# robj0nes/VectorizedMultiAgentSimulator

Hardware: AMD Instinct MI355X
Metric: env-steps/sec (num_envs x steps / wall-s), 'balance' @32k envs, 1->8 GPU (higher is better)
Workload: dtype f32; 1 GPU; balance 32768 envs/GPU, n_agents=4, substeps=10, broadphase=batch; scenario=balance, num_envs_per_gpu=32768, global_envs=32768, n_agents=4, substeps=10, parallelism=replicas x1 (one process per GPU, no collective in the step), math=relaxed

## Files before the change

### include/vmas_mi355x.h

```cpp
#ifndef VMAS_MI355X_H
#define VMAS_MI355X_H

#ifndef __HIPCC_RTC__
#include <stdint.h>
#endif

#ifdef __cplusplus
extern "C" {
#endif

#define VMAS_ABI_VERSION 14

#define VMAS_OK 0
#define VMAS_E_INVALID (-1)
#define VMAS_E_HIP (-2)
#define VMAS_E_NOMEM (-3)
#define VMAS_E_NOCONVERGE (-4)
#define VMAS_E_UNSUPPORTED (-5)

#define VMAS_SPHERE 0
#define VMAS_BOX 1
#define VMAS_LINE 2

#define VMAS_PAIR_JOINT 0
// ... 376 lines not shown
    float* obs[VMAS_SCN_MAX_AGENTS];
    uint8_t* done;
    float* pos_rew_prev;
    const int64_t* out_delta;
} VmasBalanceIO;
int32_t vmas_balance_outputs(int32_t device, const VmasBalanceIO* io, void* stream);
int32_t vmas_test_exact_math(int32_t device, const float* a, const float* b, float* out, int64_t n, void* stream);
int32_t vmas_test_fast_trig(int32_t device, const float* x, float* out, int64_t n, void* stream);

#define VMAS_SCN_MAX_RAY_TARGETS 16
#define VMAS_FLOCK_MAX_AGENTS 16
typedef struct VmasFlockingIO {
    int32_t batch, n_all, n_policy, what;
    int32_t target, n_rays, n_ray_targets, sum_mode;
    float min_collision_distance, collision_reward, desired_distance, dist_shaping_factor;
    float max_range, pad0;
    int32_t collide_reward_on;
    int32_t fast_lidar;
    VmasShapeRef agents[VMAS_FLOCK_MAX_AGENTS];
    int32_t scripted[VMAS_FLOCK_MAX_AGENTS];
    int32_t policy[VMAS_FLOCK_MAX_AGENTS];
    VmasVec vel[VMAS_FLOCK_MAX_AGENTS];
    VmasVec rot[VMAS_FLOCK_MAX_AGENTS];
    const float* angles[VMAS_FLOCK_MAX_AGENTS];
    int32_t ang_s0[VMAS_FLOCK_MAX_AGENTS], ang_s1[VMAS_FLOCK_MAX_AGENTS];
    VmasRayTarget ray_targets[VMAS_SCN_MAX_RAY_TARGETS];
    float* t;
    const float* shaping_in[VMAS_FLOCK_MAX_AGENTS];
    float* shaping_out[VMAS_FLOCK_MAX_AGENTS];
    float* dist_rew[VMAS_FLOCK_MAX_AGENTS];
    float* collision_rew[VMAS_FLOCK_MAX_AGENTS];
    float* rewards[VMAS_FLOCK_MAX_AGENTS];
    float* obs[VMAS_FLOCK_MAX_AGENTS];
    float* lidar[VMAS_FLOCK_MAX_AGENTS];
    const int64_t* out_delta;
} VmasFlockingIO;
int32_t vmas_flocking_outputs(int32_t device, const VmasFlockingIO* io, void* stream);
int32_t vmas_flocking_target_action(int32_t device, const float* t, int32_t batch, float period, float* u,
                                    void* stream);

#define VMAS_NAV_MAX_AGENTS 16
#define VMAS_NAV_WS_WORDS 32
typedef struct VmasNavigationIO {
    int32_t batch, n_agents, what, n_rays;
    int32_t shared_rew, observe_all_goals;
    int32_t lidar_on;
    int32_t fast_lidar;
    float pos_shaping_factor, final_reward, agent_collision_penalty, min_collision_distance;
    float max_range, pad0;
    VmasShapeRef agents[VMAS_NAV_MAX_AGENTS];
    VmasVec goal_pos[VMAS_NAV_MAX_AGENTS];
    float goal_radius[VMAS_NAV_MAX_AGENTS];
    double circ[VMAS_NAV_MAX_AGENTS];
    uint32_t pair_static[VMAS_NAV_MAX_AGENTS];
    VmasVec vel[VMAS_NAV_MAX_AGENTS];
    VmasVec rot[VMAS_NAV_MAX_AGENTS];
    const float* angles[VMAS_NAV_MAX_AGENTS];
    int32_t ang_s0[VMAS_NAV_MAX_AGENTS], ang_s1[VMAS_NAV_MAX_AGENTS];
    const float* shaping_in[VMAS_NAV_MAX_AGENTS];
    float* shaping_out[VMAS_NAV_MAX_AGENTS];
    float* dist_to_goal[VMAS_NAV_MAX_AGENTS];
    uint8_t* on_goal[VMAS_NAV_MAX_AGENTS];
    float* agent_pos_rew[VMAS_NAV_MAX_AGENTS];
    float* collision_rew[VMAS_NAV_MAX_AGENTS];
    float* rewards[VMAS_NAV_MAX_AGENTS];
    float* obs[VMAS_NAV_MAX_AGENTS];
    float* lidar[VMAS_NAV_MAX_AGENTS];
    float* pos_rew;
    float* final_rew;
    uint8_t* all_goal_reached;
    uint8_t* done;
    uint32_t* ws;
    const int64_t* out_delta;
} VmasNavigationIO;
int32_t vmas_navigation_outputs(int32_t device, const VmasNavigationIO* io, void* stream);

#define VMAS_TRANSPORT_MAX_PACKAGES 8
#define VMAS_TRANSPORT_MAX_AGENTS 16
typedef struct VmasTransportIO {
    int32_t batch, n_agents, n_packages, what;
    float shaping_factor, red[3], green[3], pad0;
    VmasShapeRef package[VMAS_TRANSPORT_MAX_PACKAGES], goal[VMAS_TRANSPORT_MAX_PACKAGES];
    VmasVec package_vel[VMAS_TRANSPORT_MAX_PACKAGES];
    VmasVec agent_pos[VMAS_TRANSPORT_MAX_AGENTS], agent_vel[VMAS_TRANSPORT_MAX_AGENTS];
    const float* global_shaping[VMAS_TRANSPORT_MAX_PACKAGES];
    int32_t gs_s0[VMAS_TRANSPORT_MAX_PACKAGES];
    float* global_shaping_out[VMAS_TRANSPORT_MAX_PACKAGES];
    float* dist_to_goal[VMAS_TRANSPORT_MAX_PACKAGES];
    uint8_t* on_goal[VMAS_TRANSPORT_MAX_PACKAGES];
    float* color[VMAS_TRANSPORT_MAX_PACKAGES];
    const uint8_t* on_goal_in[VMAS_TRANSPORT_MAX_PACKAGES];
    float* rew;
    float* obs[VMAS_TRANSPORT_MAX_AGENTS];
    uint8_t* done;
    const int64_t* out_delta;
    float* rew_attr;
} VmasTransportIO;
int32_t vmas_transport_outputs(int32_t device, const VmasTransportIO* io, void* stream);

#define VMAS_DISC_MAX_AGENTS 16
#define VMAS_DISC_MAX_TARGETS 16
#define VMAS_DISC_MAX_ENTITIES 32
#define VMAS_DISC_MAX_LIDARS 2
typedef struct VmasDiscoveryIO {
    int32_t batch, n_agents, n_targets, what;
    float covering_range, covering_rew_coeff, time_penalty;
    int32_t agents_per_target, shared_reward, n_entities, n_lidars;
    int32_t time_int;
    int32_t fast_lidar;
    int64_t time_penalty_i;
    int32_t agent_entity[VMAS_DISC_MAX_AGENTS];
    int32_t target_entity[VMAS_DISC_MAX_TARGETS];
    VmasVec pos[VMAS_DISC_MAX_ENTITIES];
    float radius[VMAS_DISC_MAX_ENTITIES];
    VmasVec vel[VMAS_DISC_MAX_AGENTS], rot[VMAS_DISC_MAX_AGENTS];
    int32_t n_rays[VMAS_DISC_MAX_LIDARS];
    float max_range[VMAS_DISC_MAX_LIDARS];
    uint32_t mask[VMAS_DISC_MAX_LIDARS];
    const float* angles[VMAS_DISC_MAX_LIDARS][VMAS_DISC_MAX_AGENTS];
    int32_t ang_s0[VMAS_DISC_MAX_LIDARS][VMAS_DISC_MAX_AGENTS], ang_s1[VMAS_DISC_MAX_LIDARS][VMAS_DISC_MAX_AGENTS];
    float* lidar[VMAS_DISC_MAX_LIDARS][VMAS_DISC_MAX_AGENTS];
    float* obs[VMAS_DISC_MAX_AGENTS];
    float* agents_pos;
    float* targets_pos;
    float* dists;
    int64_t* per_target;
    uint8_t* covered;
    void* time_rew;
    float* shared;
    float* covering[VMAS_DISC_MAX_AGENTS];
    float* collision[VMAS_DISC_MAX_AGENTS];
    float* rewards[VMAS_DISC_MAX_AGENTS];
    int64_t* covered_count;
    const uint8_t* all_time;
    uint8_t* done;
    const int64_t* out_delta;
    const uint64_t* stage_in;
    uint64_t* stage_out;
} VmasDiscoveryIO;
int32_t vmas_discovery_outputs(int32_t device, const VmasDiscoveryIO* io, void* stream);

#define VMAS_COPY_STORE64 (-8)
#define VMAS_COPY_MAX_SPANS 160
typedef struct VmasCopySpan {
    const void* src;
    void* dst;
    int64_t nbytes;
} VmasCopySpan;
int32_t vmas_copy_spans(int32_t device, const VmasCopySpan* spans, int32_t n, void* stream);
int32_t vmas_copy_spans_draw(int32_t device, const VmasCopySpan* spans, int32_t n_spans, int64_t numel,
                             const VmasUniformColumn* cols, int32_t n_cols, uint64_t seed, uint64_t offset,
                             const uint64_t* offset_dev, int32_t mode, int64_t u_snap_delta, uint64_t* increment,
                             void* stream);
int32_t vmas_graph_chain_launch_tail(const VmasKernelChain* chain, int32_t wb, const VmasCopySpan* spans,
                                     int32_t n_spans, int64_t numel, const VmasUniformColumn* cols, int32_t n_cols,
                                     uint64_t seed, uint64_t offset, const uint64_t* offset_dev, int32_t mode,
                                     int64_t u_snap_delta, uint64_t* increment, void* stream);
int32_t vmas_test_tail_draw(int32_t device, const VmasUniformColumn* cols, int32_t n_cols, int64_t numel, uint64_t seed,
                            uint64_t offset, int32_t mode, uint64_t* increment, void* stream);

const char* vmas_aux_last_error(void);

typedef struct VmasGradIO {
    float* const* pos;
    float* const* vel;
    float* const* rot;
    float* const* ang_vel;
    float* const* force;
    float* const* torque;
} VmasGradIO;
int32_t vmas_world_step_vjp(const VmasWorldConfig* cfg, const VmasEntityDesc* entities,
                            const VmasPairDesc* pairs, const VmasJointDesc* joints,
                            const VmasStepIO* io, const VmasStepIO* grad_out,
                            const VmasGradIO* grad_in, void* stream);
int32_t vmas_distance_vjp(int32_t device, int32_t batch, int32_t kind, const VmasShapeRef* a,
                          const VmasShapeRef* b, const float* test_point, int32_t tp_s0, int32_t tp_s1,
                          const float* grad_out, float* grad_a_pos, float* grad_a_rot, float* grad_b_pos,
                          float* grad_b_rot, float* grad_point, void* stream);
int32_t vmas_cast_rays_vjp(int32_t device, int32_t batch, int32_t n_rays, const float* origin,
                           int32_t o_s0, int32_t o_s1, const float* angles, int32_t a_s0,
                           int32_t a_s1, const float* rot, int32_t r_s0,
                           const VmasRayTarget* targets, int32_t n_targets, float max_range,
                           const float* grad_out, float* grad_origin, float* grad_rot,
                           float* grad_angles, float* const* grad_target_pos,
                           float* const* grad_target_rot, void* stream);

typedef struct VmasJitWorld VmasJitWorld;
int32_t vmas_jit_world_create(const VmasWorldConfig* cfg, const VmasEntityDesc* entities,
                              const VmasPairDesc* pairs, const VmasJointDesc* joints,
                              VmasJitWorld** out_world);
int32_t vmas_jit_world_destroy(VmasJitWorld* world);
int32_t vmas_jit_world_step(VmasJitWorld* world, const VmasStepIO* io, void* stream,
                            int32_t* iterations);
int32_t vmas_jit_world_set_params(VmasJitWorld* world, const VmasWorldConfig* cfg,
                                  const VmasEntityDesc* entities, const VmasPairDesc* pairs,
                                  const VmasJointDesc* joints);
int32_t vmas_jit_world_check(VmasJitWorld* world);
int32_t vmas_jit_world_passes(VmasJitWorld* world, int32_t* passes);
int32_t vmas_jit_world_grid(const VmasJitWorld* world);
int32_t vmas_jit_world_set_timing(VmasJitWorld* world, int32_t enable);
int32_t vmas_jit_world_get_timing(VmasJitWorld* world, int32_t reset, double* total_ms,
                                  int64_t* launches);
int32_t vmas_jit_world_device_timing(VmasJitWorld* world, int32_t reset, double* total_ms,
                                     int64_t* launches, double* clock_ghz);
int32_t vmas_jit_world_source(const VmasJitWorld* world, char* buf, int64_t cap);
int32_t vmas_jit_world_epilogue(const VmasJitWorld* world);
int32_t vmas_jit_program_outputs(VmasJitWorld* world, int32_t kind, const void* io, void* stream);
int32_t vmas_jit_compile_check(const VmasWorldConfig* cfg, const VmasEntityDesc* entities,
                               const VmasPairDesc* pairs, const VmasJointDesc* joints, char* buf,
                               int64_t cap);
int32_t vmas_jit_world_profile(VmasJitWorld* world, uint64_t* out, int64_t cap);
const char* vmas_jit_last_error(void);
int32_t vmas_jit_stats(int64_t* compiles, int64_t* cached);

#define VMAS_PRIM_NONE 0
#define VMAS_PRIM_DISC 1
#define VMAS_PRIM_POLY 2
#define VMAS_PRIM_SEG 3
#define VMAS_PRIM_RING 4
#define VMAS_PRIM_GRID 5
#define VMAS_PRIM_BORDER 1

typedef struct VmasRenderPrim {
    int32_t kind;
    int32_t flags;
    float rgba[4];
    float p[6];
    int32_t v0, nv;
    float bbox[4];
} VmasRenderPrim;

int32_t vmas_render_frames(int32_t device, int32_t n_frames, int32_t height, int32_t width,
                           const VmasRenderPrim* prims, int32_t n_prims, const float* verts,
                           int32_t n_verts, uint8_t* out, void* stream);

#define VMAS_RENDER_AGENT 1
#define VMAS_RENDER_ACTION 2
#define VMAS_RENDER_MAX_AGENTS 32

typedef struct VmasRenderEntity {
    const float* pos;
    const float* rot;
    const float* color;
    const uint8_t* mask;
    const float* force;
    int32_t pos_s0, rot_s0, color_s0, force_s0;
    int32_t shape;
    int32_t flags;
    float radius, length, width;
    float alpha;
    float action_scale;
    int32_t slot;
    int32_t action_slot;
    int32_t vert_slot;
} VmasRenderEntity;

typedef struct VmasRenderLidar {
    const float* pos;
    const float* rot;
    const float* angles;
    const float* dist;
    const uint8_t* mask;
    int32_t pos_s0, rot_s0, angles_s0, dist_s0;
    int32_t n_rays;
    int32_t slot;
    float alpha;
    float rgb[3];
} VmasRenderLidar;

typedef struct VmasRenderScene {
    int32_t width, height;
    int32_t focus;
    int32_t n_boundary;
    float boundary[4][4];
    int32_t plot_grid;
    float grid_spacing;
    float origin[2];
    float zoom;
    float max_agent_radius;
    int32_t n_boxes;
    int32_t n_prims;
    int32_t batch;
} VmasRenderScene;

int32_t vmas_render_scene(int32_t device, int32_t n_frames, const int64_t* env_index,
                          const VmasRenderEntity* entities, int32_t n_entities,
                          const VmasRenderLidar* lidars, int32_t n_lidars,
                          const VmasRenderScene* scene, VmasRenderPrim* prims, float* verts,
                          float* bounds, void* stream);

#define VMAS_MASKED_MAX_SPANS 96
typedef struct VmasMaskedSpan {
    void* dst;
    const void* src;
    int64_t row_bytes;
    int64_t dst_stride, src_stride;
} VmasMaskedSpan;
int32_t vmas_masked_rows(int32_t device, const VmasMaskedSpan* spans, int32_t n, const uint8_t* mask, int64_t batch,
                         int32_t copy_if_set, void* stream);

typedef struct VmasMutVec {
    float* p;
    int32_t s0, s1;
} VmasMutVec;
typedef struct VmasResetEntity {
    VmasMutVec pos, vel, rot, ang_vel;
// ... 119 lines not shown
```

### vectorizedmultiagentsimulator_amd/_native.py

```python
from __future__ import annotations

import ctypes
import os
from pathlib import Path

import numpy as np

LIB_NAME = "libvmas_mi355x.so"
LIB_PATH = Path(os.environ.get("VMAS_LIB_PATH") or Path(__file__).resolve().parent / LIB_NAME)

VMAS_ABI_VERSION = 14
VMAS_SPHERE, VMAS_BOX, VMAS_LINE = 0, 1, 2
(
    VMAS_PAIR_JOINT,
    VMAS_PAIR_SS,
    VMAS_PAIR_LS,
    VMAS_PAIR_LL,
    VMAS_PAIR_BS,
    VMAS_PAIR_BL,
    VMAS_PAIR_BB,
) = range(7)
F_MOVABLE = 1 << 0
F_ROTATABLE = 1 << 1
F_HOLLOW = 1 << 2
F_AGENT = 1 << 3
F_MAX_F = 1 << 4
F_F_RANGE = 1 << 5
F_MAX_T = 1 << 6
F_T_RANGE = 1 << 7
F_MAX_SPEED = 1 << 8
F_V_RANGE = 1 << 9
F_LIN_FRIC = 1 << 10
F_ANG_FRIC = 1 << 11
F_GRAVITY = 1 << 12
BROADPHASE_BATCH = 0
BROADPHASE_ENV = 1
DIST_POINT, DIST_PAIR, OVERLAP_PAIR = 0, 1, 2
EPILOGUE_NONE, EPILOGUE_BALANCE, EPILOGUE_TRANSPORT = 0, 1, 2

EXPORTED_SYMBOLS = (
    "vmas_abi_version",
    "vmas_device_count",
    "vmas_last_error",
    "vmas_stream_abort_capture",
    "vmas_graph_launch",
    "vmas_graph_chain_build",
    "vmas_graph_chain_launch",
    "vmas_graph_chain_free",
    "vmas_graph_chain_nodes",
    "vmas_graph_chain_fused",
    "vmas_graph_chain_set_writeback",
    "vmas_graph_chain_launch_wb",
    "vmas_jit_world_epilogue",
    "vmas_jit_program_outputs",
    "vmas_host_waits",
    "vmas_test_hold",
    "vmas_balance_outputs",
    "vmas_test_exact_math",
    "vmas_test_fast_trig",
    "vmas_copy_spans",
    "vmas_spawn_targets",
    "vmas_spawn_scratch_words",
    "vmas_spawn_channel_create",
    "vmas_spawn_channel_destroy",
    "vmas_spawn_channel_arm",
    "vmas_spawn_channel_in",
    "vmas_spawn_channel_wait",
    "vmas_spawn_profile",
    "vmas_world_step_vjp",
    "vmas_distance_vjp",
    "vmas_cast_rays_vjp",
    "vmas_flocking_outputs",
    "vmas_flocking_target_action",
    "vmas_navigation_outputs",
    "vmas_sampling_outputs",
    "vmas_sampling_max_pdf",
    "vmas_assert_publish_range",
    "vmas_transport_outputs",
    "vmas_discovery_outputs",
    "vmas_world_create",
    "vmas_world_destroy",
    "vmas_world_step",
    "vmas_world_set_timing",
    "vmas_world_get_timing",
    "vmas_cast_rays",
    "vmas_distance",
    "vmas_check_actions",
    "vmas_apply_actions",
    "vmas_apply_actions_launch",
    "vmas_apply_actions_flags",
    "vmas_apply_discrete_actions",
    "vmas_apply_discrete_actions_launch",
    "vmas_uniform_columns",
    "vmas_uniform_columns_snap",
    "vmas_copy_spans_draw",
    "vmas_graph_chain_launch_tail",
    "vmas_test_tail_draw",
    "vmas_assert_create",
    "vmas_assert_destroy",
    "vmas_assert_publish",
    "vmas_assert_wait",
    "vmas_spawn_resolve",
    "vmas_aux_last_error",
    "vmas_jit_world_create",
    "vmas_jit_world_destroy",
    "vmas_jit_world_step",
    "vmas_jit_world_set_timing",
    "vmas_jit_world_get_timing",
    "vmas_jit_world_device_timing",
    "vmas_jit_world_source",
    "vmas_jit_compile_check",
    "vmas_jit_world_profile",
    "vmas_jit_world_passes",
    "vmas_jit_world_check",
    "vmas_jit_world_grid",
    "vmas_jit_world_set_params",
    "vmas_jit_stats",
    "vmas_jit_last_error",
    "vmas_render_frames",
    "vmas_render_scene",
    "vmas_masked_rows",
    "vmas_balance_reset",
    "vmas_spawn_reset",
    "vmas_action_programs",
    "vmas_velocity_pid",
)

_i32 = ctypes.c_int32
_u32 = ctypes.c_uint32
_f32 = ctypes.c_float
_vp = ctypes.c_void_p


class VmasEntityDesc(ctypes.Structure):
    _fields_ = [
        ("shape", _i32),
        ("flags", _u32),
        ("agent_index", _i32),
        ("out_lin", _i32),
        ("out_rot", _i32),
        ("out_force", _i32),
        ("out_torque", _i32),
        ("radius", _f32),
        ("half_length", _f32),
        ("half_width", _f32),
        ("mass", _f32),
        ("inertia", _f32),
        ("one_minus_drag", _f32),
        ("lin_fric", _f32),
        ("ang_fric", _f32),
        ("max_speed", _f32),
        ("v_range", _f32),
        ("max_f", _f32),
        ("f_range", _f32),
        ("max_t", _f32),
        ("t_range", _f32),
    ]


class VmasPairDesc(ctypes.Structure):
    _fields_ = [
        ("cls", _i32),
        ("ea", _i32),
        ("eb", _i32),
        ("joint", _i32),
        ("bp_radius", _f32),
        ("dmin", _f32),
    ]


class VmasJointDesc(ctypes.Structure):
    _fields_ = [
        ("delta_a_x", _f32),
        ("delta_a_y", _f32),
        ("delta_b_x", _f32),
        ("delta_b_y", _f32),
        ("dist", _f32),
        ("rotate", _i32),
        ("fixed_rotation", _f32),
        ("pad", _i32),
    ]


class VmasWorldConfig(ctypes.Structure):
    _fields_ = [
        ("n_entities", _i32),
        ("n_agents", _i32),
        ("n_pairs", _i32),
        ("n_joints", _i32),
        ("batch", _i32),
        ("device", _i32),
        ("n_out_lin", _i32),
        ("n_out_rot", _i32),
        ("n_out_force", _i32),
        ("n_out_torque", _i32),
        ("contact_margin", _f32),
        ("collision_force", _f32),
        ("joint_force", _f32),
        ("torque_constraint_force", _f32),
        ("gravity_x", _f32),
        ("gravity_y", _f32),
        ("has_world_gravity", _i32),
        ("x_semidim", _f32),
        ("y_semidim", _f32),
        ("has_x_semidim", _i32),
        ("has_y_semidim", _i32),
        ("max_substeps", _i32),
        ("export_forces", _i32),
        ("epilogue", _i32),
        ("pad_cfg", _i32),
    ]


class VmasStepIO(ctypes.Structure):
    _fields_ = [
        ("entities", _vp),
        ("agents", _vp),
        ("joints", _vp),
        ("out_pos", _vp),
        ("out_vel", _vp),
        ("out_rot", _vp),
        ("out_ang_vel", _vp),
        ("out_force", _vp),
        ("out_torque", _vp),
        ("substeps", _i32),
        ("sub_dt", _f32),
        ("broadphase", _i32),
        ("pad", _i32),
        ("out_fdict", _vp),
        ("out_tdict", _vp),
    ]


class VmasShapeRef(ctypes.Structure):
    _fields_ = [
        ("shape", _i32),
        ("pad0", _i32),
        ("radius", _f32),
        ("length", _f32),
        ("width", _f32),
        ("radius_lmd", _f32),
        ("pos", _vp),
        ("rot", _vp),
        ("pos_s0", _i32),
        ("pos_s1", _i32),
        ("rot_s0", _i32),
        ("pad", _i32),
    ]


VMAS_COPY_MAX_SPANS = 160


class VmasCopySpan(ctypes.Structure):
    _fields_ = [("src", _vp), ("dst", _vp), ("nbytes", ctypes.c_int64)]


def copy_raw(device_index: int, spans, stream) -> None:
    n = len(spans)
    if not n:
        return
    arr = (VmasCopySpan * n)()
    for i, (src, dst, nb) in enumerate(spans):
        arr[i].src, arr[i].dst, arr[i].nbytes = src, dst, nb
    check_aux(load_library().vmas_copy_spans(device_index, arr, n, stream), "vmas_copy_spans")


VMAS_SPAWN_MAX_TARGETS = 16
VMAS_SPAWN_MAX_TRIES = 65536


VMAS_SPAWN_ERR_WORD = 64
VMAS_SPAWN_OFF_END_WORD = 36
VMAS_SPAWN_RNG_WORD = 40


def spawn_words(n_targets: int) -> int:
    return 96 + 32 * n_targets + 32 * 32


class VmasSpawnTargetsIO(ctypes.Structure):
    _fields_ = [
        ("batch", _i32), ("n_agents", _i32), ("n_targets", _i32), ("mode", _i32),
        ("agents", _vp), ("ag_s0", _i32), ("ag_s1", _i32), ("ag_s2", _i32), ("max_tries", _i32),
        ("pos", _vp * VMAS_SPAWN_MAX_TARGETS), ("pos_s0", _i32 * VMAS_SPAWN_MAX_TARGETS),
        ("pos_s1", _i32 * VMAS_SPAWN_MAX_TARGETS),
        ("covered", _vp), ("cov_s0", _i32), ("cov_s1", _i32),
        ("min_dist", _f32), ("x_lo", _f32), ("x_hi", _f32), ("y_lo", _f32), ("y_hi", _f32), ("pad1", _f32),
        ("seed", ctypes.c_uint64), ("offset", ctypes.c_uint64), ("max_accepted", _vp), ("channel", _vp),
        ("backup", _vp), ("scratch", _vp), ("scratch_words", ctypes.c_int64), ("prestaged", _i32), ("pad2", _i32),
    ]


COPY_SPAN_DTYPE = np.dtype([("src", np.uint64), ("dst", np.uint64), ("nbytes", np.int64)])
VMAS_COPY_STORE64 = -8


def stream_ptr(index: int) -> int:
    return _raw_stream(index)


def _raw_stream(index):
    import torch

    return torch._C._cuda_getCurrentRawStream(index)


def launch_args(device):
    if device.type != "cuda":
        return -1, None
    import torch

    idx = device.index if device.index is not None else torch.cuda.current_device()
    return idx, stream_ptr(idx)


def copy_table(device_index: int, table: np.ndarray, lo: int, hi: int, stream) -> None:
    copy_table_at(device_index, table.ctypes.data, lo, hi, stream)


def copy_table_at(device_index: int, table_addr: int, lo: int, hi: int, stream) -> None:
    if hi > lo:
        rc = (_copy_fn or _bind_copy())(device_index, table_addr + lo * COPY_SPAN_DTYPE.itemsize, hi - lo, stream)
        if rc:
            check_aux(rc, "vmas_copy_spans")


_copy_fn = None


def _bind_copy():
    global _copy_fn
    _copy_fn = load_library().vmas_copy_spans
    return _copy_fn


def copy_spans(device_index: int, pairs, stream) -> None:
    copy_raw(device_index, [(s.data_ptr(), d.data_ptr(), d.numel() * d.element_size()) for d, s in pairs], stream)


VMAS_PRIM_NONE, VMAS_PRIM_DISC, VMAS_PRIM_POLY, VMAS_PRIM_SEG, VMAS_PRIM_RING, VMAS_PRIM_GRID = range(6)
VMAS_PRIM_BORDER = 1
VMAS_RENDER_AGENT, VMAS_RENDER_ACTION = 1, 2
VMAS_RENDER_MAX_AGENTS = 32
RENDER_PRIM_DTYPE = np.dtype([("kind", np.int32), ("flags", np.int32), ("rgba", np.float32, 4), ("p", np.float32, 6),
                              ("v0", np.int32), ("nv", np.int32), ("bbox", np.float32, 4)])
assert RENDER_PRIM_DTYPE.itemsize == 72


class VmasRenderEntity(ctypes.Structure):
    _fields_ = [("pos", _vp), ("rot", _vp), ("color", _vp), ("mask", _vp), ("force", _vp),
                ("pos_s0", _i32), ("rot_s0", _i32), ("color_s0", _i32), ("force_s0", _i32),
                ("shape", _i32), ("flags", _i32), ("radius", _f32), ("length", _f32), ("width", _f32),
                ("alpha", _f32), ("action_scale", _f32), ("slot", _i32), ("action_slot", _i32), ("vert_slot", _i32)]


class VmasRenderLidar(ctypes.Structure):
    _fields_ = [("pos", _vp), ("rot", _vp), ("angles", _vp), ("dist", _vp), ("mask", _vp),
                ("pos_s0", _i32), ("rot_s0", _i32), ("angles_s0", _i32), ("dist_s0", _i32),
                ("n_rays", _i32), ("slot", _i32), ("alpha", _f32), ("rgb", _f32 * 3)]


class VmasRenderScene(ctypes.Structure):
    _fields_ = [("width", _i32), ("height", _i32), ("focus", _i32), ("n_boundary", _i32),
                ("boundary", (_f32 * 4) * 4), ("plot_grid", _i32), ("grid_spacing", _f32), ("origin", _f32 * 2),
                ("zoom", _f32), ("max_agent_radius", _f32), ("n_boxes", _i32), ("n_prims", _i32), ("batch", _i32)]


assert ctypes.sizeof(VmasRenderEntity) == 96 and ctypes.sizeof(VmasRenderLidar) == 80


class VmasGradIO(ctypes.Structure):
    _fields_ = [("pos", _vp), ("vel", _vp), ("rot", _vp), ("ang_vel", _vp), ("force", _vp), ("torque", _vp)]


class VmasVec(ctypes.Structure):
    _fields_ = [("p", _vp), ("s0", _i32), ("s1", _i32)]


VMAS_SCN_MAX_AGENTS = 32
VMAS_SCN_REWARD, VMAS_SCN_OBS, VMAS_SCN_DONE = 1, 2, 4


class VmasBalanceIO(ctypes.Structure):
    _fields_ = [
        ("batch", _i32), ("n_agents", _i32), ("what", _i32), ("pad0", _i32),
        ("shaping_factor", _f32), ("fall_reward", _f32), ("pi", _f32), ("pad1", _f32),
        ("package", VmasShapeRef), ("goal", VmasShapeRef), ("line", VmasShapeRef), ("floor", VmasShapeRef),
        ("package_vel", VmasVec), ("line_vel", VmasVec), ("line_ang_vel", VmasVec),
        ("agent_pos", VmasVec * VMAS_SCN_MAX_AGENTS), ("agent_vel", VmasVec * VMAS_SCN_MAX_AGENTS),
        ("global_shaping", _vp), ("gs_s0", _i32), ("pad2", _i32),
        ("global_shaping_out", _vp), ("package_dist", _vp), ("pos_rew", _vp), ("ground_rew", _vp),
        ("on_the_ground", _vp),
        ("rewards", _vp * VMAS_SCN_MAX_AGENTS), ("obs", _vp * VMAS_SCN_MAX_AGENTS),
        ("done", _vp), ("pos_rew_prev", _vp),
        ("out_delta", _vp),
    ]


VMAS_MASKED_MAX_SPANS = 96
MASKED_SPAN_DTYPE = np.dtype([("dst", np.uint64), ("src", np.uint64), ("row_bytes", np.int64),
                              ("dst_stride", np.int64), ("src_stride", np.int64)])


class VmasMaskedSpan(ctypes.Structure):
    _fields_ = [("dst", _vp), ("src", _vp), ("row_bytes", ctypes.c_int64), ("dst_stride", ctypes.c_int64),
                ("src_stride", ctypes.c_int64)]


def masked_rows(device_index: int, spans, mask_ptr: int, batch: int, copy_if_set: bool, stream) -> None:
    n = len(spans)
    if not n:
        return
    tbl = np.array(spans, dtype=np.uint64)
    assert tbl.shape == (n, 5)
    check_aux(load_library().vmas_masked_rows(device_index, tbl.ctypes.data, n, mask_ptr, batch, int(bool(copy_if_set)),
                                              stream), "vmas_masked_rows")


class VmasMutVec(ctypes.Structure):
    _fields_ = [("p", _vp), ("s0", _i32), ("s1", _i32)]


class VmasResetEntity(ctypes.Structure):
    _fields_ = [("pos", VmasMutVec), ("vel", VmasMutVec), ("rot", VmasMutVec), ("ang_vel", VmasMutVec)]


class VmasBalanceResetIO(ctypes.Structure):
    _fields_ = [
        ("batch", _i32), ("n_agents", _i32), ("mode", _i32), ("pad0", _i32),
        ("seed", ctypes.c_uint64), ("offset", ctypes.c_uint64), ("mask", _vp),
        ("lo", _f32 * 4), ("hi", _f32 * 4),
        ("line_y", _f32), ("package_rel_y", _f32), ("floor_x", _f32), ("floor_y", _f32), ("agent_dy", _f32),
        ("shaping_factor", _f32),
        ("floor_length", _f32), ("floor_width", _f32), ("line_length", _f32), ("package_radius_lmd", _f32),
        ("agent_dx", _f32 * VMAS_SCN_MAX_AGENTS),
        ("goal", VmasResetEntity), ("package", VmasResetEntity), ("line", VmasResetEntity), ("floor", VmasResetEntity),
        ("agents", VmasResetEntity * VMAS_SCN_MAX_AGENTS),
        ("force", VmasMutVec * VMAS_SCN_MAX_AGENTS), ("torque", VmasMutVec * VMAS_SCN_MAX_AGENTS),
        ("on_the_ground", _vp), ("global_shaping", VmasMutVec), ("steps", _vp),
    ]


VMAS_RESET_MAX_PLACE = 16
VMAS_RESET_MAX_WRITE = 24
VMAS_RESET_MAX_AGENTS = 16
VMAS_RESET_MAX_FIXED = 8
# ... 242 lines not shown
        ("flat", "<i4"),
        ("n_comp", "<i4"),
        ("n_phys", "<i4"),
        ("nvec", "<i4", (DISCRETE_MAX_COMPONENTS,)),
    ]
)
UNIFORM_COLUMN_DTYPE = np.dtype([("out", "<u8"), ("stride", "<i8"), ("from_", "<f4"), ("to", "<f4"), ("offset", "<u8"),
                                 ("u_out", "<u8"), ("u_stride", "<i8"), ("u_range", "<f4"), ("u_mult", "<f4"),
                                 ("u_clamp", "<i4"), ("pad", "<i4")])
DYNAMICS_DIFF_DRIVE, DYNAMICS_BICYCLE, DYNAMICS_DRONE = range(3)
INTEGRATION_EULER, INTEGRATION_RK4 = 0, 1
ACTION_PROGRAM_MAX_REFS = 8
ACTION_PROGRAM_REF_DTYPE = np.dtype(
    [(k, "<u8") for k in ("u", "pos", "vel", "rot", "ang_vel", "force", "torque", "drone_in", "drone_out")]
    + [(k, "<i8") for k in ("u_s0", "u_s1", "pos_s0", "pos_s1", "vel_s0", "vel_s1", "rot_s0", "ang_s0", "force_s0",
                            "force_s1")]
    + [(k, "<i4") for k in ("kind", "integration", "div_mode", "pad")]
    + [(k, "<f4") for k in ("mass", "moment_of_inertia", "dt", "dt2", "inv_dt2", "dt_6", "l_r", "wheelbase",
                            "inv_wheelbase", "max_steering_angle", "inv_mass", "g", "mass_g", "i_yz", "i_zx", "i_xy",
                            "i_xx", "i_yy", "i_zz", "inv_i_xx", "inv_i_yy", "inv_i_zz")]
)
VELOCITY_PID_REF_DTYPE = np.dtype(
    [(k, "<u8") for k in ("u", "vel", "u_out", "err_out", "prev_err", "accum", "accum_clamped")]
    + [(k, "<i8") for k in ("u_s0", "u_s1", "vel_s0", "vel_s1")]
    + [(k, "<i4") for k in ("dim", "use_integrator", "div_mode", "pad")]
    + [(k, "<f4") for k in ("gain", "inv_ti", "t_d", "dt", "inv_dt", "cutoff", "mass", "pad2")]
)
assert ACTION_PROGRAM_REF_DTYPE.itemsize == 256
assert VELOCITY_PID_REF_DTYPE.itemsize == 136
ACTION_PROGRAM_CALLS = {"vmas_action_programs": 0, "vmas_velocity_pid": 0}


def action_programs(device_index: int, batch: int, refs: np.ndarray, stream) -> int:
    ACTION_PROGRAM_CALLS["vmas_action_programs"] += 1
    return load_library().vmas_action_programs(device_index, batch, refs.ctypes.data, len(refs), stream)


def velocity_pid(device_index: int, batch: int, ref: np.ndarray, stream) -> int:
    ACTION_PROGRAM_CALLS["vmas_velocity_pid"] += 1
    return load_library().vmas_velocity_pid(device_index, batch, ref.ctypes.data, stream)


assert UNIFORM_COLUMN_DTYPE.itemsize == 64
assert ACTION_REF_DTYPE.itemsize == 40
assert ACTION_APPLY_REF_DTYPE.itemsize == 56
assert DISCRETE_ACTION_REF_DTYPE.itemsize == 96
assert ENTITY_IO_DTYPE.itemsize == 72
assert AGENT_IO_DTYPE.itemsize == 32
assert JOINT_IO_DTYPE.itemsize == 16
assert RAY_TARGET_DTYPE.itemsize == 48 and ctypes.sizeof(VmasRayTarget) == 48
assert ctypes.sizeof(VmasEntityDesc) == 84
assert ctypes.sizeof(VmasShapeRef) == 56


class NativeLibraryError(RuntimeError):
    pass


_lib = None


def load_library(path: os.PathLike | str | None = None) -> ctypes.CDLL:
    global _lib
    if _lib is not None and path is None:
        return _lib
    p = Path(path) if path is not None else LIB_PATH
    if not p.exists():
        raise NativeLibraryError(
            f"{p} not found: build it with `python -c 'import __graft_entry__ as g; g.build()'` "
            "(the MI355X engine has no Python fallback)"
        )
    lib = ctypes.CDLL(str(p))
    lib.vmas_abi_version.restype = _i32
    lib.vmas_device_count.restype = _i32
    lib.vmas_last_error.restype = ctypes.c_char_p
    lib.vmas_host_waits.restype = _i32
    lib.vmas_host_waits.argtypes = []
    lib.vmas_test_hold.restype = _i32
    lib.vmas_test_hold.argtypes = [_i32, _i32, ctypes.c_int64, _vp]
    lib.vmas_balance_outputs.restype = _i32
    lib.vmas_balance_outputs.argtypes = [_i32, _vp, _vp]
    lib.vmas_test_exact_math.restype = _i32
    lib.vmas_test_exact_math.argtypes = [_i32, _vp, _vp, _vp, ctypes.c_int64, _vp]
    lib.vmas_test_fast_trig.restype = _i32
    lib.vmas_test_fast_trig.argtypes = [_i32, _vp, _vp, ctypes.c_int64, _vp]
    lib.vmas_discovery_outputs.restype = _i32
    lib.vmas_discovery_outputs.argtypes = [_i32, _vp, _vp]
    lib.vmas_transport_outputs.restype = _i32
    lib.vmas_transport_outputs.argtypes = [_i32, _vp, _vp]
    lib.vmas_flocking_outputs.restype = _i32
    lib.vmas_flocking_outputs.argtypes = [_i32, _vp, _vp]
    lib.vmas_navigation_outputs.restype = _i32
    lib.vmas_navigation_outputs.argtypes = [_i32, _vp, _vp]
    lib.vmas_sampling_outputs.restype = _i32
    lib.vmas_sampling_outputs.argtypes = [_i32, _vp, _vp]
    lib.vmas_sampling_max_pdf.restype = _i32
    lib.vmas_sampling_max_pdf.argtypes = [_i32, _vp, _vp]
    lib.vmas_distance_vjp.restype = _i32
    lib.vmas_distance_vjp.argtypes = [_i32, _i32, _i32, _vp, _vp, _vp, _i32, _i32, _vp, _vp, _vp, _vp, _vp, _vp, _vp]
    lib.vmas_cast_rays_vjp.restype = _i32
    lib.vmas_cast_rays_vjp.argtypes = [_i32, _i32, _i32, _vp, _i32, _i32, _vp, _i32, _i32, _vp, _i32, _vp, _i32,
                                       ctypes.c_float, _vp, _vp, _vp, _vp, _vp, _vp, _vp]
    lib.vmas_world_step_vjp.restype = _i32
    lib.vmas_world_step_vjp.argtypes = [_vp, _vp, _vp, _vp, _vp, _vp, _vp, _vp]
    lib.vmas_spawn_targets.restype = _i32
    lib.vmas_spawn_targets.argtypes = [_i32, _vp, ctypes.POINTER(ctypes.c_uint64), _vp]
    lib.vmas_spawn_scratch_words.restype = ctypes.c_int64
    lib.vmas_spawn_scratch_words.argtypes = [_i32, _i32]
    lib.vmas_spawn_channel_create.restype = _i32
    lib.vmas_spawn_channel_create.argtypes = [_i32, ctypes.POINTER(_vp)]
    lib.vmas_spawn_channel_destroy.restype = _i32
    lib.vmas_spawn_channel_destroy.argtypes = [_vp]
    lib.vmas_spawn_channel_in.restype = _i32
    lib.vmas_spawn_channel_in.argtypes = [_vp, ctypes.POINTER(_vp)]
    lib.vmas_spawn_channel_arm.restype = _i32
    lib.vmas_spawn_channel_arm.argtypes = [_vp, ctypes.c_uint64, ctypes.c_uint64, ctypes.c_uint32]
    lib.vmas_spawn_channel_wait.restype = _i32
    lib.vmas_spawn_channel_wait.argtypes = [_vp, ctypes.c_uint32, ctypes.POINTER(_i32), _i32, _vp]
    lib.vmas_spawn_profile.restype = _i32
    lib.vmas_spawn_profile.argtypes = [_vp, ctypes.c_int64]
    lib.vmas_copy_spans.restype = _i32
    lib.vmas_copy_spans.argtypes = [_i32, _vp, _i32, _vp]
    lib.vmas_copy_spans_draw.restype = _i32
    lib.vmas_copy_spans_draw.argtypes = [_i32, _vp, _i32, ctypes.c_int64, _vp, _i32, ctypes.c_uint64, ctypes.c_uint64,
                                         _vp, _i32, ctypes.c_int64, ctypes.POINTER(ctypes.c_uint64), _vp]
    lib.vmas_masked_rows.restype = _i32
    lib.vmas_masked_rows.argtypes = [_i32, _vp, _i32, _vp, ctypes.c_int64, _i32, _vp]
    lib.vmas_balance_reset.restype = _i32
    lib.vmas_balance_reset.argtypes = [_i32, _vp, ctypes.POINTER(ctypes.c_uint64), _vp]
    lib.vmas_spawn_reset.restype = _i32
    lib.vmas_spawn_reset.argtypes = [_i32, _vp, ctypes.POINTER(ctypes.c_uint64), ctypes.POINTER(_i32), _vp]
    lib.vmas_stream_abort_capture.restype = _i32
    lib.vmas_stream_abort_capture.argtypes = [_vp]
    lib.vmas_graph_launch.restype = _i32
    lib.vmas_graph_launch.argtypes = [_vp, _vp]
    lib.vmas_graph_chain_build.restype = _i32
    lib.vmas_graph_chain_build.argtypes = [_vp, _i32, ctypes.POINTER(_vp)]
    lib.vmas_graph_chain_launch.restype = _i32
    lib.vmas_graph_chain_launch.argtypes = [_vp, _vp]
    lib.vmas_graph_chain_free.restype = _i32
    lib.vmas_graph_chain_nodes.restype = _i32
    lib.vmas_graph_chain_nodes.argtypes = [_vp]
    lib.vmas_graph_chain_fused.restype = _i32
    lib.vmas_graph_chain_fused.argtypes = [_vp]
    lib.vmas_graph_chain_set_writeback.restype = _i32
    lib.vmas_graph_chain_set_writeback.argtypes = [_vp, ctypes.c_int64]
    lib.vmas_graph_chain_launch_wb.restype = _i32
    lib.vmas_graph_chain_launch_wb.argtypes = [_vp, _vp]
    lib.vmas_test_tail_draw.restype = _i32
    lib.vmas_test_tail_draw.argtypes = [_i32, _vp, _i32, ctypes.c_int64, ctypes.c_uint64, ctypes.c_uint64, _i32, _vp, _vp]
    lib.vmas_graph_chain_launch_tail.restype = _i32
    lib.vmas_graph_chain_launch_tail.argtypes = [_vp, _i32, _vp, _i32, ctypes.c_int64, _vp, _i32, ctypes.c_uint64,
                                                 ctypes.c_uint64, _vp, _i32, ctypes.c_int64, _vp, _vp]
    lib.vmas_graph_chain_free.argtypes = [_vp]
    lib.vmas_world_create.restype = _i32
    lib.vmas_world_create.argtypes = [_vp, _vp, _vp, _vp, ctypes.POINTER(_vp)]
    lib.vmas_world_destroy.restype = _i32
    lib.vmas_world_destroy.argtypes = [_vp]
    lib.vmas_world_step.restype = _i32
    lib.vmas_world_step.argtypes = [_vp, _vp, _vp, _vp]
    lib.vmas_world_set_timing.restype = _i32
    lib.vmas_world_set_timing.argtypes = [_vp, _i32]
    lib.vmas_world_get_timing.restype = _i32
    lib.vmas_world_get_timing.argtypes = [_vp, _i32, ctypes.POINTER(ctypes.c_double), ctypes.POINTER(ctypes.c_int64)]
    lib.vmas_cast_rays.restype = _i32
    lib.vmas_cast_rays.argtypes = [
        _i32, _i32, _i32, _vp, _i32, _i32, _vp, _i32, _i32, _vp, _i32, _vp, _i32, _f32, _vp, _vp,
    ]
    lib.vmas_check_actions.restype = _i32
    lib.vmas_check_actions.argtypes = [_i32, _i32, _vp, _i32, _vp, _vp]
    lib.vmas_apply_actions.restype = _i32
    lib.vmas_apply_actions.argtypes = [_i32, _i32, _vp, _i32, _vp, _vp, _vp]
    lib.vmas_apply_actions_launch.restype = _i32
    lib.vmas_apply_actions_launch.argtypes = [_i32, _i32, _vp, _i32, _vp, ctypes.POINTER(ctypes.c_uint32), _vp]
    lib.vmas_apply_actions_flags.restype = _i32
    lib.vmas_apply_actions_flags.argtypes = [_i32, ctypes.c_uint32, _i32, _vp, _vp]
    lib.vmas_apply_discrete_actions.restype = _i32
    lib.vmas_apply_discrete_actions.argtypes = [_i32, _i32, _vp, _i32, _vp, _i32, _vp, _vp]
    lib.vmas_apply_discrete_actions_launch.restype = _i32
    lib.vmas_apply_discrete_actions_launch.argtypes = [_i32, _i32, _vp, _i32, _vp, _i32, ctypes.POINTER(ctypes.c_uint32), _vp]
    lib.vmas_uniform_columns.restype = _i32
    lib.vmas_uniform_columns.argtypes = [_i32, ctypes.c_int64, _vp, _i32, ctypes.c_uint64, ctypes.c_uint64, _i32,
                                         ctypes.POINTER(ctypes.c_uint64), _vp]
    lib.vmas_uniform_columns_snap.restype = _i32
    lib.vmas_uniform_columns_snap.argtypes = [_i32, ctypes.c_int64, _vp, _i32, ctypes.c_uint64, ctypes.c_uint64, _i32,
                                              ctypes.c_int64, ctypes.POINTER(ctypes.c_uint64), _vp]
    lib.vmas_assert_create.restype = _i32
    lib.vmas_assert_create.argtypes = [_i32, _i32, ctypes.POINTER(_vp)]
    lib.vmas_assert_destroy.restype = _i32
    lib.vmas_assert_destroy.argtypes = [_vp]
    lib.vmas_assert_publish.restype = _i32
    lib.vmas_assert_publish.argtypes = [_vp, _i32, _vp, ctypes.c_int64, _vp]
    lib.vmas_assert_wait.restype = _i32
    lib.vmas_assert_wait.argtypes = [_vp, _i32, ctypes.c_uint32, ctypes.POINTER(_i32), _vp]
    lib.vmas_assert_publish_range.restype = _i32
    lib.vmas_assert_publish_range.argtypes = [_vp, _i32, _vp, ctypes.c_int64, ctypes.c_int64, _i32, _i32, _vp, _vp, _vp]
    lib.vmas_flocking_target_action.restype = _i32
    lib.vmas_flocking_target_action.argtypes = [_i32, _vp, _i32, _f32, _vp, _vp]
    lib.vmas_distance.restype = _i32
    lib.vmas_distance.argtypes = [_i32, _i32, _i32, _vp, _vp, _vp, _i32, _i32, _vp, _vp]
    lib.vmas_spawn_resolve.restype = _i32
    lib.vmas_spawn_resolve.argtypes = [
        _i32, _i32, _vp, _i32, _i32, _i32, _i32, _vp, _i32, _i32, _f32, _vp, _vp,
        ctypes.POINTER(_i32), ctypes.POINTER(_i32), _vp,
    ]
    lib.vmas_aux_last_error.restype = ctypes.c_char_p
    lib.vmas_render_frames.restype = _i32
    lib.vmas_render_frames.argtypes = [_i32, _i32, _i32, _i32, _vp, _i32, _vp, _i32, _vp, _vp]
    lib.vmas_render_scene.restype = _i32
    lib.vmas_render_scene.argtypes = [_i32, _i32, _vp, _vp, _i32, _vp, _i32, _vp, _vp, _vp, _vp, _vp]
    lib.vmas_jit_world_create.restype = _i32
    lib.vmas_jit_world_create.argtypes = [_vp, _vp, _vp, _vp, ctypes.POINTER(_vp)]
    lib.vmas_jit_world_destroy.restype = _i32
    lib.vmas_jit_world_destroy.argtypes = [_vp]
    lib.vmas_jit_world_step.restype = _i32
    lib.vmas_jit_world_step.argtypes = [_vp, _vp, _vp, _vp]
    lib.vmas_jit_world_set_timing.restype = _i32
    lib.vmas_jit_world_set_timing.argtypes = [_vp, _i32]
    lib.vmas_jit_world_get_timing.restype = _i32
    lib.vmas_jit_world_get_timing.argtypes = [_vp, _i32, ctypes.POINTER(ctypes.c_double),
                                              ctypes.POINTER(ctypes.c_int64)]
    lib.vmas_jit_world_source.restype = _i32
    lib.vmas_jit_world_source.argtypes = [_vp, _vp, ctypes.c_int64]
    lib.vmas_jit_compile_check.restype = _i32
    lib.vmas_jit_compile_check.argtypes = [_vp, _vp, _vp, _vp, _vp, ctypes.c_int64]
    lib.vmas_jit_world_profile.restype = _i32
    lib.vmas_jit_world_profile.argtypes = [_vp, _vp, ctypes.c_int64]
    lib.vmas_jit_world_passes.restype = _i32
    lib.vmas_jit_world_passes.argtypes = [_vp, ctypes.POINTER(_i32)]
    lib.vmas_jit_world_device_timing.restype = _i32
    lib.vmas_jit_world_device_timing.argtypes = [_vp, _i32, ctypes.POINTER(ctypes.c_double),
                                                 ctypes.POINTER(ctypes.c_int64), ctypes.POINTER(ctypes.c_double)]
    lib.vmas_jit_world_check.restype = _i32
    lib.vmas_jit_world_check.argtypes = [_vp]
    lib.vmas_jit_world_grid.restype = _i32
    lib.vmas_jit_world_grid.argtypes = [_vp]
    lib.vmas_jit_world_set_params.restype = _i32
    lib.vmas_jit_world_set_params.argtypes = [_vp, _vp, _vp, _vp, _vp]
    lib.vmas_jit_stats.restype = _i32
    lib.vmas_jit_stats.argtypes = [ctypes.POINTER(ctypes.c_int64), ctypes.POINTER(ctypes.c_int64)]
    lib.vmas_jit_last_error.restype = ctypes.c_char_p
    lib.vmas_jit_world_epilogue.restype = _i32
    lib.vmas_jit_world_epilogue.argtypes = [_vp]
    lib.vmas_jit_program_outputs.restype = _i32
    lib.vmas_jit_program_outputs.argtypes = [_vp, _i32, _vp, _vp]
    lib.vmas_action_programs.restype = _i32
    lib.vmas_action_programs.argtypes = [_i32, _i32, _vp, _i32, _vp]
    lib.vmas_velocity_pid.restype = _i32
    lib.vmas_velocity_pid.argtypes = [_i32, _i32, _vp, _vp]
    ver = lib.vmas_abi_version()
    if ver != VMAS_ABI_VERSION:
        raise NativeLibraryError(f"ABI version mismatch: library {ver}, python {VMAS_ABI_VERSION}")
    if path is None:
        _lib = lib
    return lib


def check(rc: int, what: str) -> None:
    if rc != 0:
        msg = load_library().vmas_last_error().decode(errors="replace")
        raise NativeLibraryError(f"{what} failed ({rc}): {msg}")


def check_jit(rc: int, what: str) -> None:
    if rc < 0:
        msg = load_library().vmas_jit_last_error().decode(errors="replace")
        raise NativeLibraryError(f"{what} failed ({rc}): {msg}")


def check_aux(rc: int, what: str) -> None:
    if rc != 0:
        msg = load_library().vmas_aux_last_error().decode(errors="replace")
        raise NativeLibraryError(f"{what} failed ({rc}): {msg}")


def jit_stats():
    c, n = ctypes.c_int64(0), ctypes.c_int64(0)
    load_library().vmas_jit_stats(ctypes.byref(c), ctypes.byref(n))
    return c.value, n.value


HOST_EXT_PATH = Path(__file__).resolve().parent / "_vmas_host.so"
_host = None


def load_host():
    global _host
    if _host is not None:
        return _host
    if not HOST_EXT_PATH.exists():
        raise NativeLibraryError(
            f"{HOST_EXT_PATH} not found: build it with `python -c 'import __graft_entry__ as g; g.build()'`")
    import importlib.util

    load_library()
    spec = importlib.util.spec_from_file_location("_vmas_host", HOST_EXT_PATH)
    mod = importlib.util.module_from_spec(spec)
    spec.loader.exec_module(mod)
    if mod.ABI_VERSION != VMAS_ABI_VERSION:
        raise NativeLibraryError(f"_vmas_host ABI {mod.ABI_VERSION} != library ABI {VMAS_ABI_VERSION}")
    _host = mod
    return mod


_fn_addrs = {}

# ... 7 lines not shown
```

### vectorizedmultiagentsimulator_amd/csrc/vmas_jit.hip

```cpp
#include <hip/hip_runtime.h>
#include <hip/hiprtc.h>
#include <hip/hip_ext.h>
#include <dlfcn.h>

#include "vmas_aux.hpp"
#include "vmas_jit_ops.hpp"
#include "vmas_jit_registry.hpp"

#include <algorithm>
#include <cstdarg>
#include <cstdio>
#include <cstdlib>
#include <cmath>
#include <cstring>
#include <memory>
#include <mutex>
#include <string>
#include <unordered_map>
#include <unordered_set>
#include <utility>
#include <vector>

#include "vmas_mi355x.h"

namespace {

thread_local std::string g_jit_err;

int32_t jfail(int32_t code, const char* fmt, ...) {
    char buf[1024];
    va_list ap;
    va_start(ap, fmt);
    vsnprintf(buf, sizeof buf, fmt, ap);
    va_end(ap);
    g_jit_err = buf;
    return code;
}

#define JHIP(x)                                                                                 \
    do {                                                                                        \
        hipError_t e_ = (x);                                                                    \
        if (e_ != hipSuccess) {                                                                 \
            (void)hipGetLastError();                                                            \
            return jfail(VMAS_E_HIP, "%s: %s", #x, hipGetErrorString(e_));                      \
        }                                                                                       \
    } while (0)

std::string fl(float v) {
    if (v != v) return "__builtin_nanf(\"\")";
    if (v == __builtin_huge_valf()) return "__builtin_huge_valf()";
    if (v == -__builtin_huge_valf()) return "(-__builtin_huge_valf())";
    char b[64];
    snprintf(b, sizeof b, "%af", (double)v);
    return b;
}
std::string it(long v) { return std::to_string(v); }
std::string bl(bool v) { return v ? "true" : "false"; }

constexpr const char* kRelaxedTag = "// vmas-math: relaxed";
constexpr const char* kFlagsTag = "// vmas-cflags:";

std::string codegen_flags(bool relaxed) {
    std::string f = " -fno-slp-vectorize";
    if (relaxed) f += " -fapprox-func -fno-hip-fp32-correctly-rounded-divide-sqrt";
    if (const char* x = getenv("VMAS_JIT_CFLAGS")) f += std::string(" ") + x;
    return f;
}


float sq_limit(float r) {
    if (!(r >= 0.f)) return -1.f;
    if (r == __builtin_huge_valf()) return __builtin_huge_valf();
    float x = r * r;
    while (x > 0.f && std::sqrt(x) > r) x = std::nextafter(x, 0.f);
    while (std::sqrt(std::nextafter(x, __builtin_huge_valf())) <= r) x = std::nextafter(x, __builtin_huge_valf());
    return x;
}

constexpr int kNW = 8;
constexpr int kMaxNW = 16;
constexpr int kProfBlocks = 4096;
constexpr int kProfRec = 24;
constexpr int kMaxArgBytes = 3584;
static_assert(sizeof(VmasBalanceIO) % 8 == 0 && sizeof(VmasTransportIO) % 8 == 0,
              "a scenario program's argument block is copied into LDS in 8-byte words");
constexpr int kEpiQRows = 28;
constexpr int kLdsTwoPerCu = 64 * 1024;
constexpr int kLdsOnePerCu = 150 * 1024;

enum Src { S_POS, S_VEL, S_ROT, S_ANG, S_GRAV, S_FORCE, S_TORQUE, S_JFIX };
enum Prm { kPrmMass, kPrmInertia, kPrmDrag, kPrmLinFric, kPrmAngFric, kPrmMaxSpeed, kPrmVRange, kPrmMaxF, kPrmFRange,
           kPrmMaxT, kPrmTRange };
inline float prm_value(const VmasEntityDesc& d, int k) {
    switch (k) {
        case kPrmMass: return d.mass;
        case kPrmInertia: return d.inertia;
        case kPrmDrag: return d.one_minus_drag;
        case kPrmLinFric: return d.lin_fric;
        case kPrmAngFric: return d.ang_fric;
        case kPrmMaxSpeed: return d.max_speed;
        case kPrmVRange: return d.v_range;
        case kPrmMaxF: return d.max_f;
        case kPrmFRange: return d.f_range;
        case kPrmMaxT: return d.max_t;
        default: return d.t_range;
    }
}
inline float prm_world_value(const VmasWorldConfig& c, int k) {
    return k == 0 ? c.gravity_x : k == 1 ? c.gravity_y : k == 2 ? c.x_semidim : c.y_semidim;
}

struct Item {
    int pair, side, torque;
};
constexpr int kWhole = -1, kFinish = -2;
struct Task {
    int pair, part;
    float cost;
};

struct Gen {
    const VmasWorldConfig& cfg;
    const std::vector<VmasEntityDesc>& ed;
    const std::vector<VmasPairDesc>& pd;
    const std::vector<VmasJointDesc>& jd;
    int E, P, A, J, W, nfl;
    bool split_boxes = true;
    bool side_prune = true;
    bool splits(int cls) const {
        return split_boxes && (cls == VMAS_PAIR_BB || (cls == VMAS_PAIR_BL && !side_prune));
    }
    long lds_budget = kLdsTwoPerCu;
    bool global_rows = false;
    int nw = kNW;
    int prof_block = -1;
    bool relaxed = false;
    std::vector<char> dyn, in_pair, need_trig, need_rot, split;
    std::vector<int> owner;
    std::vector<std::vector<int>> wave_ents, wave_static;
    std::vector<std::vector<Task>> wave_tasks;
    std::vector<std::vector<Item>> items;
    std::vector<int> split_idx;
    int n_split = 0;
    std::vector<int> r_p, r_rot, r_trig, r_res;
    int n_rows = 0;
    std::vector<std::pair<int, int>> ptr_src, str_src;
    std::vector<int> ptr_of[8], str_of[8][2];
    std::string src;

    Gen(const VmasWorldConfig& c, const std::vector<VmasEntityDesc>& e, const std::vector<VmasPairDesc>& p,
        const std::vector<VmasJointDesc>& j)
        : cfg(c), ed(e), pd(p), jd(j) {
        E = c.n_entities;
        P = c.n_pairs;
        A = c.n_agents;
        J = c.n_joints;
        W = std::max(1, (P + 31) / 32);
        nfl = 2 * c.max_substeps * W;
    }

    static int parts(int cls) { return cls == VMAS_PAIR_BL ? 4 : 8; }

    int ptr(Src s, int idx) {
        int& slot = ptr_of[s][idx];
        if (slot < 0) {
            slot = (int)ptr_src.size();
            ptr_src.push_back({s, idx});
        }
        return slot;
    }
    int str(Src s, int k, int idx) {
        int& slot = str_of[s][k][idx];
        if (slot < 0) {
            slot = (int)str_src.size();
            str_src.push_back({s * 4 + k, idx});
        }
        return slot;
    }
    int rows(int n) {
        const int r = n_rows;
        n_rows += n;
        return r;
    }

    bool plan(std::string* why) {
        dyn.assign(E, 0);
        in_pair.assign(E, 0);
        need_trig.assign(E, 0);
        need_rot.assign(E, 0);
        split.assign(P, 0);
        split_idx.assign(P, -1);
        for (int e = 0; e < E; ++e) dyn[e] = (ed[e].flags & (VMAS_F_MOVABLE | VMAS_F_ROTATABLE)) != 0;
        for (const auto& q : pd) {
            in_pair[q.ea] = in_pair[q.eb] = 1;
            if (q.cls == VMAS_PAIR_JOINT) need_trig[q.ea] = need_trig[q.eb] = need_rot[q.ea] = need_rot[q.eb] = 1;
        }
        for (int e = 0; e < E; ++e) {
            if (in_pair[e] && ed[e].shape != VMAS_SPHERE) need_trig[e] = 1;
            if (need_trig[e]) need_rot[e] = 1;
        }
        for (int p = 0; p < P; ++p) {
            split[p] = splits(pd[p].cls);
            if (split[p]) split_idx[p] = n_split++;
        }
        items.assign(E, {});
        for (int p = 0; p < P; ++p) {
            for (int side = 0; side < 2; ++side) {
                const int e = side ? pd[p].eb : pd[p].ea;
                if (!dyn[e]) continue;
                int tq = 1;
                if (pd[p].cls == VMAS_PAIR_SS) tq = 0;
                if ((pd[p].cls == VMAS_PAIR_LS || pd[p].cls == VMAS_PAIR_BS) && side == 1) tq = 0;
                items[e].push_back({p, side, tq});
            }
        }
        const float kCost[7] = {1.5f, 0.5f, 2.0f, 1.8f, 2.2f, 7.4f, 30.f};
        const float finish_cost = 3.0f;
        const float bl_part_cost = 1.8f, bb_part_cost = 3.8f;
        std::vector<Task> all;
        for (int p = 0; p < P; ++p) {
            if (split[p]) {
                for (int k = 0; k < parts(pd[p].cls); ++k)
                    all.push_back({p, k, pd[p].cls == VMAS_PAIR_BL ? bl_part_cost : bb_part_cost});
                all.push_back({p, kFinish, finish_cost});
            } else {
                all.push_back({p, kWhole, kCost[pd[p].cls]});
            }
        }
        std::stable_sort(all.begin(), all.end(), [](const Task& a, const Task& b) { return a.cost > b.cost; });
        wave_tasks.assign(nw, {});
        std::vector<float> load(nw, 0.f);
        auto place = [&](const Task& t) {
            const int w = (int)(std::min_element(load.begin(), load.end()) - load.begin());
            wave_tasks[w].push_back(t);
            load[w] += t.cost;
        };
        for (const Task& t : all) place(t);
        for (auto& v : wave_tasks)
            std::stable_sort(v.begin(), v.end(), [](const Task& a, const Task& b) {
                const int ra = a.part >= 0 ? 0 : a.part == kFinish ? 2 : 1;
                const int rb = b.part >= 0 ? 0 : b.part == kFinish ? 2 : 1;
                return ra != rb ? ra < rb : a.pair < b.pair;
            });
        owner.assign(E, -1);
        wave_ents.assign(nw, {});
        wave_static.assign(nw, {});
        {
            std::vector<int> order;
            for (int e = 0; e < E; ++e)
                if (dyn[e]) order.push_back(e);
            std::stable_sort(order.begin(), order.end(), [&](int a, int b) { return items[a].size() > items[b].size(); });
            std::vector<float> eload(nw, 0.f);
            for (int e : order) {
                const int w = (int)(std::min_element(eload.begin(), eload.end()) - eload.begin());
                owner[e] = w;
                wave_ents[w].push_back(e);
                eload[w] += 4.f + items[e].size();
            }
            int rr = 0;
            for (int e = 0; e < E; ++e)
                if (!dyn[e] && in_pair[e]) {
                    owner[e] = rr % nw;
                    wave_static[rr % nw].push_back(e);
                    ++rr;
                }
        }
        r_p.assign(E, -1);
        r_rot.assign(E, -1);
        r_trig.assign(E, -1);
        r_res.assign(P, -1);
        for (int e = 0; e < E; ++e) {
            if (!in_pair[e]) continue;
            r_p[e] = rows(2);
            if (need_rot[e]) r_rot[e] = rows(1);
            if (need_trig[e]) r_trig[e] = rows(4);
        }
        for (int p = 0; p < P; ++p) r_res[p] = rows(split[p] ? 4 * parts(pd[p].cls) + 8 : res_rows(p));
        const long red = (!global_rows && (long)std::max(n_rows, 1) * 64 >= nfl + 2) ? 0 : nfl + 2;
        const long lds = (global_rows ? 0L : (long)n_rows * 256) + (long)nfl * 4 + 4 * (n_split + 1) +
                         4L * (nfl / 2) + 4 * red + (has_epi() && !epi_q_in_rows() ? (long)kEpiQRows * 256 : 0L) +
                         (has_epi() ? (long)(cfg.epilogue == VMAS_EPILOGUE_BALANCE ? sizeof(VmasBalanceIO)
                                                                                   : sizeof(VmasTransportIO)) : 0L);
        if (lds > lds_budget) {
            *why = "LDS budget exceeded (" + it(lds) + " B)";
            return false;
        }
        for (auto& v : ptr_of) v.assign(std::max(E, std::max(A, J)) + 1, -1);
        for (auto& a : str_of)
            for (auto& v : a) v.assign(std::max(E, std::max(A, J)) + 1, -1);
        for (int e = 0; e < E; ++e) {
            if (!(dyn[e] || in_pair[e])) continue;
            ptr(S_POS, e), str(S_POS, 0, e), str(S_POS, 1, e);
            if (need_rot[e] || dyn[e]) ptr(S_ROT, e), str(S_ROT, 0, e);
            if (dyn[e]) {
                ptr(S_VEL, e), str(S_VEL, 0, e), str(S_VEL, 1, e);
                ptr(S_ANG, e), str(S_ANG, 0, e);
                if (ed[e].flags & VMAS_F_GRAVITY) ptr(S_GRAV, e), str(S_GRAV, 0, e), str(S_GRAV, 1, e);
                if (ed[e].agent_index >= 0) {
                    const int a = ed[e].agent_index;
                    ptr(S_FORCE, a), str(S_FORCE, 0, a), str(S_FORCE, 1, a);
                    ptr(S_TORQUE, a), str(S_TORQUE, 0, a);
                }
            }
        }
        for (int p = 0; p < P; ++p)
            if (pd[p].cls == VMAS_PAIR_JOINT) ptr(S_JFIX, pd[p].joint), str(S_JFIX, 0, pd[p].joint);
        if (str_src.size() % 2) str_src.push_back({-1, 0});
        plan_params();
        {
            const char* tl = getenv("VMAS_JIT_TAIL");
            tail = has_epi() && !(tl && tl[0] == '0');
            if (tail && arg_bytes() > kMaxArgBytes) tail = false;
            tail_stage = tail && lds + (long)sizeof(VmasTail) <= lds_budget;
        }
        if (arg_bytes() > kMaxArgBytes) {
            *why = "kernel argument block too large (" + it(arg_bytes()) + " B)";
            return false;
        }
        return true;
    }

    size_t n_out() const { return cfg.export_forces ? 8 : 6; }

    bool has_epi() const { return cfg.epilogue == VMAS_EPILOGUE_BALANCE || cfg.epilogue == VMAS_EPILOGUE_TRANSPORT; }
    const char* epi_type() const { return cfg.epilogue == VMAS_EPILOGUE_BALANCE ? "VmasBalanceIO" : "VmasTransportIO"; }
    std::string epi_call(const std::string& io, const std::string& g, const std::string& wave, const std::string& lane,
                         const std::string& q) const {
        if (cfg.epilogue == VMAS_EPILOGUE_BALANCE)
            return "balance_group(" + io + ", " + g + ", " + wave + ", " + it(nw) + ", " + lane + ", " + q + ")";
        return "transport_group(" + io + ", " + g + ", " + wave + ", " + it(nw) + ", " + lane + ")";
    }
    bool epi_q_in_rows() const { return !global_rows && n_rows >= kEpiQRows; }
    size_t epi_offset() const { return 8 * (std::max<size_t>(ptr_src.size(), 1) + n_out() + 7 + (global_rows ? 1 : 0)); }
    size_t wbd_offset() const { return epi_offset() + (has_epi() ? 8 : 0); }

    size_t tail_offset() const {
        const size_t n = 8 * (std::max<size_t>(ptr_src.size(), 1) + n_out() + 7 + (global_rows ? 1 : 0) + (has_epi() ? 1 : 0) + 1) +
                         4 * (std::max<size_t>(str_src.size(), 2) + 4) +
                         4 * std::max<size_t>(prm_src.size(), 1);
        return (n + 7) & ~(size_t)7;
    }
    size_t arg_bytes() const {
        return tail_offset() + (tail ? sizeof(VmasTail) : 0);
    }

    static std::string row(int r, int k = 0) { return "L[" + it((long)(r + k) * 64) + " + lane]"; }
    bool mine(int e, int w) const { return dyn[e] && owner[e] == w; }
    std::vector<char> pre_pos, pre_trig, pre_rot;
    std::string pos(int e, int w) const {
        if (mine(e, w)) return "p" + it(e);
        if (!pre_pos.empty() && pre_pos[e]) return "q" + it(e);
        return "mk(" + row(r_p[e]) + ", " + row(r_p[e], 1) + ")";
    }
    std::string rot(int e, int w) const {
        if (mine(e, w)) return "r" + it(e);
        if (!pre_rot.empty() && pre_rot[e]) return "o" + it(e);
        return row(r_rot[e]);
    }
    std::string trig(int e, int w) const {
        if (mine(e, w)) return "t" + it(e);
        if (!pre_trig.empty() && pre_trig[e]) return "u" + it(e);
        return "Trig{" + row(r_trig[e]) + ", " + row(r_trig[e], 1) + ", " + row(r_trig[e], 2) + ", " +
               row(r_trig[e], 3) + "}";
    }
    void task_reads(int w, std::vector<char>& rp, std::vector<char>& rt, std::vector<char>& rr) const {
        rp.assign(E, 0);
        rt.assign(E, 0);
        rr.assign(E, 0);
        for (const Task& k : wave_tasks[w]) {
            if (k.part == kFinish) continue;
            const VmasPairDesc& q = pd[k.pair];
            for (int side = 0; side < 2; ++side) {
                const int e = side ? q.eb : q.ea;
                if (mine(e, w)) continue;
                rp[e] = 1;
                const bool t = q.cls == VMAS_PAIR_LL || q.cls == VMAS_PAIR_BL || q.cls == VMAS_PAIR_BB ||
                               q.cls == VMAS_PAIR_JOINT ||
                               (side == 0 && (q.cls == VMAS_PAIR_LS || q.cls == VMAS_PAIR_BS));
                if (t && r_trig[e] >= 0) rt[e] = 1;
                if (q.cls == VMAS_PAIR_JOINT && r_rot[e] >= 0) rr[e] = 1;
            }
        }
    }
    std::string preload(int e, bool p, bool t, bool r) const {
        std::string o;
        if (p) o += "        const V2 q" + it(e) + " = mk(" + row(r_p[e]) + ", " + row(r_p[e], 1) + ");\n";
        if (t)
            o += "        const Trig u" + it(e) + " = Trig{" + row(r_trig[e]) + ", " + row(r_trig[e], 1) + ", " +
                 row(r_trig[e], 2) + ", " + row(r_trig[e], 3) + "};\n";
        if (r) o += "        const float o" + it(e) + " = " + row(r_rot[e]) + ";\n";
        return o;
    }
    std::string P_(Src s, int i) const { return "a.ptr[" + it(ptr_of[s][i]) + "]"; }
    std::string S_(Src s, int k, int i) const { return "a.str[" + it(str_of[s][k][i]) + "]"; }
    std::string ld2(Src s, int i, bool rb = false) const {
        return "ld2(" + (rb ? "rbp(" + P_(s, i) + ", rbd)" : P_(s, i)) + ", " + S_(s, 0, i) + ", " + S_(s, 1, i) + ", bb)";
    }
    std::string ld1(Src s, int i, bool rb = false) const {
        return (rb ? "rbp(" + P_(s, i) + ", rbd)" : P_(s, i)) + "[(long)bb * " + S_(s, 0, i) + "]";
    }
    std::string mbit(int p) const { return "(m" + it(p >> 5) + " & " + it(1u << (p & 31)) + "u)"; }
    int res(int p) const { return split[p] ? r_res[p] + 4 * parts(pd[p].cls) + 4 : r_res[p]; }

    std::string stamp(int w, const std::string& slot) const {
        if (prof_block < 0) return "";
        return "if ((b >> 6) == " + it(prof_block) + " && lane == 0) a.prof[(" + slot + ") * " + it(kMaxNW) + " + " +
               it(w) + "] = __builtin_amdgcn_s_memtime();\n";
    }

    std::string block_stamp(int k, const std::string& v) const {
        if (prof_block < 0) return "";
        return "    if (threadIdx.x == 0 && blockIdx.x < " + it(kProfBlocks) + ") a.prof[" +
               it((long)(cfg.max_substeps * 4 + 2) * kMaxNW) + " + blockIdx.x * " + it(kProfRec) + " + " + it(k) +
               "] = " + v + ";\n";
    }

    std::string desc(int e) const {
        const VmasEntityDesc& d = ed[e];
        std::string o = "{" + it(d.shape) + ", " + it(d.flags) + "u, " + it(d.agent_index) + ", " + it(d.out_lin) + ", " +
                        it(d.out_rot) + ", " + it(d.out_force) + ", " + it(d.out_torque) + ", " + fl(d.radius) + ", " +
                        fl(d.half_length) + ", " + fl(d.half_width);
        for (int k = 0; k <= kPrmTRange; ++k) o += ", 0.f";
        return o + "}";
    }
    static std::vector<int> value_fields(const VmasEntityDesc& d) {
        std::vector<int> f;
        const bool mov = d.flags & VMAS_F_MOVABLE, rotb = d.flags & VMAS_F_ROTATABLE;
        if (mov || (d.flags & VMAS_F_LIN_FRIC)) f.push_back(kPrmMass);
        if (rotb || (d.flags & VMAS_F_ANG_FRIC)) f.push_back(kPrmInertia);
        if (mov || rotb) f.push_back(kPrmDrag);
        if (d.flags & VMAS_F_LIN_FRIC) f.push_back(kPrmLinFric);
        if (d.flags & VMAS_F_ANG_FRIC) f.push_back(kPrmAngFric);
        if (d.flags & VMAS_F_MAX_SPEED) f.push_back(kPrmMaxSpeed);
        if (d.flags & VMAS_F_V_RANGE) f.push_back(kPrmVRange);
        if (d.flags & VMAS_F_MAX_F) f.push_back(kPrmMaxF);
// ... 220 lines not shown
                if (rotf)
                    bk_code += "        bk1(" + P_(S_ROT, e) + ", " + S_(S_ROT, 0, e) + ", bb, a.wbd, r" + s + ");\n        bk1(" +
                               P_(S_ANG, e) + ", " + S_(S_ANG, 0, e) + ", bb, a.wbd, w" + s + ");\n";
            }
            if (d.agent_index >= 0)
                o += "    V2 af" + s + " = " + ld2(S_FORCE, d.agent_index) + "; float at" + s + " = " +
                     ld1(S_TORQUE, d.agent_index) + ";\n";
            else
                o += "    V2 af" + s + " = mk(0.f, 0.f); float at" + s + " = 0.f;\n";
            if (d.flags & VMAS_F_GRAVITY) o += "    const V2 eg" + s + " = " + ld2(S_GRAV, e) + ";\n";
            else o += "    const V2 eg" + s + " = mk(0.f, 0.f);\n";
            if (need_trig[e])
                o += "    Trig t" + s + " = make_trig_for(r" + s + ", " + bl(d.shape == VMAS_BOX) + ");\n";
            publish(o, e, "    ", true, true);
            if (cfg.export_forces) o += "    float lfx" + s + " = 0.f, lfy" + s + " = 0.f, ltq" + s + " = 0.f;\n";
            o += runtime_desc(e, "    ");
        }
        const std::string pro = it((long)cfg.max_substeps * 4);
        if (w == 0) o += "    if (spec && threadIdx.x == 0) QL[65] = spec_ok ? 1u : 0u;\n";
        o += "    " + stamp(w, pro);
        o += "    __syncthreads();\n";
        o += "    const bool own = !spec || QL[65] != 0u;  // (a lost speculative claim: compute, store nothing)\n";
        if (!bk_code.empty()) o += "    if (bk && valid && own) {\n" + bk_code + "    }\n";
        o += "    " + stamp(w, pro + " + 1");
        std::vector<char> rp, rt, rr;
        task_reads(w, rp, rt, rr);
        for (int e = 0; e < E; ++e)
            if (!dyn[e] && (rp[e] || rt[e] || rr[e])) o += preload(e, rp[e], rt[e], rr[e]).substr(4);
        o += "    for (int s = 0; s < a.S; ++s) {\n";
        o += "        if (4 * s < a.S) __builtin_amdgcn_s_setprio(3); else if (2 * s < a.S) __builtin_amdgcn_s_setprio(2);"
             " else if (4 * s < 3 * a.S) __builtin_amdgcn_s_setprio(1); else __builtin_amdgcn_s_setprio(0);\n";
        std::vector<char> word(W, 0);
        for (const Task& t : wave_tasks[w]) word[t.pair >> 5] = 1;
        for (int e : wave_ents[w])
            for (const Item& x : items[e]) word[x.pair >> 5] = 1;
        for (int k = 0; k < W; ++k)
            if (word[k]) o += "        const uint32_t m" + it(k) + " = MSK[s * " + it(W) + " + " + it(k) + "];\n";
        std::vector<char> fword(W, 0);
        for (const Task& t : wave_tasks[w]) fword[t.pair >> 5] = 1;
        for (int k = 0; k < W; ++k)
            if (fword[k]) o += "        uint32_t fr" + it(k) + " = 0u, fz" + it(k) + " = 0u;\n";
        for (int e = 0; e < E; ++e)
            if (dyn[e] && (rp[e] || rt[e] || rr[e])) o += preload(e, rp[e], rt[e], rr[e]);
        pre_pos = rp;
        pre_trig = rt;
        pre_rot = rr;
        for (const Task& t : wave_tasks[w]) task_code(o, t, w);
        pre_pos.clear();
        pre_trig.clear();
        pre_rot.clear();
        o += flag_flush(fword);
        o += "        " + stamp(w, "s * 4");
        o += "        __syncthreads();\n";
        o += "        " + stamp(w, "s * 4 + 1");
        if (w == 0 && n_split)
            o += "        for (int i = lane; i < " + it(n_split) + "; i += 64) DONE[i] = 0u;\n";
        for (int e : wave_ents[w]) {
            const VmasEntityDesc& d = ed[e];
            const std::string s = it(e);
            const bool mov = d.flags & VMAS_F_MOVABLE, rotb = d.flags & VMAS_F_ROTATABLE;
            o += "        {  // entity " + s + "\n";
            o += "            float fx, fy, tq;\n";
            o += "            pre_forces(D" + s + ", " + bl(d.agent_index >= 0) + ", af" + s + ", at" + s + ", v" + s +
                 ", w" + s + ", eg" + s + ", " + bl(d.flags & VMAS_F_GRAVITY) + ", GX, GY, HAS_G, a.sdt, fx, fy, tq);\n";
            int k = 0;
            for (const Item& x : items[e]) {
                const int r = res(x.pair);
                const std::string c = "c" + it(k++);
                if (mov) o += "            const float " + c + "x = " + row(r) + ", " + c + "y = " + row(r, 1) + ";\n";
                if (rotb && x.torque) o += "            const float " + c + "t = " + row(r, x.side ? 3 : 2) + ";\n";
            }
            k = 0;
            for (const Item& x : items[e]) {
                const std::string c = "c" + it(k++), m = mbit(x.pair);
                if (mov) {
                    const std::string sx = x.side ? "-" + c + "x" : c + "x", sy = x.side ? "-" + c + "y" : c + "y";
                    o += "            fx = " + m + " ? fx + " + sx + " : fx; fy = " + m + " ? fy + " + sy + " : fy;\n";
                }
                if (rotb && x.torque) o += "            tq = " + m + " ? tq + " + c + "t : tq;\n";
            }
            if (cfg.export_forces) o += "            lfx" + s + " = fx; lfy" + s + " = fy; ltq" + s + " = tq;\n";
            o += "            integrate(D" + s + ", s, a.sdt, fx, fy, tq, HAS_XS, XS, HAS_YS, YS, p" + s + ", v" + s +
                 ", r" + s + ", w" + s + ");\n";
            if (need_trig[e] && rotb)
                o += "            t" + s + " = make_trig_for(r" + s + ", " + bl(d.shape == VMAS_BOX) + ");\n";
            publish(o, e, "            ", mov, rotb);
            o += "        }\n";
        }
        o += "        " + stamp(w, "s * 4 + 2");
        o += "        __syncthreads();\n";
        o += "        " + stamp(w, "s * 4 + 3");
        o += "    }\n";
        if (!wave_ents[w].empty()) {
            o += "    if (valid && own) {\n";
            for (int e : wave_ents[w]) {
                const VmasEntityDesc& d = ed[e];
                const std::string s = it(e);
                if (d.out_lin >= 0)
                    o += "        st_out2(a.out[0], (size_t)" + it(d.out_lin) + " * a.B + b, p" + s + ");\n        st_out2(a.out[1], (size_t)" +
                         it(d.out_lin) + " * a.B + b, v" + s + ");\n";
                if (d.out_rot >= 0)
                    o += "        st_out1(a.out[2], (size_t)" + it(d.out_rot) + " * a.B + b, r" + s + ");\n        st_out1(a.out[3], (size_t)" +
                         it(d.out_rot) + " * a.B + b, w" + s + ");\n";
                if (d.agent_index >= 0) {
                    if (d.out_force >= 0)
                        o += "        st_out2(a.out[4], (size_t)" + it(d.out_force) + " * a.B + b, af" + s + ");\n";
                    if (d.out_torque >= 0)
                        o += "        st_out1(a.out[5], (size_t)" + it(d.out_torque) + " * a.B + b, at" + s + ");\n";
                }
                if (cfg.export_forces)
                    o += "        st_out2(a.out[6], (size_t)" + s + " * a.B + b, mk(lfx" + s + ", lfy" + s +
                         "));\n        st_out1(a.out[7], (size_t)" + s + " * a.B + b, ltq" + s + ");\n";
                if (d.out_lin >= 0 || d.out_rot >= 0) {
                    o += "        if (wbk) {\n";
                    if (d.out_lin >= 0)
                        o += "            wb2(" + P_(S_POS, e) + ", " + S_(S_POS, 0, e) + ", " + S_(S_POS, 1, e) + ", b, p" + s +
                             ");\n            wb2(" + P_(S_VEL, e) + ", " + S_(S_VEL, 0, e) + ", " + S_(S_VEL, 1, e) + ", b, v" +
                             s + ");\n";
                    if (d.out_rot >= 0)
                        o += "            wb1(" + P_(S_ROT, e) + ", " + S_(S_ROT, 0, e) + ", b, r" + s + ");\n            wb1(" +
                             P_(S_ANG, e) + ", " + S_(S_ANG, 0, e) + ", b, w" + s + ");\n";
                    o += "        }\n";
                }
            }
            o += "    }\n";
        }
        o += "    return own;\n}\n\n";
    }

    std::string wb_helpers() const {
        return "__device__ __forceinline__ const float* rbp(const float* p, long long d) {\n"
               "    return reinterpret_cast<const float*>(reinterpret_cast<const char*>(p) + d);\n}\n"
               "__device__ __forceinline__ void bk1(const float* p, int s0, int b, long long d, float v) {\n"
               "    st_out1(const_cast<float*>(rbp(p, d)), (size_t)((long)b * s0), v);\n}\n"
               "__device__ __forceinline__ void bk2(const float* p, int s0, int s1, int b, long long d, V2 v) {\n"
               "    float* q = const_cast<float*>(rbp(p, d));\n"
               "    st_out1(q, (size_t)((long)b * s0), v.x);\n    st_out1(q, (size_t)((long)b * s0 + s1), v.y);\n}\n"
               "__device__ __forceinline__ void wb1(const float* p, int s0, int b, float v) {\n"
               "    const_cast<float*>(p)[(long)b * s0] = v;\n}\n"
               "__device__ __forceinline__ void wb2(const float* p, int s0, int s1, int b, V2 v) {\n"
               "    float* q = const_cast<float*>(p);\n    q[(long)b * s0] = v.x;\n    q[(long)b * s0 + s1] = v.y;\n}\n\n";
    }

    bool tail = false;
    bool tail_stage = false;
    std::string epi_text() const {
        if (!has_epi()) return "";
        return "        if (a.epi) {\n"
               "            __syncthreads();\n"
               "            " + epi_call("*PROG_IOP", "g", "wave", "lane", epi_q_in_rows() ? "L" : "EQ") + ";\n"
               "            __syncthreads();\n"
               "        }\n";
    }
    std::string loop_text() const {
        return "    bool spec = persistent && spec_first, spec_ok = true, own = true;\n"
               "    if (spec && threadIdx.x == 0) spec_ok = grid_claim(claim, (int)blockIdx.x, (CURP)->base);\n"
               "    for (;;) {\n"
               "        const int g = spec ? (int)blockIdx.x : grid_next(persistent, a.ctl, claim, a.mask, MSK, nwords, ngrp, CURP, QL);\n"
               "        if (g < 0) break;\n" + block_stamp(4, "__builtin_amdgcn_s_memrealtime()") +
               "        if (persistent) {\n"
               "            for (int i = threadIdx.x; i < nfl; i += blockDim.x) FL[i] = 0u;\n"
               "            __syncthreads();\n"
               "        }\n"
               "        {\n"
               "            const int b = g * 64 + lane;\n"
               "            const bool valid = b < a.B;\n"
               "            const int bb = valid ? b : (a.B - 1);\n"
               "            // the state write-back (Args.wbd, wb_text): this pass's inputs, its backup\n"
               "            const bool wbx = persistent && a.wbd != 0;\n"
               "            const long long rbd = (wbx && (CURP)->pass > 0) ? a.wbd : 0ll;\n"
               "            const bool bk = wbx && (CURP)->pass == 0;\n"
               "            own = run<WAVE>(a, L, FL, DONE, MSK, lane, b, bb, valid, rbd, bk, wbx, spec, spec_ok, QL);\n"
               "        }\n"
               "        spec = false;\n"
               "        if (!own) continue;\n" + epi_text() +
               "        if (persistent && grid_finish(g, FL, nfl, a.blk, a.mask, MSK, a.ctl, a.err, a.herr, nwords, ngrp, CURP,\n"
               "                                      a.max_pass, RED, &QL[65], a.tm, t0s.rt, t0s.sc))\n"
               "            poison_outputs(a);\n" + block_stamp(5, "__builtin_amdgcn_s_memrealtime()") +
               "    }\n";
    }

    void generate() {
        std::string& o = src;
        o += "// generated by vmas_jit.hip for one world\n";
        if (relaxed) o += std::string(kRelaxedTag) + "\n#define VMAS_PHYS_RELAXED 1\n";
        o += std::string(kFlagsTag) + codegen_flags(relaxed) + "\n";
        if (prof_block >= 0) o += "#define VMAS_JIT_PROFILE_SLOTS 1\n";
        if (const char* mp = getenv("VMAS_JIT_TEST_PASSES"))
            o += "#define VMAS_GRID_MIN_PASSES " + it(std::max(1, atoi(mp))) + "\n";
        o += "#include \"vmas_jit_ops.hpp\"\n";
        if (has_epi()) o += "#include \"vmas_programs.hpp\"\n";
        o += "using namespace vmas;\n\n";
        o += "struct Args {\n    const float* ptr[" + it(std::max<size_t>(ptr_src.size(), 1)) +
             "];\n    float* out[" + it(n_out()) + "];\n    uint32_t* mask;\n    uint32_t* blk;\n    unsigned long long* prof;\n"
             "    uint32_t* ctl;\n    uint32_t* err;\n    uint32_t* herr;\n    unsigned long long* tm;\n" +
             std::string(global_rows ? "    float* rows;\n" : "") +
             std::string(has_epi() ? std::string("    const ") + epi_type() + "* epi;\n" : std::string()) +
             "    long long wbd;\n" +
             "    int str[" + it(std::max<size_t>(str_src.size(), 2)) + "];\n    int B, S;\n    float sdt;\n    int max_pass;\n"
             "    float prm[" + it(std::max<size_t>(prm_src.size(), 1)) + "];\n" +
             std::string(tail ? "    VmasTail tail;\n" : "") + "};\n"
             "static_assert(sizeof(Args) == " + it((long)arg_bytes()) + ", \"argument block layout\");\n\n";
        o += "__device__ __forceinline__ V2 ld2(const float* p, int s0, int s1, int b) {\n"
             "    return mk(p[(long)b * s0], p[(long)b * s0 + s1]);\n}\n\n";
        o += wb_helpers();
        o += "constexpr WorldK WK{" + fl(cfg.contact_margin) + ", " + fl(cfg.collision_force) + ", " +
             fl(cfg.joint_force) + ", " + fl(cfg.torque_constraint_force) + "};\n";
        o += "__shared__ float PRM[" + it(std::max<size_t>(prm_src.size(), 1)) + "];\n";
        o += "constexpr float GX = " + fl(cfg.gravity_x) + ", GY = " + fl(cfg.gravity_y) + ";\n";
        o += "constexpr float XS = " + fl(cfg.x_semidim) + ", YS = " + fl(cfg.y_semidim) + ";\n";
        o += "constexpr bool HAS_G = " + bl(cfg.has_world_gravity) + ";\n";
        o += "constexpr bool HAS_XS = " + bl(cfg.has_x_semidim) + ", HAS_YS = " + bl(cfg.has_y_semidim) + ";\n";
        for (int e = 0; e < E; ++e)
            if (dyn[e]) o += "constexpr VmasEntityDesc D" + it(e) + "c" + desc(e) + ";\n";
        o += "\ntemplate <int WAVE>\n__device__ __forceinline__ bool run(const Args& a, float* L, uint32_t* FL, "
             "uint32_t* DONE, const uint32_t* MSK, int lane, int b, int bb, bool valid, long long rbd, bool bk, bool wbk, "
             "bool spec, bool spec_ok, uint32_t* QL);\n\n";
        for (int w = 0; w < nw; ++w) wave_body(o, w);
        const int waves_per_eu = (lds_budget <= kLdsTwoPerCu ? 2 : 1) * nw / 4;
        {
            const int n_lin = cfg.n_out_lin, n_rot = cfg.n_out_rot, n_f = cfg.n_out_force, n_t = cfg.n_out_torque;
            const int per_env[6] = {2 * n_lin, 2 * n_lin, n_rot, n_rot, 2 * n_f, n_t};
            o += "__device__ __forceinline__ void poison_outputs(const Args& a) {\n"
                 "    const float nan = __builtin_nanf(\"\");\n";
            for (int k = 0; k < 6; ++k)
                if (per_env[k] > 0)
                    o += "    for (size_t i = threadIdx.x; i < (size_t)" + it(per_env[k]) +
                         " * a.B; i += blockDim.x) a.out[" + it(k) + "][i] = nan;\n";
            o += "}\n\n";
        }
        o += "template <int WAVE>\n__device__ __forceinline__ void group_loop(const Args& a, float* L, uint32_t* FL, uint32_t* DONE, "
             "uint32_t* MSK, uint32_t* QL, uint32_t* RED, float* EQ, GridCursor* CURP, uint32_t* claim, TimerStart t0s, "
             "bool persistent, bool spec_first, int nfl, int nwords, int ngrp, int lane, int wave" +
             std::string(has_epi() ? std::string(", const ") + epi_type() + "* PROG_IOP" : std::string()) + ") {\n    (void)EQ;\n";
        o += loop_text();
        o += "}\n\n";
        o += "__device__ __forceinline__ void world_body(const Args& a) {\n";
        if (global_rows)
            o += "    float* L = a.rows + (size_t)blockIdx.x * " + it((long)std::max(n_rows, 1) * 64) + ";\n";
        else
            o += "    __shared__ __attribute__((aligned(16))) float L[" + it(std::max(n_rows, 1) * 64) + "];\n";
        o += "    __shared__ uint32_t FL[" + it(nfl) + "];\n";
        if (has_epi() && !epi_q_in_rows()) o += "    __shared__ float EQ[" + it((long)kEpiQRows * 64) + "];\n";
        if (has_epi()) o += std::string("    __shared__ __attribute__((aligned(16))) ") + epi_type() + " PROG_IO;\n";
        o += "    __shared__ uint32_t DONE[" + it(std::max(n_split, 1)) + "];\n";
        if (tail_stage)
            o += "    __shared__ __attribute__((aligned(16))) VmasTail TL;\n";
        const int red_words = nfl + 2;
        o += "    __shared__ uint32_t MSK[" + it(std::max(nfl / 2, 1)) + "];\n";
        o += "    __shared__ uint32_t QL[66];\n";
        if (!global_rows && (long)std::max(n_rows, 1) * 64 >= red_words)
            o += "    uint32_t* RED = reinterpret_cast<uint32_t*>(L);\n";
        else
            o += "    __shared__ uint32_t RED[" + it(red_words) + "];\n";
        o += "    const int lane = threadIdx.x & 63, wave = threadIdx.x >> 6;\n";
        o += "    const int nfl = 2 * a.S * " + it(W) + ", nwords = a.S * " + it(W) + ", ngrp = (a.B + 63) >> 6;\n"
             "    for (int i = threadIdx.x; i < " + it(n_split) + "; i += blockDim.x) DONE[i] = 0u;\n";
        o += "    const bool persistent = a.ctl != nullptr;\n"
             "    uint32_t* claim = a.mask + " + it(vmas::grid_claim_offset((long)cfg.max_substeps * W)) + ";\n"
             "    const TimerStart t0s = device_timer_start(persistent ? a.tm : nullptr, true);\n"
             "    __shared__ GridCursor CUR;\n"
             "    const bool spec_first = persistent && (int)blockIdx.x < ngrp;  // (the speculative first group: loop_text)\n"
             "    if (threadIdx.x == 0)\n"
             "        CUR = GridCursor{0, (int)blockIdx.x + (spec_first ? (int)gridDim.x : 0), 0, 0, 0, persistent ? ld64(&a.ctl[kGridEpoch]) : 0ull, 0};\n"
             "    for (int i = threadIdx.x; i < nfl; i += blockDim.x) FL[i] = 0u;\n"
             "    for (int i = threadIdx.x; i < nwords; i += blockDim.x) MSK[i] = ~ld_agent(&a.mask[i]);\n" +
             std::string(has_epi() ?
                 "    if (a.epi)\n"
                 "        for (int i = threadIdx.x; i < (int)(sizeof(PROG_IO) / 8); i += blockDim.x)\n"
                 "            reinterpret_cast<unsigned long long*>(&PROG_IO)[i] = reinterpret_cast<const unsigned long long*>(a.epi)[i];\n"
                 : "") +
             std::string(tail_stage ?
                 "    if (persistent && a.tail.n_items > 0) {\n"
                 "        const unsigned long long* ka = reinterpret_cast<const unsigned long long*>(\n"
                 "            (const char*)__builtin_amdgcn_kernarg_segment_ptr() + " + it((long)tail_offset()) + ");\n"
                 "        for (int i = threadIdx.x; i < (int)(sizeof(VmasTail) / 8); i += blockDim.x)\n"
                 "            reinterpret_cast<unsigned long long*>(&TL)[i] = ka[i];\n"
                 "    }\n"
                 : "") +
             prm_copy() +
             "    __syncthreads();\n" +
             block_stamp(0, "__builtin_amdgcn_s_memrealtime()") + block_stamp(1, "__builtin_amdgcn_s_getreg(63492)") +
             block_stamp(2, "__builtin_amdgcn_s_getreg(30740)") +
             (prof_block >= 0 ? "    if (lane == 0 && blockIdx.x < " + it(kProfBlocks) + ") a.prof[" +
                                    it((long)(cfg.max_substeps * 4 + 2) * kMaxNW) + " + blockIdx.x * " + it(kProfRec) +
                                    " + 8 + wave] = __builtin_amdgcn_s_getreg(63492);\n"
                              : "") +
             (prof_block >= 0 ? "    if (threadIdx.x == 0) vmas_prof_blk = a.prof + " + it((long)(cfg.max_substeps * 4 + 2) * kMaxNW) + ";\n" : "") +
             "";
        std::string sw = "    switch (wave) {\n";
        for (int w = 0; w < nw; ++w)
            sw += "        case " + it(w) + ": group_loop<" + it(w) + ">(a, L, FL, DONE, MSK, QL, RED, " +
                  std::string(has_epi() && !epi_q_in_rows() ? "EQ" : "nullptr") +
                  ", &CUR, claim, t0s, persistent, spec_first, nfl, nwords, ngrp, lane, wave" +
                  std::string(has_epi() ? ", &PROG_IO" : "") + "); break;\n";
        o += sw + "        default: break;\n    }\n";
        o += block_stamp(3, "__builtin_amdgcn_s_memrealtime()") +
             std::string(tail ? "    // the replay's post-replay work (vmas_tail.hpp): every group's final pass is decided\n"
                                "    if (persistent && a.tail.n_items > 0) " +
                                    std::string(tail_stage ? "vmas_tail::run(TL)" : "vmas_tail::run(a.tail)") + ";\n" : "") +
             "    if (!persistent) {\n"
             "        if (!a.blk) return;\n"
             "        __syncthreads();\n"
             "        for (int i = threadIdx.x; i < nfl; i += blockDim.x) st_agent(&a.blk[(size_t)blockIdx.x * nfl + i], FL[i]);\n"
             "        return;\n"
             "    }\n"
             "}\n\n";
        const std::string bounds = "__launch_bounds__(" + it(nw * 64) + ", " + it(waves_per_eu) + ")";
        o += "extern \"C\" __global__ void " + bounds + " k_world(Args a) {\n    world_body(a);\n}\n";
        if (has_epi())
            o += "\nextern \"C\" __global__ void __launch_bounds__(" + it(nw * 64) + ") k_program_jit(" + epi_type() + " io_arg) {\n"
                 "    VMAS_PROGRAM_ARGS(" + epi_type() + ", io_arg);\n"
                 "    __shared__ float Q[" + it((long)kEpiQRows * 64) + "];\n"
                 "    " + epi_call("io", "blockIdx.x", "(int)(threadIdx.x >> 6)", "(int)(threadIdx.x & 63)", "Q") + ";\n}\n";
    }
};

std::unique_ptr<Gen> make_plan(const VmasWorldConfig& cfg, const std::vector<VmasEntityDesc>& ed,
                               const std::vector<VmasPairDesc>& pd, const std::vector<VmasJointDesc>& jd,
                               std::string* why, int force_nw = 0) {
    const char* sp = getenv("VMAS_JIT_SPLIT");
    const bool allow_split = !(sp && sp[0] == '0');
    const char* spr = getenv("VMAS_JIT_SIDE_PRUNE");
    const bool side_prune = !(spr && spr[0] == '0');
    const struct {
        bool split;
        long budget;
        bool global_rows;
    } tries[] = {{true, kLdsTwoPerCu, false}, {false, kLdsTwoPerCu, false}, {false, kLdsOnePerCu, false},
                 {false, kLdsOnePerCu, true}};
    for (const auto& t : tries) {
        if (t.split && !allow_split) continue;
        std::unique_ptr<Gen> g(new Gen(cfg, ed, pd, jd));
        if ((size_t)cfg.max_substeps * g->W > 1024) {
            *why = "too many substeps x pairs";
            return nullptr;
        }
        g->split_boxes = t.split;
        g->side_prune = side_prune;
        g->lds_budget = t.budget;
        g->global_rows = t.global_rows;
        int n_tasks = 0;
        for (const auto& q : pd)
            n_tasks += g->splits(q.cls) ? Gen::parts(q.cls) + 1 : 1;
        g->nw = n_tasks >= 32 ? 16 : kNW;
        if (const char* nws = getenv("VMAS_JIT_WAVES")) g->nw = atoi(nws) == 16 ? 16 : kNW;
        if (force_nw) g->nw = force_nw;
        why->clear();
        if (g->plan(why)) return g;
    }
    return nullptr;
}

__global__ void __launch_bounds__(1024) k_jit_flags_reduce(const uint32_t* blk, int nblk, int S, int W,
                                                           uint32_t* mask, uint32_t* viol_out) {
    __shared__ uint32_t R[1024], Z[1024];
    __shared__ uint32_t viol;
    const int nwords = S * W;
    for (int w = threadIdx.x; w < nwords; w += blockDim.x) {
        R[w] = 0u;
        Z[w] = 0u;
    }
    if (threadIdx.x == 0) viol = 0u;
    __syncthreads();
    const int groups = max(1, (int)blockDim.x / nwords);
    if ((int)threadIdx.x < groups * nwords) {
        const int w = threadIdx.x % nwords, g0 = threadIdx.x / nwords;
        uint32_t r = 0u, z = 0u;
        for (int i = g0; i < nblk; i += groups) {
            r |= blk[(size_t)i * 2 * nwords + w];
            z |= blk[(size_t)i * 2 * nwords + nwords + w];
        }
        if (r) atomicOr(&R[w], r);
        if (z) atomicOr(&Z[w], z);
    }
    __syncthreads();
    for (int w = threadIdx.x; w < nwords; w += blockDim.x) {
        const uint32_t m = ~mask[w];
        if ((m & ~R[w] & Z[w]) | (~m & R[w])) atomicOr(&viol, 1u);
    }
    __syncthreads();
    if (viol)
        for (int w = threadIdx.x; w < nwords; w += blockDim.x) mask[w] = ~R[w];
    if (threadIdx.x == 0) *viol_out = viol;
}

bool relaxed_math(const VmasWorldConfig& cfg) {
    const char* m = getenv("VMAS_JIT_MATH");
    return !(m && std::string(m) == "exact") && cfg.n_joints == 0;
}

std::mutex g_cache_mu;
std::unordered_map<std::string, std::pair<std::vector<char>, uint64_t>> g_code_cache;
uint64_t g_cache_tick = 0;
constexpr size_t kCodeCacheMax = 32;
size_t code_cache_max() {
    const char* c = getenv("VMAS_JIT_CACHE");
    return c ? (size_t)std::max(1, atoi(c)) : kCodeCacheMax;
}

std::string module_dir() {
    Dl_info info{};
    if (dladdr((const void*)&jfail, &info) && info.dli_fname) {
        std::string p = info.dli_fname;
        const size_t k = p.rfind('/');
        return k == std::string::npos ? std::string(".") : p.substr(0, k);
    }
    return ".";
}

int64_t g_jit_compiles = 0;

int32_t compile(const std::string& src, std::vector<char>* code) {
    {
        std::lock_guard<std::mutex> lk(g_cache_mu);
        auto f = g_code_cache.find(src);
        if (f != g_code_cache.end()) {
            *code = f->second.first;
            f->second.second = ++g_cache_tick;
            return VMAS_OK;
        }
    }
    const std::string dir = module_dir();
    const std::string inc1 = "-I" + dir + "/csrc", inc2 = "-I" + dir + "/../include";
    std::vector<const char*> opts = {"--offload-arch=gfx950", "-O3", "-std=c++17", "-ffp-contract=off", "-fno-fast-math",
                                     inc1.c_str(), inc2.c_str()};
    std::vector<std::string> extra;
    const size_t at = src.find(kFlagsTag);
    if (at != std::string::npos) {
        const size_t b = at + strlen(kFlagsTag), e = src.find('\n', b);
        const std::string line = src.substr(b, e == std::string::npos ? std::string::npos : e - b);
        std::string t;
        for (char c : line + " ") {
            if (c == ' ') {
                if (!t.empty()) extra.push_back(t);
                t.clear();
            } else {
                t += c;
            }
        }
    }
    for (const std::string& x : extra) opts.push_back(x.c_str());
    hiprtcProgram prog;
    if (hiprtcCreateProgram(&prog, src.c_str(), "vmas_world.hip", 0, nullptr, nullptr) != HIPRTC_SUCCESS)
        return jfail(VMAS_E_HIP, "hiprtcCreateProgram failed");
    const hiprtcResult rc = hiprtcCompileProgram(prog, (int)opts.size(), opts.data());
    if (rc != HIPRTC_SUCCESS) {
        size_t n = 0;
        hiprtcGetProgramLogSize(prog, &n);
        std::string log(n + 1, '\0');
        hiprtcGetProgramLog(prog, &log[0]);
        hiprtcDestroyProgram(&prog);
        return jfail(VMAS_E_HIP, "hipRTC compile failed: %.900s", log.c_str());
    }
    size_t n = 0;
    hiprtcGetCodeSize(prog, &n);
    code->resize(n);
    hiprtcGetCode(prog, code->data());
    hiprtcDestroyProgram(&prog);
    std::lock_guard<std::mutex> lk(g_cache_mu);
    ++g_jit_compiles;
    while (!g_code_cache.empty() && g_code_cache.size() >= code_cache_max()) {
        auto lru = g_code_cache.begin();
        for (auto it2 = g_code_cache.begin(); it2 != g_code_cache.end(); ++it2)
            if (it2->second.second < lru->second.second) lru = it2;
        g_code_cache.erase(lru);
    }
    g_code_cache[src] = {*code, ++g_cache_tick};
    return VMAS_OK;
}

}

namespace vmas {
namespace {
std::mutex g_fn_mu;
std::unordered_map<const void*, JitFnInfo> g_live_fns;
}
void fn_register(hipFunction_t f, const JitFnInfo& info) {
    std::lock_guard<std::mutex> lk(g_fn_mu);
    g_live_fns[(const void*)f] = info;
}
void fn_unregister(hipFunction_t f) {
    if (!f) return;
    std::lock_guard<std::mutex> lk(g_fn_mu);
    g_live_fns.erase((const void*)f);
}
bool jit_fn_info(const void* f, JitFnInfo* out) {
    std::lock_guard<std::mutex> lk(g_fn_mu);
    auto it = g_live_fns.find(f);
    if (it == g_live_fns.end()) return false;
    if (out) *out = it->second;
    return true;
}
}

struct VmasJitWorld {
    VmasWorldConfig cfg{};
    std::vector<VmasEntityDesc> ed;
    std::vector<VmasPairDesc> pd;
    std::vector<VmasJointDesc> jd;
    std::string src;
    std::vector<std::pair<int, int>> ptr_src, str_src, prm_src;
    size_t arg_bytes = 0;
    int W = 1, nblk = 0, nw = kNW;
    hipModule_t mod = nullptr;
    hipFunction_t fn = nullptr;
    hipFunction_t fn_prog = nullptr;
    size_t epi_offset = 0;
    uint32_t *d_mask = nullptr, *d_blk = nullptr, *d_viol = nullptr, *h_viol = nullptr;
    uint32_t *d_ctl = nullptr, *d_err = nullptr, *h_err = nullptr, *dh_err = nullptr;
    int grid = 0;
    int max_passes = 0;
    hipStream_t last_stream = nullptr;
    int last_passes = 0;
    bool last_persistent = false;
    unsigned long long* d_prof = nullptr;
    size_t n_prof = 0;
    bool timing = false;
    std::vector<std::pair<hipEvent_t, hipEvent_t>> ev_pending, ev_free;
    double timed_ms = 0.0;
    long timed_launches = 0;
    unsigned long long* d_tm = nullptr;
    int wall_khz = 0;
    bool global_rows = false;
    float* d_rows = nullptr;
};

extern "C" {

const char* vmas_jit_last_error(void) { return g_jit_err.c_str(); }

int32_t vmas_jit_stats(int64_t* compiles, int64_t* cached) {
    std::lock_guard<std::mutex> lk(g_cache_mu);
    if (compiles) *compiles = g_jit_compiles;
    if (cached) *cached = (int64_t)g_code_cache.size();
    return VMAS_OK;
}

int32_t vmas_jit_world_destroy(VmasJitWorld* W) {
    if (!W) return VMAS_OK;
    if (W->cfg.device >= 0) {
        (void)hipSetDevice(W->cfg.device);
        vmas::chain_free_drain();
        vmas::fn_unregister(W->fn);
        vmas::fn_unregister(W->fn_prog);
        if (W->mod) (void)hipModuleUnload(W->mod);
        if (W->d_mask) (void)hipFree(W->d_mask);
        if (W->d_blk) (void)hipFree(W->d_blk);
        if (W->d_viol) (void)hipFree(W->d_viol);
        if (W->h_viol) (void)hipHostFree(W->h_viol);
        if (W->d_prof) (void)hipFree(W->d_prof);
        if (W->d_rows) (void)hipFree(W->d_rows);
        if (W->d_ctl) (void)hipFree(W->d_ctl);
        if (W->d_err) (void)hipFree(W->d_err);
        if (W->h_err) (void)hipHostFree(W->h_err);
        for (auto& ev : W->ev_pending) { (void)hipEventDestroy(ev.first); (void)hipEventDestroy(ev.second); }
        for (auto& ev : W->ev_free) { (void)hipEventDestroy(ev.first); (void)hipEventDestroy(ev.second); }
        if (W->d_tm) (void)hipFree(W->d_tm);
    }
    delete W;
    return VMAS_OK;
}

int32_t vmas_jit_world_create(const VmasWorldConfig* cfg, const VmasEntityDesc* entities, const VmasPairDesc* pairs,
                              const VmasJointDesc* joints, VmasJitWorld** out_world) {
    if (!cfg || !out_world) return jfail(VMAS_E_INVALID, "null argument");
    if (cfg->device < 0) return jfail(VMAS_E_INVALID, "the specialised step is a GPU path (device >= 0)");
    if (cfg->batch <= 0 || cfg->n_entities <= 0 || cfg->n_pairs < 0 || cfg->max_substeps <= 0)
        return jfail(VMAS_E_INVALID, "bad world config");
    auto* W = new VmasJitWorld();
    W->cfg = *cfg;
    W->ed.assign(entities, entities + cfg->n_entities);
    W->pd.assign(pairs, pairs + cfg->n_pairs);
    if (cfg->n_joints) W->jd.assign(joints, joints + cfg->n_joints);
    for (const auto& q : W->pd)
        if (q.ea < 0 || q.ea >= cfg->n_entities || q.eb < 0 || q.eb >= cfg->n_entities || q.cls < 0 || q.cls > 6 ||
            (q.cls == VMAS_PAIR_JOINT && (q.joint < 0 || q.joint >= cfg->n_joints))) {
            delete W;
            return jfail(VMAS_E_INVALID, "bad pair table");
        }
    auto cleanup = [&](int32_t rc) {
        vmas_jit_world_destroy(W);
        return rc;
    };
    JHIP(hipSetDevice(cfg->device));
    std::string why;
    std::unique_ptr<Gen> gp;
    for (int force_nw : {0, kNW}) {
        gp = make_plan(W->cfg, W->ed, W->pd, W->jd, &why, force_nw);
        if (!gp) {
            delete W;
            return jfail(VMAS_E_INVALID, "world not specialised: %s", why.c_str());
        }
        Gen& g = *gp;
        if (const char* pb = getenv("VMAS_JIT_PROFILE")) g.prof_block = std::max(0, atoi(pb));
        g.relaxed = relaxed_math(W->cfg);
        g.generate();
        std::vector<char> code;
        if (int32_t rc = compile(g.src, &code)) return cleanup(rc);
        if (W->mod) {
            W->fn = nullptr;
            (void)hipModuleUnload(W->mod);
            W->mod = nullptr;
        }
        if (hipModuleLoadData(&W->mod, code.data()) != hipSuccess)
            return cleanup(jfail(VMAS_E_HIP, "hipModuleLoadData"));
        if (hipModuleGetFunction(&W->fn, W->mod, "k_world") != hipSuccess)
            return cleanup(jfail(VMAS_E_HIP, "hipModuleGetFunction"));
        int scratch = 0;
        (void)hipFuncGetAttribute(&scratch, HIP_FUNC_ATTRIBUTE_LOCAL_SIZE_BYTES, W->fn);
        if (scratch == 0 || g.nw == kNW) break;
    }
    Gen& g = *gp;
    W->src = g.src;
    W->ptr_src = g.ptr_src;
    W->str_src = g.str_src;
    W->prm_src = g.prm_src;
    W->arg_bytes = g.arg_bytes();
    W->W = g.W;
    W->nw = g.nw;
    W->nblk = (cfg->batch + 63) / 64;
    if (g.has_epi()) {
        if (hipModuleGetFunction(&W->fn_prog, W->mod, "k_program_jit") != hipSuccess)
            return cleanup(jfail(VMAS_E_HIP, "hipModuleGetFunction(k_program_jit)"));
        W->epi_offset = g.epi_offset();
    }
    {
        vmas::JitFnInfo info{};
        info.kind = vmas::kJitFnWorld;
        info.world = W;
        info.world_fn = W->fn;
        info.arg_bytes = W->arg_bytes;
        info.epi_offset = W->fn_prog ? (long)W->epi_offset : -1L;
        info.wbd_offset = (long)g.wbd_offset();
        info.tail_offset = g.tail ? (long)g.tail_offset() : -1L;
        info.batch = cfg->batch;
        info.epilogue = g.has_epi() ? cfg->epilogue : VMAS_EPILOGUE_NONE;
        info.io_bytes = cfg->epilogue == VMAS_EPILOGUE_BALANCE ? sizeof(VmasBalanceIO)
                        : cfg->epilogue == VMAS_EPILOGUE_TRANSPORT ? sizeof(VmasTransportIO) : 0;
        vmas::fn_register(W->fn, info);
        if (W->fn_prog) {
            info.kind = vmas::kJitFnProgram;
            vmas::fn_register(W->fn_prog, info);
        }
    }
    const size_t nwords = (size_t)cfg->max_substeps * W->W;
    if (hipMalloc((void**)&W->d_mask, nwords * 4) != hipSuccess ||
        hipMalloc((void**)&W->d_blk, (size_t)W->nblk * 2 * nwords * 4) != hipSuccess ||
        hipMalloc((void**)&W->d_viol, 4) != hipSuccess ||
        hipHostMalloc((void**)&W->h_viol, 4, hipHostMallocDefault) != hipSuccess)
        return cleanup(jfail(VMAS_E_NOMEM, "hipMalloc broadphase scratch"));
    const size_t ctl_words = vmas::kGridCtlWords + (size_t)vmas::grid_claim_offset((long)nwords) +
                             (size_t)W->nblk * vmas::kClaimStride;
    if (hipMalloc((void**)&W->d_ctl, ctl_words * 4) != hipSuccess || hipMalloc((void**)&W->d_err, 4) != hipSuccess ||
        hipHostMalloc((void**)&W->h_err, 4, hipHostMallocMapped | hipHostMallocCoherent) != hipSuccess ||
        hipHostGetDevicePointer((void**)&W->dh_err, W->h_err, 0) != hipSuccess ||
        hipMemset(W->d_err, 0, 4) != hipSuccess ||
        hipMemset(W->d_ctl, 0, ctl_words * 4) != hipSuccess)
        return cleanup(jfail(VMAS_E_NOMEM, "hipMalloc fixed-point control words"));
    *W->h_err = 0u;
    if (hipMalloc((void**)&W->d_tm, 8 * 8) != hipSuccess || hipMemset(W->d_tm, 0, 8 * 8) != hipSuccess ||
        hipDeviceGetAttribute(&W->wall_khz, hipDeviceAttributeWallClockRate, cfg->device) != hipSuccess ||
        W->wall_khz <= 0)
        return cleanup(jfail(VMAS_E_HIP, "device timer (hipMalloc / wall clock rate)"));
    {
        const char* gm = getenv("VMAS_JIT_GRID");
        const std::string mode = gm ? gm : "persistent";
        int per_cu = 0, cus = 0;
        if (mode != "host" &&
            hipModuleOccupancyMaxActiveBlocksPerMultiprocessor(&per_cu, W->fn, W->nw * 64, 0) == hipSuccess &&
            hipDeviceGetAttribute(&cus, hipDeviceAttributeMultiprocessorCount, cfg->device) == hipSuccess &&
            per_cu > 0 && cus > 0) {
            W->grid = std::min(W->nblk, per_cu * cus);
            if (const char* cap = getenv("VMAS_JIT_GRID_CAP")) W->grid = std::max(1, std::min(W->grid, atoi(cap)));
            if (const char* r = getenv("VMAS_JIT_MAX_PASSES")) W->max_passes = std::max(1, atoi(r));
        }
    }
    W->global_rows = g.global_rows;
    if (g.global_rows) {
        const size_t slab = (size_t)std::max(W->nblk, W->grid) * (size_t)std::max(g.n_rows, 1) * 64 * 4;
        if (hipMalloc((void**)&W->d_rows, slab) != hipSuccess) return cleanup(jfail(VMAS_E_NOMEM, "hipMalloc row slabs"));
    }
    if (g.prof_block >= 0) {
        W->n_prof = ((size_t)cfg->max_substeps * 4 + 2) * kMaxNW + (size_t)kProfBlocks * kProfRec;
        if (hipMalloc((void**)&W->d_prof, W->n_prof * 8) != hipSuccess ||
            hipMemset(W->d_prof, 0, W->n_prof * 8) != hipSuccess)
            return cleanup(jfail(VMAS_E_NOMEM, "hipMalloc profile buffer"));
    }
    *out_world = W;
    return VMAS_OK;
}

int32_t vmas_jit_world_profile(VmasJitWorld* W, uint64_t* out, int64_t cap) {
    if (!W) return jfail(VMAS_E_INVALID, "null world");
    if (!W->d_prof) return 0;
    JHIP(hipSetDevice(W->cfg.device));
    JHIP(hipDeviceSynchronize());
    const size_t n = std::min<size_t>(W->n_prof, cap > 0 ? (size_t)cap : 0);
    if (out && n) JHIP(hipMemcpy(out, W->d_prof, n * 8, hipMemcpyDeviceToHost));
    return (int32_t)W->n_prof;
}

int32_t vmas_jit_compile_check(const VmasWorldConfig* cfg, const VmasEntityDesc* entities, const VmasPairDesc* pairs,
                               const VmasJointDesc* joints, char* buf, int64_t cap) {
    if (!cfg || cfg->n_entities <= 0 || cfg->max_substeps <= 0) return jfail(VMAS_E_INVALID, "bad world config");
    std::vector<VmasEntityDesc> ed(entities, entities + cfg->n_entities);
    std::vector<VmasPairDesc> pd(pairs, pairs + cfg->n_pairs);
    std::vector<VmasJointDesc> jd;
    if (cfg->n_joints) jd.assign(joints, joints + cfg->n_joints);
    std::string why;
    std::unique_ptr<Gen> gp = make_plan(*cfg, ed, pd, jd, &why);
    if (!gp) return jfail(VMAS_E_INVALID, "world not specialised: %s", why.c_str());
    Gen& g = *gp;
    g.relaxed = relaxed_math(*cfg);
    g.generate();
    std::vector<char> code;
    if (int32_t rc = compile(g.src, &code)) return rc;
    if (buf && cap > 0) {
        const size_t k = std::min<size_t>(g.src.size(), (size_t)cap - 1);
        memcpy(buf, g.src.data(), k);
        buf[k] = '\0';
    }
    return (int32_t)g.src.size();
}

int32_t vmas_jit_world_source(const VmasJitWorld* W, char* buf, int64_t cap) {
    if (!W) return jfail(VMAS_E_INVALID, "null world");
    const int64_t n = (int64_t)W->src.size();
    if (buf && cap > 0) {
        const int64_t k = std::min(n, cap - 1);
        memcpy(buf, W->src.data(), (size_t)k);
        buf[k] = '\0';
    }
    return (int32_t)std::min<int64_t>(n, INT32_MAX);
}

int32_t vmas_jit_world_step(VmasJitWorld* W, const VmasStepIO* io, void* stream_, int32_t* iterations) {
    if (!W || !io) return jfail(VMAS_E_INVALID, "null argument");
    const VmasWorldConfig& cfg = W->cfg;
    if (io->substeps <= 0 || io->substeps > cfg.max_substeps)
        return jfail(VMAS_E_INVALID, "substeps %d outside [1, %d]", io->substeps, cfg.max_substeps);
    int cur = -1;
    JHIP(hipGetDevice(&cur));
    if (cur != cfg.device) JHIP(hipSetDevice(cfg.device));
    hipStream_t stream = (hipStream_t)stream_;
    std::vector<char> buf(W->arg_bytes, 0);
    char* p = buf.data();
    auto put_ptr = [&](const void* v) {
        memcpy(p, &v, 8);
        p += 8;
    };
    auto put_i32 = [&](int32_t v) {
        memcpy(p, &v, 4);
        p += 4;
    };
    for (const auto& s : W->ptr_src) {
        const int i = s.second;
        const VmasEntityIO* e = io->entities + (s.first <= S_GRAV ? i : 0);
        switch (s.first) {
            case S_POS: put_ptr(e->pos); break;
            case S_VEL: put_ptr(e->vel); break;
            case S_ROT: put_ptr(e->rot); break;
            case S_ANG: put_ptr(e->ang_vel); break;
            case S_GRAV: put_ptr(e->gravity); break;
            case S_FORCE: put_ptr(io->agents[i].force); break;
            case S_TORQUE: put_ptr(io->agents[i].torque); break;
            default: put_ptr(io->joints ? io->joints[i].fixed_rotation : nullptr); break;
        }
    }
    if (W->ptr_src.empty()) put_ptr(nullptr);
    put_ptr(io->out_pos);
    put_ptr(io->out_vel);
    put_ptr(io->out_rot);
    put_ptr(io->out_ang_vel);
    put_ptr(io->out_force);
    put_ptr(io->out_torque);
    if (W->cfg.export_forces) {
        put_ptr(io->out_fdict);
        put_ptr(io->out_tdict);
    }
    const bool batch_bp = io->broadphase == VMAS_BROADPHASE_BATCH;
    const bool persistent = batch_bp && W->grid > 0;
    uint32_t* nmask = persistent ? W->d_ctl + vmas::kGridCtlWords : W->d_mask;
    put_ptr(nmask);
    put_ptr(batch_bp ? W->d_blk : nullptr);
    put_ptr(W->d_prof);
    put_ptr(persistent ? W->d_ctl : nullptr);
    put_ptr(W->d_err);
// ... 248 lines not shown
```

### vectorizedmultiagentsimulator_amd/csrc/vmas_jit_ops.hpp

```cpp
#pragma once

#include "vmas_physics.hpp"
#include "vmas_tail.hpp"

namespace vmas {


#ifndef __HIP_MEMORY_SCOPE_AGENT
#define __HIP_MEMORY_SCOPE_AGENT 4
#endif

constexpr uint32_t kGridErrNoConverge = 2u, kGridErrStateTimeout = 4u;
constexpr unsigned long long kGridStartWaitTicks = 1000000000ull;

constexpr int kGridMaxPasses = 64, kGridShards = 32;
constexpr int kGridEpoch = 32, kGridStartBase = 64, kGridCand = 96, kGridTop = 128, kGridDone = 160;
constexpr int kGridDec = kGridDone + 32 * kGridShards;
constexpr int kGridStart = kGridDec + 2 * kGridMaxPasses;
constexpr int kGridCtlWords = kGridStart + 32 * kGridShards;
static_assert(kGridCtlWords % 32 == 0, "mask words start on a 128-byte line");

__host__ __device__ constexpr long grid_claim_offset(long mask_words) { return (mask_words + 31) / 32 * 32; }

typedef unsigned long long u64;
__device__ __forceinline__ u64 ld64(const uint32_t* p) {
    return __hip_atomic_load(reinterpret_cast<const u64*>(p), __ATOMIC_RELAXED, __HIP_MEMORY_SCOPE_AGENT);
}
__device__ __forceinline__ void st64(uint32_t* p, u64 v) {
    __hip_atomic_store(reinterpret_cast<u64*>(p), v, __ATOMIC_RELAXED, __HIP_MEMORY_SCOPE_AGENT);
}
__device__ __forceinline__ u64 add64(uint32_t* p, u64 v) {
    return __hip_atomic_fetch_add(reinterpret_cast<u64*>(p), v, __ATOMIC_RELAXED, __HIP_MEMORY_SCOPE_AGENT);
}
__device__ __forceinline__ bool cas64(uint32_t* p, u64 expect, u64 v) {
    return __hip_atomic_compare_exchange_strong(reinterpret_cast<u64*>(p), &expect, v, __ATOMIC_RELAXED,
                                                __ATOMIC_RELAXED, __HIP_MEMORY_SCOPE_AGENT);
}

__device__ __forceinline__ bool grid_arrive(uint32_t* ctl, uint32_t g, uint32_t ngrp, u64 G) {
    const uint32_t k = g % kGridShards, n_k = (ngrp + kGridShards - 1u - k) / kGridShards;
    const uint32_t n_top = ngrp < (uint32_t)kGridShards ? ngrp : (uint32_t)kGridShards;
    if (add64(&ctl[kGridDone + 32 * k], 1ull) != (u64)n_k * (G + 1ull) - 1ull) return false;
    return add64(&ctl[kGridTop], 1ull) == (u64)n_top * (G + 1ull) - 1ull;
}

__device__ __forceinline__ uint32_t ld_agent(const uint32_t* p) {
    return __hip_atomic_load(p, __ATOMIC_RELAXED, __HIP_MEMORY_SCOPE_AGENT);
}
__device__ __forceinline__ void st_agent(uint32_t* p, uint32_t v) {
    __hip_atomic_store(p, v, __ATOMIC_RELAXED, __HIP_MEMORY_SCOPE_AGENT);
}
__device__ __forceinline__ uint32_t add_agent(uint32_t* p, uint32_t v) {
    return __hip_atomic_fetch_add(p, v, __ATOMIC_RELAXED, __HIP_MEMORY_SCOPE_AGENT);
}
__device__ __forceinline__ bool cas_agent(uint32_t* p, uint32_t expect, uint32_t v) {
    return __hip_atomic_compare_exchange_strong(p, &expect, v, __ATOMIC_RELAXED, __ATOMIC_RELAXED,
                                                __HIP_MEMORY_SCOPE_AGENT);
}
__device__ __forceinline__ void st_out1(float* p, size_t i, float v) {
    __hip_atomic_store(reinterpret_cast<uint32_t*>(p) + i, __float_as_uint(v), __ATOMIC_RELAXED, __HIP_MEMORY_SCOPE_AGENT);
}
__device__ __forceinline__ void st_out2(float* p, size_t i, V2 v) {
    const unsigned long long bits = (unsigned long long)__float_as_uint(v.x) | ((unsigned long long)__float_as_uint(v.y) << 32);
    __hip_atomic_store(reinterpret_cast<unsigned long long*>(p) + i, bits, __ATOMIC_RELAXED, __HIP_MEMORY_SCOPE_AGENT);
}

struct TimerStart {
    unsigned long long rt, sc;
};
__device__ __forceinline__ TimerStart device_timer_start(unsigned long long* tm, bool stamp_start) {
    TimerStart t{0ull, 0ull};
    if (tm && threadIdx.x == 0) {
        t.rt = __builtin_amdgcn_s_memrealtime();
        t.sc = __builtin_amdgcn_s_memtime();
        if (stamp_start && blockIdx.x == 0)
            __hip_atomic_store(&tm[0], t.rt, __ATOMIC_RELAXED, __HIP_MEMORY_SCOPE_AGENT);
    }
    return t;
}

__device__ __forceinline__ void report_err(uint32_t* err, uint32_t* herr, uint32_t bit) {
    const uint32_t v = atomicOr(err, bit) | bit;
    if (herr) __hip_atomic_store(herr, v, __ATOMIC_RELAXED, __HIP_MEMORY_SCOPE_SYSTEM);
}

constexpr int kClaimStride = 32;

__device__ __forceinline__ bool grid_claim(uint32_t* claim, int g, u64 G) {
    return cas64(&claim[(size_t)g * kClaimStride], G, G + 1ull);
}

__device__ __forceinline__ int grid_steal(uint32_t* claim, int ngrp, u64 G, uint32_t* LIST, bool* seen) {
    if (threadIdx.x == 0) LIST[64] = 0u;
    __syncthreads();
    for (int g = (int)threadIdx.x; g < ngrp; g += (int)blockDim.x) {
        uint32_t* w = &claim[(size_t)g * kClaimStride];
        if (ld64(w) != G) continue;
        const uint32_t i = atomicAdd(&LIST[64], 1u);
        if (i < 64u) LIST[i] = cas64(w, G, G + 1ull) ? (uint32_t)g : ~0u;
    }
    __syncthreads();
    const uint32_t r = LIST[64];
    __syncthreads();
    *seen = r != 0u;
    return r < 64u ? (int)r : 64;
}

__device__ __forceinline__ void grid_started(uint32_t* ctl) {
    __builtin_amdgcn_s_waitcnt(0);
    (void)add64(&ctl[kGridStart + 32 * (int)(blockIdx.x % kGridShards)], 1ull);
}

__device__ __forceinline__ u64 grid_starts(const uint32_t* ctl) {
    const uint32_t nsh = gridDim.x < (uint32_t)kGridShards ? gridDim.x : (uint32_t)kGridShards;
    u64 v = threadIdx.x < nsh ? ld64(&ctl[kGridStart + 32 * (int)threadIdx.x]) : 0ull;
    for (int off = 16; off > 0; off >>= 1) v += __shfl_xor(v, off, 64);
    return __shfl(v, 0, 64);
}

__device__ __forceinline__ bool grid_complete(uint32_t* ctl, int g, int ngrp, u64 G, uint32_t* FLAG) {
    __builtin_amdgcn_s_waitcnt(0);
    __syncthreads();
    if (threadIdx.x == 0) *FLAG = grid_arrive(ctl, (uint32_t)g, (uint32_t)ngrp, G) ? 1u : 0u;
    __syncthreads();
    const bool last = *FLAG != 0u;
    __syncthreads();
    return last;
}

__device__ __forceinline__ void grid_time(unsigned long long* tm, TimerStart t0s) {
    const unsigned long long t1 = __builtin_amdgcn_s_memrealtime();
    const unsigned long long c1 = __builtin_amdgcn_s_memtime();
    const unsigned long long t0 = __hip_atomic_load(&tm[0], __ATOMIC_RELAXED, __HIP_MEMORY_SCOPE_AGENT);
    (void)__hip_atomic_fetch_add(&tm[2], t1 > t0 ? t1 - t0 : 0ull, __ATOMIC_RELAXED, __HIP_MEMORY_SCOPE_AGENT);
    (void)__hip_atomic_fetch_add(&tm[4], 1ull, __ATOMIC_RELAXED, __HIP_MEMORY_SCOPE_AGENT);
    if (c1 > t0s.sc && t1 > t0s.rt) {
        (void)__hip_atomic_fetch_add(&tm[5], c1 - t0s.sc, __ATOMIC_RELAXED, __HIP_MEMORY_SCOPE_AGENT);
        (void)__hip_atomic_fetch_add(&tm[6], t1 - t0s.rt, __ATOMIC_RELAXED, __HIP_MEMORY_SCOPE_AGENT);
    }
}

struct GridCursor {
    int pass, own, nl, il, started;
    u64 base;
    int fin;
};

#ifndef VMAS_GRID_MIN_PASSES
#define VMAS_GRID_MIN_PASSES 1
#endif

__device__ inline bool grid_decide(const uint32_t* blk, uint32_t* nmask, const uint32_t* MSK, uint32_t* ctl, uint32_t* err,
                                   uint32_t* herr, int nwords, int ngrp, u64 G, int pass, int max_pass, uint32_t* RED,
                                   unsigned long long* tm, TimerStart t0s, GridCursor* CUR) {
    const int nw2 = 2 * nwords;
    const bool force = pass + 1 < VMAS_GRID_MIN_PASSES;
    if (threadIdx.x == 0) RED[nw2] = (force || ld64(&ctl[kGridCand]) == G + 1ull) ? 1u : 0u;
    for (int w = threadIdx.x; w < nw2; w += blockDim.x) RED[w] = 0u;
    if (threadIdx.x == 0) RED[nw2 + 1] = 0u;
    __syncthreads();
    if (RED[nw2] != 0u) {
        const int rows = ngrp, t = (int)threadIdx.x;
        if (nw2 <= (int)blockDim.x) {
            const int per = (int)blockDim.x / nw2, w = t % nw2, g0 = t / nw2;
            if (g0 < per) {
                uint32_t r0 = 0u, r1 = 0u, r2 = 0u, r3 = 0u;
                int i = g0;
                for (; i + 3 * per < rows; i += 4 * per) {
                    r0 |= ld_agent(&blk[(size_t)i * nw2 + w]);
                    r1 |= ld_agent(&blk[(size_t)(i + per) * nw2 + w]);
                    r2 |= ld_agent(&blk[(size_t)(i + 2 * per) * nw2 + w]);
                    r3 |= ld_agent(&blk[(size_t)(i + 3 * per) * nw2 + w]);
                }
                for (; i < rows; i += per) r0 |= ld_agent(&blk[(size_t)i * nw2 + w]);
                const uint32_t r = r0 | r1 | r2 | r3;
                if (r) atomicOr(&RED[w], r);
            }
        } else {
            for (int w = t; w < nw2; w += blockDim.x) {
                uint32_t r = 0u;
                for (int i = 0; i < rows; ++i) r |= ld_agent(&blk[(size_t)i * nw2 + w]);
                RED[w] = r;
            }
        }
        __syncthreads();
        for (int w = threadIdx.x; w < nwords; w += blockDim.x) {
            const uint32_t m = MSK[w], r = RED[w], z = RED[nwords + w];
            if ((m & ~r & z) | (~m & r)) atomicOr(&RED[nw2 + 1], 1u);
        }
    }
    __syncthreads();
    const bool viol = RED[nw2 + 1] != 0u || force;
    const bool more = viol && pass + 1 < max_pass;
    if (more)
        for (int w = threadIdx.x; w < nwords; w += blockDim.x) st_agent(&nmask[w], ~RED[w]);
    __builtin_amdgcn_s_waitcnt(0);
    __syncthreads();
    if (threadIdx.x == 0) {
        if (viol && !more) report_err(err, herr, kGridErrNoConverge);
        if (!more) st_agent(&ctl[2], (uint32_t)(pass + 1));
        st64(&ctl[kGridDec + 2 * (int)(G % (u64)kGridMaxPasses)], ((G + 1ull) << 1) | (more ? 1ull : 0ull));
    }
    if (!more) {
        const bool self = CUR->started != 0;
        if (threadIdx.x < 64) {
            const u64 base = ld64(&ctl[kGridStartBase]);
            const u64 want = base + (u64)gridDim.x - (self ? 0ull : 1ull);
            const unsigned long long t0 = __builtin_amdgcn_s_memrealtime();
            bool late = false;
            while (grid_starts(ctl) != want) {
                if (__builtin_amdgcn_s_memrealtime() - t0 > kGridStartWaitTicks) {
                    late = true;
                    break;
                }
                __builtin_amdgcn_s_sleep(8);
            }
            if (threadIdx.x == 0) {
                st64(&ctl[kGridStartBase], base + (u64)gridDim.x);
                RED[nw2 + 1] = late ? 2u : (viol ? 1u : 0u);
            }
        }
        if (threadIdx.x == 0) {
            if (RED[nw2 + 1] == 2u) report_err(err, herr, kGridErrStateTimeout);
            st64(&ctl[kGridEpoch], G + 1ull);
            if (!self) {
                grid_started(ctl);
                CUR->started = 1;
            }
            CUR->fin = 1;
            if (tm) grid_time(tm, t0s);
        }
        __syncthreads();
        if (pass > 0)
            for (int w = threadIdx.x; w < nwords; w += blockDim.x) st_agent(&nmask[w], 0u);
    }
    __syncthreads();
    return RED[nw2 + 1] == 2u || (viol && !more);
}

__device__ __forceinline__ bool grid_wait(uint32_t* ctl, u64 G, uint32_t* FLAG, int* started) {
    if (threadIdx.x == 0) {
        if (!*started) grid_started(ctl);
        const uint32_t* dec = &ctl[kGridDec + 2 * (int)(G % (u64)kGridMaxPasses)];
        u64 d;
        while (((d = ld64(dec)) >> 1) != G + 1ull) __builtin_amdgcn_s_sleep(4);
        *FLAG = (uint32_t)(d & 1ull);
    }
    *started = 1;
    __syncthreads();
    const bool more = *FLAG != 0u;
    __syncthreads();
    return more;
}

#ifdef VMAS_JIT_PROFILE_SLOTS
__device__ unsigned long long* vmas_prof_blk;
#endif

__device__ __attribute__((noinline)) int grid_next(bool persistent, uint32_t* ctl, uint32_t* claim, const uint32_t* mask,
                                                   uint32_t* MSK, int nwords, int ngrp, GridCursor* CUR, uint32_t* QL) {
    GridCursor c = *CUR;
    int g = -1;
    if (c.fin) return g;
    for (;;) {
        if (c.own < ngrp) {
            const int own = c.own;
            c.own += (int)gridDim.x;
            if (!persistent) {
                g = own;
                break;
            }
#ifdef VMAS_JIT_PROFILE_SLOTS
            if (threadIdx.x == 0 && blockIdx.x < 4096u) vmas_prof_blk[blockIdx.x * 24 + 6] = __builtin_amdgcn_s_memrealtime();
#endif
            if (threadIdx.x == 0) QL[65] = grid_claim(claim, own, c.base + (u64)c.pass) ? 1u : 0u;
#ifdef VMAS_JIT_PROFILE_SLOTS
            if (threadIdx.x == 0 && blockIdx.x < 4096u) vmas_prof_blk[blockIdx.x * 24 + 7] = __builtin_amdgcn_s_memrealtime();
#endif
            __syncthreads();
            const bool mine = QL[65] != 0u;
            __syncthreads();
            if (mine) {
                g = own;
                break;
            }
        } else if (!persistent) {
            break;
        } else if (c.il < c.nl) {
            const uint32_t q = QL[c.il++];
            if (q != ~0u) {
                g = (int)q;
                break;
            }
        } else {
            bool seen;
            c.nl = grid_steal(claim, ngrp, c.base + (u64)c.pass, QL, &seen);
            c.il = 0;
            if (seen) continue;
            if (!grid_wait(ctl, c.base + (u64)c.pass, &QL[65], &c.started)) break;
            ++c.pass;
            c.own = (int)blockIdx.x;
            c.nl = c.il = 0;
            for (int i = threadIdx.x; i < nwords; i += blockDim.x) MSK[i] = ~ld_agent(&mask[i]);
        }
    }
    __syncthreads();
    if (threadIdx.x == 0) *CUR = c;
    __syncthreads();
    return g;
}

__device__ __attribute__((noinline)) bool grid_finish(int g, const uint32_t* FL, int nfl, uint32_t* blk, uint32_t* nmask,
                                                      const uint32_t* MSK, uint32_t* ctl, uint32_t* err, uint32_t* herr,
                                                      int nwords, int ngrp, GridCursor* CUR, int max_pass,
                                                      uint32_t* RED, uint32_t* FLAG, unsigned long long* tm,
                                                      unsigned long long t0_rt, unsigned long long t0_sc) {
    const TimerStart t0s{t0_rt, t0_sc};
    __syncthreads();
    const int pass = CUR->pass;
    const u64 G = CUR->base + (u64)pass;
    for (int i = threadIdx.x; i < nfl; i += blockDim.x) st_agent(&blk[(size_t)g * nfl + i], FL[i]);
    for (int w = threadIdx.x; w < nwords; w += blockDim.x) {
        const uint32_t m = MSK[w], r = FL[w], z = FL[nwords + w];
        if ((m & ~r & z) | (~m & r))
            (void)__hip_atomic_fetch_max(reinterpret_cast<u64*>(&ctl[kGridCand]), G + 1ull, __ATOMIC_RELAXED,
                                         __HIP_MEMORY_SCOPE_AGENT);
    }
    return grid_complete(ctl, g, ngrp, G, FLAG) &&
           grid_decide(blk, nmask, MSK, ctl, err, herr, nwords, ngrp, G, pass, max_pass, RED, tm, t0s, CUR);
}

}
```

### vectorizedmultiagentsimulator_amd/csrc/vmas_jit_registry.hpp

```cpp
#pragma once

#include <hip/hip_runtime.h>

#include <cstddef>

namespace vmas {

constexpr int kJitFnWorld = 0;
constexpr int kJitFnProgram = 1;

struct JitFnInfo {
    int kind;
    const void* world;
    hipFunction_t world_fn;
    size_t arg_bytes;
    long epi_offset;
    long wbd_offset;
    long tail_offset;
    int batch;
    int epilogue;
    size_t io_bytes;
};

bool jit_fn_info(const void* f, JitFnInfo* out);

void chain_free_drain();

}
```

### vectorizedmultiagentsimulator_amd/csrc/vmas_kernels.hip

```cpp
#include <hip/hip_runtime.h>

#include <algorithm>
#include <atomic>
#include <cstdarg>
#include <condition_variable>
#include <cstdio>
#include <cstdlib>
#include <cstring>
#include <functional>
#include <memory>
#include <mutex>
#include <string>
#include <thread>
#include <vector>

#include "vmas_aux.hpp"
#include "vmas_physics.hpp"
#include "vmas_query.hpp"
#include "vmas_jit_registry.hpp"
#include "vmas_tail.hpp"
#include "vmas_uniform.hpp"

using namespace vmas;

// ... 706 lines not shown
    std::vector<uint32_t> mask(nwords, 0xFFFFFFFFu);
    const bool batch_bp = io.broadphase == VMAS_BROADPHASE_BATCH;
    Pool& pool = Pool::get();
    const int nchunks = std::min(B, pool.size() * 4);
    const int per = (B + nchunks - 1) / nchunks;
    std::vector<uint32_t> RZ((size_t)nchunks * 2 * nwords);
    const int max_it = S + 2;
    for (int it = 0; it < max_it; ++it) {
        std::fill(RZ.begin(), RZ.end(), 0u);
        pool.run(nchunks, [&](int c) {
            std::vector<float> scratch;
            uint32_t* R = batch_bp ? &RZ[(size_t)c * 2 * nwords] : nullptr;
            uint32_t* Z = batch_bp ? R + nwords : nullptr;
            const int b0 = c * per, b1 = std::min(B, b0 + per);
            for (int b = b0; b < b1; ++b) host_step_env(W, io, mask.data(), R, Z, b, scratch);
        });
        if (iterations) *iterations = it + 1;
        if (!batch_bp) return VMAS_OK;
        std::vector<uint32_t> Rt(nwords, 0u), Zt(nwords, 0u);
        for (int c = 0; c < nchunks; ++c)
            for (int w = 0; w < nwords; ++w) {
                Rt[w] |= RZ[(size_t)c * 2 * nwords + w];
                Zt[w] |= RZ[(size_t)c * 2 * nwords + nwords + w];
            }
        bool viol = false;
        for (int w = 0; w < nwords; ++w)
            if ((mask[w] & ~Rt[w] & Zt[w]) | (~mask[w] & Rt[w])) viol = true;
        if (!viol) return VMAS_OK;
        mask = Rt;
    }
    return fail(VMAS_E_NOCONVERGE, "broadphase fixed point did not converge");
}

struct RayK {
    const VmasRayTarget* tg;
    int nt, B, R;
    const float* origin;
    int o_s0, o_s1;
    const float* ang;
    int a_s0, a_s1;
    const float* rot;
    int r_s0;
    float max_range;
    float* out;
};

__global__ void __launch_bounds__(256) k_cast_rays(RayK k) {
    const long idx = (long)blockIdx.x * blockDim.x + threadIdx.x;
    if (idx >= (long)k.B * k.R) return;
    const int b = (int)(idx / k.R), r = (int)(idx - (long)b * k.R);
    const V2 o = mk(k.origin[(long)b * k.o_s0], k.origin[(long)b * k.o_s0 + k.o_s1]);
    float a = k.ang[(long)b * k.a_s0 + (long)r * k.a_s1];
    if (k.rot) a = a + k.rot[(long)b * k.r_s0];
    k.out[idx] = cast_one(k.tg, k.nt, o, a, b, k.max_range);
}

__global__ void __launch_bounds__(256) k_distance(int B, int kind, VmasShapeRef a, VmasShapeRef bref,
                                                  const float* tp, int tp_s0, int tp_s1, void* out) {
    const int b = blockIdx.x * blockDim.x + threadIdx.x;
    if (b >= B) return;
    store_query(out, kind, b, distance_query(kind, a, bref, tp, tp_s0, tp_s1, b));
}

__global__ void __launch_bounds__(256) k_check_actions(const VmasActionRef* refs, int B, uint32_t* flags) {
    const VmasActionRef r = refs[blockIdx.y];
    uint32_t nan_seen = 0u, out_of_range = 0u;
    const long n = (long)B * r.n_cols;
    for (long idx = (long)blockIdx.x * blockDim.x + threadIdx.x; idx < n; idx += (long)gridDim.x * blockDim.x) {
        const int b = (int)(idx / r.n_cols), c = (int)(idx - (long)b * r.n_cols);
        const float x = r.u[(long)b * r.s0 + (long)c * r.s1];
        nan_seen |= (x != x);
        if (c < r.n_phys && !r.clamp) out_of_range |= (fabsf(x) > r.u_range[c]);
    }
    if (__any(nan_seen) && (threadIdx.x & 63) == 0) atomicOr(&flags[2 * blockIdx.y], 1u);
    if (__any(out_of_range) && (threadIdx.x & 63) == 0) atomicOr(&flags[2 * blockIdx.y + 1], 1u);
}

namespace {
struct CheckScratch {
    int device = -1;
    uint32_t* d_flags = nullptr;
    uint32_t* h_flags = nullptr;
};
std::mutex g_check_mu;
std::vector<CheckScratch*> g_checks;
}

constexpr int kChainMaxNodes = VMAS_GRAPH_CHAIN_MAX;

extern "C" {

int32_t vmas_abi_version(void) { return VMAS_ABI_VERSION; }

int32_t vmas_device_count(void) {
    int n = 0;
    if (hipGetDeviceCount(&n) != hipSuccess) return 0;
    return n;
}

const char* vmas_last_error(void) { return g_err.c_str(); }

int32_t vmas_stream_abort_capture(void* stream_) {
    hipStream_t stream = (hipStream_t)stream_;
    hipStreamCaptureStatus st = hipStreamCaptureStatusNone;
    if (hipStreamIsCapturing(stream, &st) != hipSuccess) {
        (void)hipGetLastError();
        return 0;
    }
    int32_t ended = 0;
    if (st != hipStreamCaptureStatusNone) {
        hipGraph_t g = nullptr;
        (void)hipStreamEndCapture(stream, &g);
        if (g) (void)hipGraphDestroy(g);
        ended = 1;
    }
    (void)hipGetLastError();
    return ended;
}

int32_t vmas_graph_launch(void* graph_exec, void* stream) {
    if (!graph_exec) return fail(VMAS_E_INVALID, "vmas_graph_launch: null graph");
    const hipError_t e = hipGraphLaunch((hipGraphExec_t)graph_exec, (hipStream_t)stream);
    if (e != hipSuccess) {
        (void)hipGetLastError();
        return fail(VMAS_E_HIP, "vmas_graph_launch: %s", hipGetErrorString(e));
    }
    return VMAS_OK;
}

struct ChainNode {
    hipFunction_t fn;
    dim3 grid, block;
    unsigned shmem;
    void** kernel_params;
    void** extra;
};
struct FusedArgs {
    std::vector<char> buf;
    size_t size = 0;
    void* extra[5];
};
struct VmasKernelChain {
    int n = 0, fused = 0;
    ChainNode node[kChainMaxNodes];
    std::vector<std::unique_ptr<FusedArgs>> args;
    std::vector<void*> dev;
    int world = -1;
    const char* world_args = nullptr;
    vmas::JitFnInfo world_info{};
    std::unique_ptr<FusedArgs> wb;
    mutable std::vector<char> tail_buf;
    mutable size_t tail_size = 0;
    mutable void* tail_extra[5] = {nullptr, nullptr, nullptr, nullptr, nullptr};
};

namespace {
std::mutex g_chain_free_mu;
std::vector<void*> g_chain_free;
}

extern "C++" {
namespace vmas {
void chain_free_drain() {
    std::lock_guard<std::mutex> lk(g_chain_free_mu);
    for (void* d : g_chain_free) (void)hipFree(d);
    g_chain_free.clear();
}
}
}

namespace {

const char* node_arg_block(const hipKernelNodeParams& p, size_t expect) {
    if (p.extra) {
        const void* buf = nullptr;
        size_t sz = 0;
        for (int i = 0; i < 8 && p.extra[i] != HIP_LAUNCH_PARAM_END; i += 2) {
            if (p.extra[i] == HIP_LAUNCH_PARAM_BUFFER_POINTER) buf = p.extra[i + 1];
            else if (p.extra[i] == HIP_LAUNCH_PARAM_BUFFER_SIZE) sz = *(const size_t*)p.extra[i + 1];
            else return nullptr;
        }
        return buf && sz >= expect ? (const char*)buf : nullptr;
    }
    return p.kernelParams && p.kernelParams[0] ? (const char*)p.kernelParams[0] : nullptr;
}

bool balance_io_fusable(const VmasBalanceIO& io, int batch) {
    if (io.batch != batch || io.n_agents < 0 || io.n_agents > VMAS_SCN_MAX_AGENTS) return false;
    if (io.package.shape != VMAS_SPHERE || io.goal.shape != VMAS_SPHERE || io.line.shape != VMAS_LINE ||
        io.floor.shape != VMAS_BOX)
        return false;
    for (const VmasShapeRef* r : {&io.package, &io.goal, &io.line, &io.floor})
        if (!r->pos || r->pos_s0 == 0 || (r->rot && r->rot_s0 == 0)) return false;
    if ((io.what & VMAS_SCN_REWARD) && io.gs_s0 == 0) return false;
    if (io.what & VMAS_SCN_OBS) {
        for (const VmasVec* v : {&io.package_vel, &io.line_vel, &io.line_ang_vel})
            if (!v->p || v->s0 == 0) return false;
        for (int i = 0; i < io.n_agents; ++i)
            if (!io.agent_pos[i].p || io.agent_pos[i].s0 == 0 || !io.agent_vel[i].p || io.agent_vel[i].s0 == 0)
                return false;
    }
    return true;
}
bool transport_io_fusable(const VmasTransportIO& io, int batch) {
    if (io.batch != batch || io.n_agents < 0 || io.n_agents > VMAS_TRANSPORT_MAX_AGENTS || io.n_packages < 0 ||
        io.n_packages > VMAS_TRANSPORT_MAX_PACKAGES)
        return false;
    for (int i = 0; i < io.n_packages; ++i) {
        for (const VmasShapeRef* r : {&io.package[i], &io.goal[i]})
            if (!r->pos || r->pos_s0 == 0 || (r->rot && r->rot_s0 == 0)) return false;
        if (io.package[i].shape != VMAS_BOX || io.goal[i].shape != VMAS_SPHERE) return false;
        if ((io.what & VMAS_SCN_REWARD) && io.gs_s0[i] == 0) return false;
        if ((io.what & VMAS_SCN_OBS) && (!io.package_vel[i].p || io.package_vel[i].s0 == 0)) return false;
    }
    if (io.what & VMAS_SCN_OBS)
        for (int i = 0; i < io.n_agents; ++i)
            if (!io.agent_pos[i].p || io.agent_pos[i].s0 == 0 || !io.agent_vel[i].p || io.agent_vel[i].s0 == 0)
                return false;
    return true;
}
bool program_io_fusable(int kind, const char* io, int batch) {
    if (kind == VMAS_EPILOGUE_BALANCE) {
        VmasBalanceIO x;
        memcpy(&x, io, sizeof x);
        return balance_io_fusable(x, batch);
    }
    if (kind == VMAS_EPILOGUE_TRANSPORT) {
        VmasTransportIO x;
        memcpy(&x, io, sizeof x);
        return transport_io_fusable(x, batch);
    }
    return false;
}
}

int32_t vmas_graph_chain_build(void* graph_, int32_t max_nodes, VmasKernelChain** out) {
    if (!graph_ || !out) return fail(VMAS_E_INVALID, "vmas_graph_chain_build: null argument");
    *out = nullptr;
    vmas::chain_free_drain();
    const hipGraph_t graph = (hipGraph_t)graph_;
    max_nodes = std::min<int32_t>(max_nodes, kChainMaxNodes);
    size_t n = 0;
    if (hipGraphGetNodes(graph, nullptr, &n) != hipSuccess) {
        (void)hipGetLastError();
        return fail(VMAS_E_HIP, "vmas_graph_chain_build: hipGraphGetNodes");
    }
    if (n == 0 || (int64_t)n > max_nodes) return fail(VMAS_E_UNSUPPORTED, "graph of %zu nodes (chain: 1..%d)", n, max_nodes);
    std::vector<hipGraphNode_t> nodes(n);
    if (hipGraphGetNodes(graph, nodes.data(), &n) != hipSuccess) {
        (void)hipGetLastError();
        return fail(VMAS_E_HIP, "vmas_graph_chain_build: hipGraphGetNodes");
    }
    std::vector<hipGraphNode_t> dep(n, nullptr);
    int root = -1;
    for (size_t i = 0; i < n; ++i) {
        hipGraphNodeType t;
        if (hipGraphNodeGetType(nodes[i], &t) != hipSuccess || t != hipGraphNodeTypeKernel) {
            (void)hipGetLastError();
            return fail(VMAS_E_UNSUPPORTED, "graph node %zu is not a kernel node", i);
        }
        size_t nd = 0;
        if (hipGraphNodeGetDependencies(nodes[i], nullptr, &nd) != hipSuccess) {
            (void)hipGetLastError();
            return fail(VMAS_E_HIP, "hipGraphNodeGetDependencies");
        }
        if (nd > 1) return fail(VMAS_E_UNSUPPORTED, "graph node %zu has %zu dependencies", i, nd);
        if (nd == 1) {
            if (hipGraphNodeGetDependencies(nodes[i], &dep[i], &nd) != hipSuccess) {
                (void)hipGetLastError();
                return fail(VMAS_E_HIP, "hipGraphNodeGetDependencies");
            }
        } else {
            if (root >= 0) return fail(VMAS_E_UNSUPPORTED, "graph has more than one root");
            root = (int)i;
        }
    }
    if (root < 0) return fail(VMAS_E_UNSUPPORTED, "graph has no root");
    std::vector<hipKernelNodeParams> prm(n);
    std::vector<hipFunction_t> fns(n);
    std::vector<char> used(n, 0);
    int cur = root;
    for (size_t k = 0; k < n; ++k) {
        if (cur < 0 || used[cur]) return fail(VMAS_E_UNSUPPORTED, "graph is not a chain");
        used[cur] = 1;
        hipKernelNodeParams p{};
        if (hipGraphKernelNodeGetParams(nodes[cur], &p) != hipSuccess) {
            (void)hipGetLastError();
            return fail(VMAS_E_HIP, "hipGraphKernelNodeGetParams");
        }
        if (!p.func || (!p.kernelParams && !p.extra)) return fail(VMAS_E_UNSUPPORTED, "kernel node without function / arguments");
        hipFunction_t f = nullptr;
        if (hipGetFuncBySymbol(&f, p.func) != hipSuccess || !f) {
            (void)hipGetLastError();
            if (!vmas::jit_fn_info(p.func, nullptr)) return fail(VMAS_E_UNSUPPORTED, "kernel node %d: unknown function", (int)k);
            f = (hipFunction_t)p.func;
        }
        prm[k] = p;
        fns[k] = f;
        int next = -1;
        for (size_t i = 0; i < n; ++i)
            if (dep[i] == nodes[cur]) {
                if (next >= 0) return fail(VMAS_E_UNSUPPORTED, "graph node has two dependents");
                next = (int)i;
            }
        if (k + 1 < n && next < 0) return fail(VMAS_E_UNSUPPORTED, "graph is not a chain");
        cur = next;
    }
    std::unique_ptr<VmasKernelChain> c(new VmasKernelChain());
    const char* fz = getenv("VMAS_GRAPH_FUSE");
    const bool fuse = !(fz && fz[0] == '0');
    for (size_t k = 0; k < n; ++k) {
        const hipKernelNodeParams& p = prm[k];
        ChainNode nd{fns[k], p.gridDim, p.blockDim, p.sharedMemBytes, p.kernelParams, p.extra};
        vmas::JitFnInfo a{}, b{};
        if (fuse && k + 1 < n && vmas::jit_fn_info(p.func, &a) && a.kind == vmas::kJitFnWorld && a.epi_offset >= 0 &&
            vmas::jit_fn_info(prm[k + 1].func, &b) && b.kind == vmas::kJitFnProgram && b.world == a.world) {
            const char* wa = node_arg_block(p, a.arg_bytes);
            const char* io = node_arg_block(prm[k + 1], b.io_bytes);
            if (wa && io && program_io_fusable(a.epilogue, io, a.batch)) {
                void* d = nullptr;
                if (hipMalloc(&d, b.io_bytes) != hipSuccess || hipMemcpy(d, io, b.io_bytes, hipMemcpyHostToDevice) != hipSuccess) {
                    (void)hipGetLastError();
                    if (d) (void)hipFree(d);
                    for (void* x : c->dev) (void)hipFree(x);
                    return fail(VMAS_E_HIP, "vmas_graph_chain_build: epilogue argument copy");
                }
                c->dev.push_back(d);
                std::unique_ptr<FusedArgs> fa(new FusedArgs());
                fa->buf.assign(wa, wa + a.arg_bytes);
                memcpy(fa->buf.data() + a.epi_offset, &d, sizeof d);
                fa->size = a.arg_bytes;
                fa->extra[0] = HIP_LAUNCH_PARAM_BUFFER_POINTER;
                fa->extra[1] = fa->buf.data();
                fa->extra[2] = HIP_LAUNCH_PARAM_BUFFER_SIZE;
                fa->extra[3] = &fa->size;
                fa->extra[4] = HIP_LAUNCH_PARAM_END;
                nd.fn = a.world_fn;
                nd.kernel_params = nullptr;
                nd.extra = fa->extra;
                if (c->world < 0) {
                    c->world = c->n;
                    c->world_args = fa->buf.data();
                    c->world_info = a;
                }
                c->args.push_back(std::move(fa));
                c->node[c->n++] = nd;
                ++c->fused;
                ++k;
                continue;
            }
        }
        if (c->world < 0 && vmas::jit_fn_info(p.func, &a) && a.kind == vmas::kJitFnWorld) {
            const char* wa = node_arg_block(p, a.arg_bytes);
            if (wa) {
                c->world = c->n;
                c->world_args = wa;
                c->world_info = a;
            }
        }
        c->node[c->n++] = nd;
    }
    *out = c.release();
    return VMAS_OK;
}

int32_t vmas_graph_chain_set_writeback(VmasKernelChain* c, int64_t backup_delta) {
    if (!c) return fail(VMAS_E_INVALID, "vmas_graph_chain_set_writeback: null chain");
    if (backup_delta == 0) {
        c->wb.reset();
        return VMAS_OK;
    }
    if (c->world < 0 || !c->world_args || c->world_info.wbd_offset <= 0 ||
        (size_t)c->world_info.wbd_offset + 8 > c->world_info.arg_bytes)
        return fail(VMAS_E_UNSUPPORTED, "vmas_graph_chain_set_writeback: the chain has no k_world launch");
    std::unique_ptr<FusedArgs> fa(new FusedArgs());
    fa->buf.assign(c->world_args, c->world_args + c->world_info.arg_bytes);
    memcpy(fa->buf.data() + c->world_info.wbd_offset, &backup_delta, sizeof backup_delta);
    fa->size = c->world_info.arg_bytes;
    fa->extra[0] = HIP_LAUNCH_PARAM_BUFFER_POINTER;
    fa->extra[1] = fa->buf.data();
    fa->extra[2] = HIP_LAUNCH_PARAM_BUFFER_SIZE;
    fa->extra[3] = &fa->size;
    fa->extra[4] = HIP_LAUNCH_PARAM_END;
    c->wb = std::move(fa);
    return VMAS_OK;
}

static int32_t chain_launch(const VmasKernelChain* c, void* stream, bool wb) {
    if (!c || c->n <= 0) return fail(VMAS_E_INVALID, "vmas_graph_chain_launch: empty chain");
    if (wb && !c->wb) return fail(VMAS_E_INVALID, "vmas_graph_chain_launch_wb: no write-back variant");
    for (int k = 0; k < c->n; ++k) {
        const ChainNode& d = c->node[k];
        const bool w = wb && k == c->world;
        const hipError_t e = hipModuleLaunchKernel(d.fn, d.grid.x, d.grid.y, d.grid.z, d.block.x, d.block.y, d.block.z,
                                                   d.shmem, (hipStream_t)stream, w ? nullptr : d.kernel_params,
                                                   w ? c->wb->extra : d.extra);
        if (e != hipSuccess) {
            (void)hipGetLastError();
            return fail(VMAS_E_HIP, "vmas_graph_chain_launch: node %d: %s", k, hipGetErrorString(e));
        }
    }
    return VMAS_OK;
}

int32_t vmas_graph_chain_launch(const VmasKernelChain* c, void* stream) { return chain_launch(c, stream, false); }

int32_t vmas_graph_chain_launch_wb(const VmasKernelChain* c, void* stream) { return chain_launch(c, stream, true); }

int32_t vmas_graph_chain_launch_tail(const VmasKernelChain* c, int32_t wb, const VmasCopySpan* spans, int32_t n_spans,
                                     int64_t numel, const VmasUniformColumn* cols, int32_t n_cols, uint64_t seed,
                                     uint64_t offset, const uint64_t* offset_dev, int32_t mode, int64_t u_snap_delta,
                                     uint64_t* increment, void* stream) {
    if (!c || !increment || n_spans < 0 || (n_spans > 0 && !spans) || n_cols < 0 || (n_cols > 0 && !cols) || mode < 0 ||
        mode > 3)
        return fail(VMAS_E_INVALID, "vmas_graph_chain_launch_tail: bad arguments");
    *increment = 0;
    static const bool off = getenv("VMAS_GRAPH_TAIL") && getenv("VMAS_GRAPH_TAIL")[0] == '0';
    const vmas::JitFnInfo& a = c->world_info;
    if (off || c->n != 1 || c->world != 0 || c->fused != 1 || c->args.empty() || a.tail_offset <= 0 ||
        (size_t)a.tail_offset + sizeof(VmasTail) > a.arg_bytes || n_cols > kTailCols || (wb && !c->wb))
        return 0;
    VmasTail t;
    memset(&t, 0, sizeof t);
    static const char* diag = getenv("VMAS_TAIL_DIAG");
    const bool no_copy = diag && strcmp(diag, "nocopy") == 0, no_draw = diag && strcmp(diag, "nodraw") == 0;
    if (no_draw) n_cols = 0;
    int n = 0;
    for (int i = 0; i < n_spans; ++i) {
        const VmasCopySpan& sp = spans[i];
        if (sp.nbytes == 0 || (sp.nbytes > 0 && sp.src == sp.dst)) continue;
        if (no_copy && sp.src && sp.nbytes != VMAS_COPY_STORE64) continue;
        if (sp.nbytes == VMAS_COPY_STORE64) {
            if (!sp.dst || ((uintptr_t)sp.dst & 7)) return 0;
        } else if (sp.nbytes < 0 || !sp.dst || (((uintptr_t)sp.src | (uintptr_t)sp.dst | (uintptr_t)sp.nbytes) & 3)) {
            return 0;
        }
        if (n == kTailSpans) return 0;
        t.s[n++] = sp;
    }
    int gx = 0;
    unsigned long long inc = 0;
    if (n_cols > 0) {
        if (numel <= 0) return fail(VMAS_E_INVALID, "vmas_graph_chain_launch_tail: numel %lld", (long long)numel);
        int dev = 0;
        if (hipGetDevice(&dev) != hipSuccess || dev < 0 || dev >= 64) {
            (void)hipGetLastError();
            return fail(VMAS_E_HIP, "vmas_graph_chain_launch_tail: device");
        }
        static int max_blocks[64] = {0};
        if (!max_blocks[dev]) {
            hipDeviceProp_t prop;
            if (hipGetDeviceProperties(&prop, dev) != hipSuccess) {
                (void)hipGetLastError();
                return fail(VMAS_E_HIP, "vmas_graph_chain_launch_tail: device properties");
            }
            max_blocks[dev] = prop.multiProcessorCount * (prop.maxThreadsPerMultiProcessor / vmas_uniform::kThreads);
        }
        vmas_uniform::grid_for(numel, max_blocks[dev], &gx, &inc);
    }
    for (int i = 0; i < n_cols; ++i) {
        if (!cols[i].out) return fail(VMAS_E_INVALID, "vmas_graph_chain_launch_tail: null column %d", i);
        t.c[i] = cols[i];
        t.c[i].offset = offset + inc * (unsigned long long)i;
    }
    t.seed = seed;
    t.numel = numel;
    t.snap = u_snap_delta;
    t.off_dev = reinterpret_cast<const unsigned long long*>(offset_dev);
    t.n_spans = n;
    t.gx_draw = gx;
    t.mode = mode;
    t.n_items = n + n_cols;
    if (t.n_items == 0) return 0;
    int64_t total = 0;
    for (int y = 0; y < n; ++y) {
        t.first[y] = (int)total;
        const VmasCopySpan& sp = t.s[y];
        const bool w8 = sp.src && ((((uintptr_t)sp.src | (uintptr_t)sp.dst | (uintptr_t)sp.nbytes) & 7) == 0);
        total += sp.nbytes == VMAS_COPY_STORE64 ? 1 : sp.nbytes / (w8 ? 8 : 4);
    }
    for (int y = n; y < n + n_cols; ++y) {
        t.first[y] = (int)total;
        total += numel;
    }
    if (total >= (int64_t)1 << 30) return 0;
    t.first[n + n_cols] = (int)total;
    const FusedArgs* base = wb ? c->wb.get() : c->args.front().get();
    c->tail_buf.assign(base->buf.begin(), base->buf.begin() + a.arg_bytes);
    memcpy(c->tail_buf.data() + a.tail_offset, &t, sizeof t);
    c->tail_size = a.arg_bytes;
    c->tail_extra[0] = HIP_LAUNCH_PARAM_BUFFER_POINTER;
    c->tail_extra[1] = c->tail_buf.data();
    c->tail_extra[2] = HIP_LAUNCH_PARAM_BUFFER_SIZE;
    c->tail_extra[3] = &c->tail_size;
    c->tail_extra[4] = HIP_LAUNCH_PARAM_END;
    const ChainNode& d = c->node[0];
    const hipError_t e = hipModuleLaunchKernel(d.fn, d.grid.x, d.grid.y, d.grid.z, d.block.x, d.block.y, d.block.z,
                                               d.shmem, (hipStream_t)stream, nullptr, c->tail_extra);
    if (e != hipSuccess) {
        (void)hipGetLastError();
        return fail(VMAS_E_HIP, "vmas_graph_chain_launch_tail: %s", hipGetErrorString(e));
    }
    *increment = inc * (unsigned long long)n_cols;
    return 1;
}

namespace {
__global__ void __launch_bounds__(256) k_test_tail(VmasTail t) { vmas_tail::run(t); }
}

int32_t vmas_test_tail_draw(int32_t device, const VmasUniformColumn* cols, int32_t n_cols, int64_t numel, uint64_t seed,
                            uint64_t offset, int32_t mode, uint64_t* increment, void* stream) {
    if (device < 0 || device >= 64 || !cols || n_cols < 1 || n_cols > kTailCols || numel <= 0 || !increment || mode < 0 ||
        mode > 3 || numel * n_cols >= ((int64_t)1 << 30))
        return fail(VMAS_E_INVALID, "vmas_test_tail_draw: bad arguments");
    HIP_TRY(hipSetDevice(device));
    hipDeviceProp_t prop;
    HIP_TRY(hipGetDeviceProperties(&prop, device));
    int gx = 0;
    unsigned long long inc = 0;
    vmas_uniform::grid_for(numel, prop.multiProcessorCount * (prop.maxThreadsPerMultiProcessor / vmas_uniform::kThreads),
                           &gx, &inc);
    VmasTail t;
    memset(&t, 0, sizeof t);
    for (int i = 0; i < n_cols; ++i) {
        t.c[i] = cols[i];
        t.c[i].offset = offset + inc * (unsigned long long)i;
        t.first[i] = (int)(numel * i);
    }
    t.first[n_cols] = (int)(numel * n_cols);
    t.seed = seed;
    t.numel = numel;
    t.gx_draw = gx;
    t.mode = mode;
    t.n_items = n_cols;
    hipLaunchKernelGGL(k_test_tail, dim3(512), dim3(256), 0, (hipStream_t)stream, t);
    HIP_TRY(hipGetLastError());
    *increment = inc * (unsigned long long)n_cols;
    return VMAS_OK;
}

int32_t vmas_graph_chain_nodes(const VmasKernelChain* c) { return c ? c->n : 0; }

int32_t vmas_graph_chain_fused(const VmasKernelChain* c) { return c ? c->fused : 0; }

int32_t vmas_graph_chain_free(VmasKernelChain* c) {
    if (c && !c->dev.empty()) {
        std::lock_guard<std::mutex> lk(g_chain_free_mu);
        g_chain_free.insert(g_chain_free.end(), c->dev.begin(), c->dev.end());
    }
    delete c;
    return VMAS_OK;
}

static size_t align_up(size_t x, size_t a) { return (x + a - 1) / a * a; }

int32_t vmas_world_create(const VmasWorldConfig* cfg, const VmasEntityDesc* entities,
                          const VmasPairDesc* pairs, const VmasJointDesc* joints,
                          VmasWorld** out_world) {
    if (!cfg || !out_world) return fail(VMAS_E_INVALID, "null argument");
    if (cfg->batch <= 0 || cfg->n_entities < 0 || cfg->n_pairs < 0 || cfg->n_agents < 0 ||
        cfg->n_joints < 0 || cfg->max_substeps <= 0)
        return fail(VMAS_E_INVALID, "bad world config");
    auto* W = new VmasWorld();
    W->cfg = *cfg;
    W->ed.assign(entities, entities + cfg->n_entities);
    W->pd.assign(pairs, pairs + cfg->n_pairs);
    if (cfg->n_joints) W->jd.assign(joints, joints + cfg->n_joints);
    const int E = cfg->n_entities, P = cfg->n_pairs;
    for (int p = 0; p < P; ++p) {
        const VmasPairDesc& pd = W->pd[p];
        if (pd.ea < 0 || pd.ea >= E || pd.eb < 0 || pd.eb >= E || pd.cls < 0 || pd.cls > 6 ||
            (pd.cls == VMAS_PAIR_JOINT && (pd.joint < 0 || pd.joint >= cfg->n_joints))) {
            delete W;
            return fail(VMAS_E_INVALID, "bad pair %d", p);
        }
    }
    W->trig_slot.assign(E, -1);
    auto need_trig = [&](int e) {
        if (W->trig_slot[e] < 0) W->trig_slot[e] = W->n_trig++;
    };
    for (int e = 0; e < E; ++e)
        if (W->ed[e].shape != VMAS_SPHERE) need_trig(e);
    for (int p = 0; p < P; ++p)
        if (W->pd[p].cls == VMAS_PAIR_JOINT) { need_trig(W->pd[p].ea); need_trig(W->pd[p].eb); }
    for (int e = 0; e < E; ++e)
        if (W->ed[e].flags & (VMAS_F_MOVABLE | VMAS_F_ROTATABLE)) W->dyn.push_back(e);
    W->items.resize(W->dyn.size());
    for (size_t i = 0; i < W->dyn.size(); ++i) {
        const int e = W->dyn[i];
        for (int p = 0; p < P; ++p) {
            const VmasPairDesc& pd = W->pd[p];
// ... 412 lines not shown
```

### vectorizedmultiagentsimulator_amd/csrc/vmas_tail.hpp

```cpp
#pragma once

#ifndef __HIPCC_RTC__
#include <stdint.h>
#endif

#include "../../include/vmas_mi355x.h"

constexpr int kTailSpans = 16, kTailCols = 12, kTailThreads = 256;

struct VmasTail {
    VmasCopySpan s[kTailSpans];
    VmasUniformColumn c[kTailCols];
    unsigned long long seed;
    long long numel, snap;
    const unsigned long long* off_dev;
    int n_spans, n_items, gx_draw, mode;
    int first[kTailSpans + kTailCols + 1];
    int pad;
};

#if defined(__HIPCC__) || defined(__HIPCC_RTC__)
namespace vmas_tail {

__device__ __forceinline__ uint4 philox10(uint4 c, uint2 k) {
#pragma unroll
    for (int r = 0; r < 10; ++r) {
        const unsigned long long p0 = (unsigned long long)c.x * 0xD2511F53u;
        const unsigned long long p1 = (unsigned long long)c.z * 0xCD9E8D57u;
        const unsigned int hi0 = (unsigned int)(p0 >> 32), lo0 = (unsigned int)p0;
        const unsigned int hi1 = (unsigned int)(p1 >> 32), lo1 = (unsigned int)p1;
        c = make_uint4(hi1 ^ c.y ^ k.x, lo1, hi0 ^ c.w ^ k.y, lo0);
        k.x += 0x9E3779B9u;
        k.y += 0xBB67AE85u;
    }
    return c;
}

struct Unit {
    int kind;
    float x, u;
    unsigned long long v;
    void* dst;
    float* out;
    float* uo;
};

__device__ __forceinline__ void prep_draw(const VmasTail& t, const VmasUniformColumn& col, long long li, Unit& w) {
    const long long step = (long long)kTailThreads * t.gx_draw;
    const long long q = li / step, idx = li - q * step;
    const unsigned long long off = col.offset + (t.off_dev ? *t.off_dev : 0ull);
    const unsigned long long c = off / 4 + (unsigned long long)(q / 4);
    const int k = (int)(q % 4) + (int)(off & 3ull);
    const uint2 key = make_uint2((unsigned int)t.seed, (unsigned int)(t.seed >> 32));
    const unsigned int ilo = (unsigned int)idx, ihi = (unsigned int)((unsigned long long)idx >> 32);
    const unsigned long long cc = c + (k >= 4 ? 1ull : 0ull);
    const uint4 v = philox10(make_uint4((unsigned int)cc, (unsigned int)(cc >> 32), ilo, ihi), key);
    const int kk = k & 3;
    const unsigned int bits = kk == 0 ? v.x : kk == 1 ? v.y : kk == 2 ? v.z : v.w;
    const float inv = 2.3283064e-10f;
    const float u01 = (t.mode & 1) ? __builtin_fmaf((float)bits, inv, inv) : inv + (float)bits * inv;
    const float from = col.from, to = col.to, range = to - from;
    const float val = (t.mode & 2) ? __builtin_fmaf(u01, range, from) : u01 * range + from;
    w.kind = 1;
    w.x = val == to ? from : val;
    w.out = col.out + li * col.stride;
    w.uo = nullptr;
    if (col.u_out) {
        w.u = (col.u_clamp ? fminf(fmaxf(w.x, -col.u_range), col.u_range) : w.x) * col.u_mult;
        w.uo = col.u_out + li * col.u_stride;
        if (t.snap) w.v = __float_as_uint(*w.uo);
    }
}

__device__ __forceinline__ void prep(const VmasTail& t, long long u, Unit& w) {
    w.kind = 0;
    if (u >= (long long)t.first[t.n_items]) return;
    int lo = 0, hi = t.n_items - 1;
    while (lo < hi) {
        const int mid = (lo + hi + 1) >> 1;
        if ((long long)t.first[mid] <= u) lo = mid;
        else hi = mid - 1;
    }
    const long long i = u - t.first[lo];
    if (lo >= t.n_spans) {
        prep_draw(t, t.c[lo - t.n_spans], i, w);
        return;
    }
    const VmasCopySpan& s = t.s[lo];
    if (s.nbytes == VMAS_COPY_STORE64) {
        w.kind = 5;
        w.dst = s.dst;
        w.v = (unsigned long long)s.src;
    } else if (!s.src) {
        w.kind = 4;
        w.dst = reinterpret_cast<float*>(s.dst) + i;
        w.x = *reinterpret_cast<const float*>(w.dst);
    } else if ((((unsigned long long)s.src | (unsigned long long)s.dst | (unsigned long long)s.nbytes) & 7) == 0) {
        w.kind = 2;
        w.dst = reinterpret_cast<unsigned long long*>(s.dst) + i;
        w.v = __hip_atomic_load(reinterpret_cast<const unsigned long long*>(s.src) + i, __ATOMIC_RELAXED,
                                __HIP_MEMORY_SCOPE_AGENT);
    } else {
        w.kind = 3;
        w.dst = reinterpret_cast<uint32_t*>(s.dst) + i;
        w.v = __hip_atomic_load(reinterpret_cast<const uint32_t*>(s.src) + i, __ATOMIC_RELAXED, __HIP_MEMORY_SCOPE_AGENT);
    }
}

__device__ __forceinline__ void finish(const VmasTail& t, const Unit& w) {
    switch (w.kind) {
        case 1:
            *w.out = w.x;
            if (w.uo) {
                if (t.snap) *reinterpret_cast<uint32_t*>(reinterpret_cast<char*>(w.uo) + t.snap) = (uint32_t)w.v;
                *w.uo = w.u;
            }
            break;
        case 2: *reinterpret_cast<unsigned long long*>(w.dst) = w.v; break;
        case 3: *reinterpret_cast<uint32_t*>(w.dst) = (uint32_t)w.v; break;
        case 4: *reinterpret_cast<float*>(w.dst) = w.x + 1.0f; break;
        case 5: *reinterpret_cast<unsigned long long*>(w.dst) = w.v; break;
        default: break;
    }
}

__device__ __forceinline__ void run(const VmasTail& t) {
    const long long T = (long long)gridDim.x * blockDim.x, total = t.first[t.n_items];
    for (long long u = (long long)blockIdx.x * blockDim.x + threadIdx.x; u < total; u += 2 * T) {
        Unit a, b;
        prep(t, u, a);
        prep(t, u + T, b);
        finish(t, a);
        finish(t, b);
    }
}

}
#endif
```

### vectorizedmultiagentsimulator_amd/simulator/environment/_post.py

```python
from __future__ import annotations

import operator
from typing import Any, Dict, List, NamedTuple, Optional, Tuple

import numpy as np
import torch
from torch import Tensor

from ... import _native as N

_VERSION = operator.attrgetter("_version")


class PostTable:

    __slots__ = (
        "tbl", "addr",
        "n_out", "n_all",
        "plain",
        "clash",
        "n_bk",
        "steps_row", "steps",
        "direct_rows",
        "contig",
        "bk_dst", "bk_lens",
        "loose",
        "host",
        "tail_ok",
    )


class Covered(NamedTuple):

    carry_ver: tuple
    bk_ver: tuple
    bk_n: int


def _clone_plan(out_tensors: List[Tensor], out_tree, direct: List[dict]):
    ts = out_tensors
    dmember = {id(m): (ri, mi) for ri, r in enumerate(direct) for mi, m in enumerate(r["members"])}
    by_key: Dict[Tuple[torch.dtype, Tuple[int, ...]], List[int]] = {}
    for i, t in enumerate(ts):
        if id(t) not in dmember:
            by_key.setdefault((t.dtype, tuple(t.shape)), []).append(i)
    plan = sorted(by_key.items(), key=lambda kv: str(kv[0][0]))
    groups = [(dt, shape, len(idx)) for (dt, shape), idx in plan]
    order = [i for _, idx in plan for i in idx]
    pos = {i: p for p, i in enumerate(order)}
    base, at = [], len(order)
    for r in direct:
        base.append(at)
        at += len(r["members"])
    for i, t in enumerate(ts):
        if id(t) in dmember:
            ri, mi = dmember[id(t)]
            pos[i] = base[ri] + mi
    group_srcs, start = [], 0
    for _, idx in plan:
        group_srcs.append((start, start + len(idx), [ts[i] for i in idx]))
        start += len(idx)
    consts: List[Any] = []
    counter = [0]

    def expr(t):
        if isinstance(t, Tensor):
            counter[0] += 1
            return f"v[{pos[counter[0] - 1]}]"
        if isinstance(t, list):
            return "[" + ", ".join(expr(x) for x in t) + "]"
        if isinstance(t, tuple):
            return "(" + "".join(expr(x) + ", " for x in t) + ")"
        if isinstance(t, dict):
            items = []
            for k, x in t.items():
                consts.append(k)
                items.append(f"c[{len(consts) - 1}]: {expr(x)}")
            return "{" + ", ".join(items) + "}"
        consts.append(t)
        return f"c[{len(consts) - 1}]"

    fn = eval("lambda v, c: " + expr(out_tree))
    return groups, group_srcs, (fn, consts)


def _post_spans(carry_dst, carry_src, bk_src, bk_dst, state_idx: Optional[int], wb: bool = False):
    carry = [(y.data_ptr(), x.data_ptr(), x.numel()) for i, (x, y) in enumerate(zip(carry_dst, carry_src))
             if not (wb and i == state_idx)]
    bk = []
    n = len(bk_src) if bk_dst else 0
    for t, d in zip(bk_src[:n], bk_dst[:n]):
        if not (t.is_contiguous() and d.is_contiguous()):
            return carry, None, 0
        lo, nb = t.data_ptr(), t.numel() * t.element_size()
        src = lo
        for y, x, cn in carry:
            if lo < x + cn and x < lo + nb:
                if not (x <= lo and lo + nb <= x + cn):
                    return carry, None, 0
                src = y + (lo - x)
        bk.append((src, d.data_ptr(), nb))
    return carry, bk, n


def _post_table(group_srcs, carry_dst, carry_src, carry_other, bk_src, bk_dst, direct: List[dict],
                state_idx: Optional[int], steps: Optional[Tensor], wb: bool = False) -> PostTable:
    out_rows = [(x.data_ptr(), 0, x.numel() * x.element_size()) for _, _, srcs in group_srcs
                for x in srcs if x.is_contiguous()]
    direct_rows = []
    for r in direct:
        direct_rows.append(len(out_rows))
        out_rows.append((0, r["word"], N.VMAS_COPY_STORE64))
    steps_row = None
    if steps is not None:
        steps_row = len(out_rows)
        out_rows.append((0, steps.data_ptr(), steps.numel() * 4))
    carry, bk, n_bk = _post_spans(carry_dst, carry_src, bk_src, bk_dst, state_idx, wb)
    plain = bool(carry_other) or bk is None
    extra = [] if plain else carry + bk
    tbl = np.zeros(len(out_rows) + len(extra), dtype=N.COPY_SPAN_DTYPE)
    for i, row in enumerate(out_rows + extra):
        tbl[i] = row
    t = PostTable()
    t.tbl, t.addr = tbl, tbl.ctypes.data
    t.n_out, t.n_all = len(out_rows), len(tbl)
    t.plain, t.n_bk = plain, n_bk
    t.clash = any(lo < x + cn and x < lo + nb for lo, _, nb in out_rows if nb > 0 for _, x, cn in carry)
    t.steps_row, t.steps = steps_row, steps
    t.direct_rows = direct_rows
    t.contig = [[x.is_contiguous() for x in srcs] for _, _, srcs in group_srcs]
    t.loose = [(start + k, x) for start, _, srcs in group_srcs for k, x in enumerate(srcs) if not x.is_contiguous()]
    t.bk_dst, t.bk_lens = bk_dst, (len(bk_dst), len(bk_src))
    t.host = t.tail_ok = None
    return t


def _steps_current(t: PostTable, st: Tensor) -> None:
    if t.steps is not st:
        row = t.tbl[t.steps_row]
        row["dst"] = st.data_ptr()
        row["nbytes"] = st.numel() * 4
        t.steps = st


def _ahead_offset_word(deferred):
    if len(deferred) != 1:
        return None if deferred else 0
    mx = getattr(getattr(deferred[0], "chan", None), "mx", None)
    return None if mx is None else mx.data_ptr() + 4 * N.VMAS_SPAWN_OFF_END_WORD


class PostStage:

    def __init__(self, *, env, dev_index: int, out_tree, out_tensors, carry_dst, carry_src, carry_other,
                 carry_ys, inplace, state_idx: Optional[int], direct: List[dict], steps_folded: bool,
                 deferred=(), tail: bool = False):
        self.env, self.dev = env, dev_index
        self.carry_dst, self.carry_src, self.carry_other = carry_dst, carry_src, carry_other
        self.carry_ys, self.inplace = carry_ys, inplace
        self.state_idx, self.steps_folded = state_idx, steps_folded
        self.direct = direct
        self.off_dev = _ahead_offset_word(deferred)
        self.tail = tail
        self.bk_src, self.bk_dst = [], []
        self.clone_groups, self.clone_group_srcs, self.clone_build = _clone_plan(out_tensors, out_tree, direct)
        self.tbl: Optional[PostTable] = None
        self.tbl_wb: Optional[PostTable] = None
        self.covered: Optional[Covered] = None
        self._fns = None

    def invalidate(self) -> None:
        self.covered = None

    def set_backups(self, src: List[Tensor], dst: List[Tensor]) -> None:
        self.bk_src, self.bk_dst = src, dst
        self.covered = None

    def carry_current(self) -> bool:
        c = self.covered
        return c is not None and c.carry_ver == tuple(map(_VERSION, self.carry_ys))

    def backup_current(self, n: int) -> bool:
        c = self.covered
        return (c is not None and c.bk_n >= n and self.carry_current()
                and c.bk_ver == tuple(map(_VERSION, self.inplace)))

    def table(self, wb: bool = False) -> PostTable:
        t = self.tbl_wb if wb else self.tbl
        bk_dst = self.bk_dst
        if t is not None and t.bk_dst is bk_dst and t.bk_lens == (len(bk_dst), len(self.bk_src)):
            return t
        t = _post_table(self.clone_group_srcs, self.carry_dst, self.carry_src, self.carry_other, self.bk_src, bk_dst,
                        self.direct, self.state_idx, self.env.steps if self.steps_folded else None, wb)
        if wb:
            self.tbl_wb = t
        else:
            self.tbl = t
        return t

    def _ready(self, t: PostTable) -> PostTable:
        if t.steps_row is not None:
            _steps_current(t, self.env.steps)
        if t.host is None:
            self._host_alloc(t)
        return t

    def _host_alloc(self, t: PostTable) -> None:
        groups, row = [], 0
        for (dt, shape, n), (_, _, srcs), contig in zip(self.clone_groups, self.clone_group_srcs, t.contig):
            ks = [k for k, c in enumerate(contig) if c]
            groups.append((srcs[0], list(shape), n, row, ks))
            row += len(ks)
        regions = [(r["buf"], r["box"], r["members"][0], row,
                    [(list(m.shape), list(m.stride()), m.storage_offset()) for m in r["members"]])
                   for r, row in zip(self.direct, t.direct_rows)]
        t.host = N.load_host().OutputAlloc(self.dev, groups, t.tbl, t.addr, N.fn_addr("vmas_copy_spans"),
                                           N.fn_addr("vmas_aux_last_error"), regions)
        if self._fns is None:
            self._fns = (N.fn_addr("vmas_graph_chain_launch"), N.fn_addr("vmas_graph_chain_launch_wb"),
                         N.fn_addr("vmas_graph_chain_launch_tail"), N.fn_addr("vmas_copy_spans_draw"))

    def _tail_admit(self, t: PostTable, ch) -> bool:
        srcs = getattr(self.env.scenario, "_vmas_tail_sources", None)
        if not self.tail or ch.n_nodes != 1 or not ch.fused or srcs is None or t.plain:
            return False
        ranges = []
        try:
            tensors = list(srcs())
        except Exception:
            return False
        for v in tensors:
            if not isinstance(v, Tensor) or not v.is_contiguous() or v.device.type != "cuda":
                return False
            ranges.append((v.data_ptr(), v.data_ptr() + v.numel() * v.element_size()))
        if self.state_idx is not None:
            y = self.carry_src[self.state_idx]
            ranges.append((y.data_ptr(), y.data_ptr() + y.numel()))
        for r in t.tbl:
            n, src = int(r["nbytes"]), int(r["src"])
            if n == N.VMAS_COPY_STORE64 or src == 0 or n == 0:
                continue
            if not any(lo <= src and src + n <= hi for lo, hi in ranges):
                return False
        return True

    def prepare(self):
        t = self._ready(self.table())
        return t, t.host.alloc()

    def _copy(self, t: PostTable, views, hi: int):
        if views is None:
            views = t.host.alloc()
        dev, st, lo = self.dev, N.stream_ptr(self.dev), 0
        if t.clash and hi > t.n_out:
            N.copy_table_at(dev, t.addr, 0, t.n_out, st)
            lo = t.n_out
        N.copy_table_at(dev, t.addr, lo, hi, st)
        t.host.commit()
        return views

    def _finish(self, t: PostTable, views):
        for k, s in t.loose:
            views[k].copy_(s)
        fn, consts = self.clone_build
        return fn(views, consts)

    def run(self, prep=None, chain=None, wb: bool = False):
        t, views = prep if prep is not None else (self.table(wb), None)
        if chain is not None and (t.plain or t.host is None or views is not None):
            chain.launch(wb, N.stream_ptr(self.dev))
            chain = None
        self._ready(t)
        if views is not None or t.plain:
            views = self._copy(t, views, t.n_all)
        else:
            host, fns = t.host, self._fns
            ch = (chain.addr, fns[1 if wb else 0]) if chain is not None else (0, 0)
            mid, hi = (t.n_out if t.clash else 0), t.n_all
            off_dev, env = self.off_dev, self.env
            ahead = env._draw_ahead_plan() if (hi - mid <= 96 and not t.n_bk and off_dev is not None) else None
            if ahead is not None:
                st, drawer, P = ahead
                tail = 0
                if ch[0] and not mid:
                    ok = t.tail_ok
                    if ok is None:
                        ok = t.tail_ok = self._tail_admit(t, chain)
                    if ok:
                        tail = fns[2]
                views, acts, snap, seed, off, inc = N.load_host().post_draw(
                    host, drawer, mid, hi, P.data_ptr(), P.numel(), fns[3], off_dev, *ch, tail, int(wb))
                env._drew_ahead(st, acts, snap, seed, off, inc)
            else:
                views = host.post(mid, hi, *ch)
        self.covered = None if t.plain else Covered(tuple(map(_VERSION, self.carry_ys)),
                                                    tuple(map(_VERSION, self.inplace)), t.n_bk)
        return self._finish(t, views)

    def clone_outputs(self):
        t = self._ready(self.table())
        return self._finish(t, self._copy(t, None, t.n_out))
```

Measured before the change: 784.1 million env-steps/s.

## Copy per-group tail outputs as each group completes in persistent kernel

Adds a completion-first mode to the persistent JIT world kernel. Each workgroup records its finished groups, runs the epilogue and copies those groups' rows of scenario tail-source outputs (and per-group NaN poisoning) itself. This replaces having every block wait for the final decision and then run a bulk tail copy. The final deciding block is also skipped in the tail loop. The change adds progress words in the claim array, LDS usage and a host-side tail-source registration, and it raises the risk of ordering bugs.

Result: slower. 198.2 million env-steps/s (-74.7%).

```diff
diff --git a/include/vmas_mi355x.h b/include/vmas_mi355x.h
--- a/include/vmas_mi355x.h
+++ b/include/vmas_mi355x.h
@@ -552,6 +552,12 @@
                              const VmasUniformColumn* cols, int32_t n_cols, uint64_t seed, uint64_t offset,
                              const uint64_t* offset_dev, int32_t mode, int64_t u_snap_delta, uint64_t* increment,
                              void* stream);
+typedef struct VmasTailSource {
+    const void* base;
+    int64_t nbytes;
+    int64_t row_bytes;
+} VmasTailSource;
+int32_t vmas_graph_chain_set_tail_sources(VmasKernelChain* chain, const VmasTailSource* sources, int32_t n);
 int32_t vmas_graph_chain_launch_tail(const VmasKernelChain* chain, int32_t wb, const VmasCopySpan* spans,
                                      int32_t n_spans, int64_t numel, const VmasUniformColumn* cols, int32_t n_cols,
                                      uint64_t seed, uint64_t offset, const uint64_t* offset_dev, int32_t mode,
diff --git a/vectorizedmultiagentsimulator_amd/_native.py b/vectorizedmultiagentsimulator_amd/_native.py
--- a/vectorizedmultiagentsimulator_amd/_native.py
+++ b/vectorizedmultiagentsimulator_amd/_native.py
@@ -95,6 +95,7 @@
     "vmas_uniform_columns_snap",
     "vmas_copy_spans_draw",
     "vmas_graph_chain_launch_tail",
+    "vmas_graph_chain_set_tail_sources",
     "vmas_test_tail_draw",
     "vmas_assert_create",
     "vmas_assert_destroy",
@@ -293,6 +294,10 @@
 
 
 COPY_SPAN_DTYPE = np.dtype([("src", np.uint64), ("dst", np.uint64), ("nbytes", np.int64)])
+
+
+class VmasTailSource(ctypes.Structure):
+    _fields_ = [("base", _vp), ("nbytes", ctypes.c_int64), ("row_bytes", ctypes.c_int64)]
 VMAS_COPY_STORE64 = -8
 
 
@@ -841,6 +846,8 @@
     lib.vmas_graph_chain_launch_tail.restype = _i32
     lib.vmas_graph_chain_launch_tail.argtypes = [_vp, _i32, _vp, _i32, ctypes.c_int64, _vp, _i32, ctypes.c_uint64,
                                                  ctypes.c_uint64, _vp, _i32, ctypes.c_int64, _vp, _vp]
+    lib.vmas_graph_chain_set_tail_sources.restype = _i32
+    lib.vmas_graph_chain_set_tail_sources.argtypes = [_vp, _vp, _i32]
     lib.vmas_graph_chain_free.argtypes = [_vp]
     lib.vmas_world_create.restype = _i32
     lib.vmas_world_create.argtypes = [_vp, _vp, _vp, _vp, ctypes.POINTER(_vp)]
diff --git a/vectorizedmultiagentsimulator_amd/csrc/vmas_jit.hip b/vectorizedmultiagentsimulator_amd/csrc/vmas_jit.hip
--- a/vectorizedmultiagentsimulator_amd/csrc/vmas_jit.hip
+++ b/vectorizedmultiagentsimulator_amd/csrc/vmas_jit.hip
@@ -127,6 +127,8 @@
     int E, P, A, J, W, nfl;
     bool split_boxes = true;
     bool side_prune = true;
+    bool completion_first = true;
+    bool early() const { return has_epi() && completion_first; }
     bool splits(int cls) const {
         return split_boxes && (cls == VMAS_PAIR_BB || (cls == VMAS_PAIR_BL && !side_prune));
     }
@@ -280,7 +282,8 @@
         const long lds = (global_rows ? 0L : (long)n_rows * 256) + (long)nfl * 4 + 4 * (n_split + 1) +
                          4L * (nfl / 2) + 4 * red + (has_epi() && !epi_q_in_rows() ? (long)kEpiQRows * 256 : 0L) +
                          (has_epi() ? (long)(cfg.epilogue == VMAS_EPILOGUE_BALANCE ? sizeof(VmasBalanceIO)
-                                                                                   : sizeof(VmasTransportIO)) : 0L);
+                                                                                   : sizeof(VmasTransportIO)) : 0L) +
+                         (early() ? 4L * (vmas::kOwnList + 5) + 24L + 8L : 0L);
         if (lds > lds_budget) {
             *why = "LDS budget exceeded (" + it(lds) + " B)";
             return false;
@@ -807,7 +810,74 @@
                "            __syncthreads();\n"
                "        }\n";
     }
+    std::string loop_text_early() const {
+        const std::string fin = "grid_finish(g, FL, nfl, a.blk, a.mask, MSK, a.ctl, a.err, a.herr, nwords, ngrp, CURP,\n"
+                                "                                      a.max_pass, RED, &QL[65], a.tm, t0s.rt, t0s.sc, ";
+        return "    bool spec = persistent && spec_first, spec_ok = true, own = true;\n"
+               "    if (spec && threadIdx.x == 0) spec_ok = grid_claim(claim, (int)blockIdx.x, (CURP)->base);\n"
+               "    const bool early = persistent && a.epi != nullptr;\n"
+               "    for (;;) {\n"
+               "        const int g = spec ? (int)blockIdx.x : grid_next(persistent, a.ctl, claim, a.mask, MSK, nwords, ngrp, CURP, QL, &OWN[kOwnDwg]);\n"
+               "        if (g < 0) break;\n" + block_stamp(4, "__builtin_amdgcn_s_memrealtime()") +
+               "        if (persistent) {\n"
+               "            for (int i = threadIdx.x; i < nfl; i += blockDim.x) FL[i] = 0u;\n"
+               "            if (early) grid_enter(claim, g, CURP, OWN, a.err, a.herr);\n"
+               "            __syncthreads();\n"
+               "        }\n"
+               "        {\n"
+               "            const int b = g * 64 + lane;\n"
+               "            const bool valid = b < a.B;\n"
+               "            const int bb = valid ? b : (a.B - 1);\n"
+               "            // the state write-back (Args.wbd, wb_text): this pass's inputs, its backup\n"
+               "            const bool wbx = persistent && a.wbd != 0;\n"
+               "            const long long rbd = (wbx && (CURP)->pass > 0) ? a.wbd : 0ll;\n"
+               "            const bool bk = wbx && (CURP)->pass == 0;\n"
+               "            own = run<WAVE>(a, L, FL, DONE, MSK, lane, b, bb, valid, rbd, bk, wbx, spec, spec_ok, QL);\n"
+               "        }\n"
+               "        spec = false;\n"
+               "        if (!own) continue;\n"
+               "        const bool first = early && OWN[0] < (uint32_t)kOwnList;  // (completion before the program)\n"
+               "        bool bad = false;\n"
+               "        if (first) bad = " + fin + "true);\n" + epi_text() +
+               "        if (early) grid_listed(claim, g, CURP, OWN, first);\n"
+               "        if (persistent && !first) bad = " + fin + "false);\n"
+               "        // (completion-first: every workgroup poisons its own groups behind the decision, world_body)\n"
+               "        if (bad && !early) poison_outputs(a);\n" + block_stamp(5, "__builtin_amdgcn_s_memrealtime()") +
+               "    }\n";
+    }
+    std::string after_early() const {
+        const std::string tl = tail ? (tail_stage ? "TL" : "a.tail") : "";
+        const std::string rows = "            own_group(a, " + std::string(tail ? "nown > 0 ? &" + tl + " : nullptr" : "nullptr") + ", G_, bad);\n";
+        std::string o =
+            "    if (persistent && a.epi) {\n"
+            "        const bool bad = OWN[kOwnBad] != 0u, cur = (int)OWN[1] == CUR.pass;\n" +
+            std::string(tail ? "        const int nown = a.tail.n_items > 0 ? " + tl + ".n_own : 0;\n" : "") +
+            "        const int nl = cur ? (int)OWN[0] : 0;\n"
+            "        for (int i = 0; i < nl; ++i) {\n"
+            "            const int G_ = (int)OWN[2 + i];\n" + rows +
+            "        }\n"
+            "        if (cur && OWN[kOwnFull] != 0u) {\n"
+            "            const u64 want = (CUR.base + (u64)CUR.pass + 1ull) | ((u64)(blockIdx.x + 1u) << kOwnShift);\n"
+            "            for (int g0 = 0; g0 < ngrp; g0 += 1024) {\n"
+            "                __syncthreads();\n"
+            "                if (threadIdx.x < 32) QL[threadIdx.x] = 0u;\n"
+            "                __syncthreads();\n"
+            "                for (int j = threadIdx.x; j < 1024 && g0 + j < ngrp; j += blockDim.x)\n"
+            "                    if (ld64(&claim[(size_t)(g0 + j) * kClaimStride + kProgWord]) == want) atomicOr(&QL[j >> 5], 1u << (j & 31));\n"
+            "                __syncthreads();\n"
+            "                for (int j = 0; j < 1024 && g0 + j < ngrp; ++j) {\n"
+            "                    if (!(QL[j >> 5] >> (j & 31) & 1u)) continue;\n"
+            "                    const int G_ = g0 + j;\n    " + rows +
+            "                }\n"
+            "            }\n"
+            "        }\n"
+            "        if ((CUR.fin & 2) && grid_close(a.mask, a.ctl, a.err, a.herr, nwords, a.tm, t0s, &CUR, &QL[65]))\n"
+            "            poison_outputs(a);\n"
+            "    }\n";
+        return o;
+    }
     std::string loop_text() const {
+        if (early()) return loop_text_early();
         return "    bool spec = persistent && spec_first, spec_ok = true, own = true;\n"
                "    if (spec && threadIdx.x == 0) spec_ok = grid_claim(claim, (int)blockIdx.x, (CURP)->base);\n"
                "    for (;;) {\n"
@@ -883,11 +953,28 @@
                     o += "    for (size_t i = threadIdx.x; i < (size_t)" + it(per_env[k]) +
                          " * a.B; i += blockDim.x) a.out[" + it(k) + "][i] = nan;\n";
             o += "}\n\n";
+            if (early()) {
+                const int comp[6] = {2, 2, 1, 1, 2, 1};
+                o += "__device__ __forceinline__ void poison_group(const Args& a, int g) {\n"
+                     "    const float nan = __builtin_nanf(\"\");\n"
+                     "    const int b0 = g * 64, nb = a.B - b0 < 64 ? a.B - b0 : 64;\n";
+                for (int k = 0; k < 6; ++k)
+                    if (per_env[k] > 0)
+                        o += "    for (int i = threadIdx.x; i < " + it(per_env[k]) + " * nb; i += blockDim.x)\n"
+                             "        a.out[" + it(k) + "][((size_t)(i / (" + it(comp[k]) + " * nb)) * a.B + b0) * " + it(comp[k]) +
+                             " + i % (" + it(comp[k]) + " * nb)] = nan;\n";
+                o += "}\n\n";
+                o += "__device__ __attribute__((noinline)) void own_group(const Args& a, const VmasTail* t, int g, bool bad) {\n"
+                     "    if (t) vmas_tail::own_rows(*t, g, a.B);\n"
+                     "    if (bad) poison_group(a, g);\n"
+                     "}\n\n";
+            }
         }
         o += "template <int WAVE>\n__device__ __forceinline__ void group_loop(const Args& a, float* L, uint32_t* FL, uint32_t* DONE, "
              "uint32_t* MSK, uint32_t* QL, uint32_t* RED, float* EQ, GridCursor* CURP, uint32_t* claim, TimerStart t0s, "
              "bool persistent, bool spec_first, int nfl, int nwords, int ngrp, int lane, int wave" +
-             std::string(has_epi() ? std::string(", const ") + epi_type() + "* PROG_IOP" : std::string()) + ") {\n    (void)EQ;\n";
+             std::string(has_epi() ? std::string(", const ") + epi_type() + "* PROG_IOP" : std::string()) +
+             std::string(early() ? ", uint32_t* OWN" : "") + ") {\n    (void)EQ;\n";
         o += loop_text();
         o += "}\n\n";
         o += "__device__ __forceinline__ void world_body(const Args& a) {\n";
@@ -899,6 +986,8 @@
         if (has_epi() && !epi_q_in_rows()) o += "    __shared__ float EQ[" + it((long)kEpiQRows * 64) + "];\n";
         if (has_epi()) o += std::string("    __shared__ __attribute__((aligned(16))) ") + epi_type() + " PROG_IO;\n";
         o += "    __shared__ uint32_t DONE[" + it(std::max(n_split, 1)) + "];\n";
+        if (early())
+            o += "    __shared__ uint32_t OWN[" + it(vmas::kOwnList + 5) + "];\n    __shared__ long long OD[3];\n";
         if (tail_stage)
             o += "    __shared__ __attribute__((aligned(16))) VmasTail TL;\n";
         const int red_words = nfl + 2;
@@ -934,7 +1023,16 @@
                  "    }\n"
                  : "") +
              prm_copy() +
+             std::string(early() ? "    if (threadIdx.x < " + it(vmas::kOwnList + 5) + ") OWN[threadIdx.x] = 0u;\n" : "") +
              "    __syncthreads();\n" +
+             std::string(early() ?
+                 "    if (persistent && a.epi && PROG_IO.out_delta) {\n"
+                 "        if (threadIdx.x < 3) OD[threadIdx.x] = PROG_IO.out_delta[threadIdx.x];\n"
+                 "        __syncthreads();\n"
+                 "        if (threadIdx.x == 0) PROG_IO.out_delta = reinterpret_cast<decltype(PROG_IO.out_delta)>(&OD[0]);\n"
+                 "        __syncthreads();\n"
+                 "    }\n"
+                 : "") +
              block_stamp(0, "__builtin_amdgcn_s_memrealtime()") + block_stamp(1, "__builtin_amdgcn_s_getreg(63492)") +
              block_stamp(2, "__builtin_amdgcn_s_getreg(30740)") +
              (prof_block >= 0 ? "    if (lane == 0 && blockIdx.x < " + it(kProfBlocks) + ") a.prof[" +
@@ -948,12 +1046,28 @@
             sw += "        case " + it(w) + ": group_loop<" + it(w) + ">(a, L, FL, DONE, MSK, QL, RED, " +
                   std::string(has_epi() && !epi_q_in_rows() ? "EQ" : "nullptr") +
                   ", &CUR, claim, t0s, persistent, spec_first, nfl, nwords, ngrp, lane, wave" +
-                  std::string(has_epi() ? ", &PROG_IO" : "") + "); break;\n";
+                  std::string(has_epi() ? ", &PROG_IO" : "") + std::string(early() ? ", OWN" : "") + "); break;\n";
         o += sw + "        default: break;\n    }\n";
         o += block_stamp(3, "__builtin_amdgcn_s_memrealtime()") +
+             std::string(early() ?
+                 "    if (persistent && a.epi && CUR.fin) {  // (the final decider: its own decision)\n"
+                 "        if (threadIdx.x == 0) {\n"
+                 "            OWN[kOwnDwg] = blockIdx.x & 0xffffu;\n"
+                 "            OWN[kOwnBad] = (CUR.fin & 4) ? 1u : 0u;\n"
+                 "        }\n"
+                 "        __syncthreads();\n"
+                 "    }\n" : "") +
+             std::string(tail && early() && tail_stage ?
+                 "    // (completion-first: the final decider's program is the last thing running -- the\n"
+                 "    // other workgroups share its units, vmas_tail.hpp skip1)\n"
+                 "    if (persistent && a.epi && a.tail.n_items > 0 && gridDim.x <= 65536u) {\n"
+                 "        if (threadIdx.x == 0) TL.skip1 = (int)OWN[kOwnDwg] + 1;\n"
+                 "        __syncthreads();\n"
+                 "    }\n" : "") +
              std::string(tail ? "    // the replay's post-replay work (vmas_tail.hpp): every group's final pass is decided\n"
                                 "    if (persistent && a.tail.n_items > 0) " +
                                     std::string(tail_stage ? "vmas_tail::run(TL)" : "vmas_tail::run(a.tail)") + ";\n" : "") +
+             (early() ? after_early() : std::string()) +
              "    if (!persistent) {\n"
              "        if (!a.blk) return;\n"
              "        __syncthreads();\n"
@@ -978,6 +1092,8 @@
     const bool allow_split = !(sp && sp[0] == '0');
     const char* spr = getenv("VMAS_JIT_SIDE_PRUNE");
     const bool side_prune = !(spr && spr[0] == '0');
+    const char* cfs = getenv("VMAS_JIT_COMPLETION_FIRST");
+    const bool completion_first = !(cfs && cfs[0] == '0');
     const struct {
         bool split;
         long budget;
@@ -993,6 +1109,7 @@
         }
         g->split_boxes = t.split;
         g->side_prune = side_prune;
+        g->completion_first = completion_first;
         g->lds_budget = t.budget;
         g->global_rows = t.global_rows;
         int n_tasks = 0;
@@ -1290,6 +1407,7 @@
         info.epi_offset = W->fn_prog ? (long)W->epi_offset : -1L;
         info.wbd_offset = (long)g.wbd_offset();
         info.tail_offset = g.tail ? (long)g.tail_offset() : -1L;
+        info.completion_first = g.early() ? 1 : 0;
         info.batch = cfg->batch;
         info.epilogue = g.has_epi() ? cfg->epilogue : VMAS_EPILOGUE_NONE;
         info.io_bytes = cfg->epilogue == VMAS_EPILOGUE_BALANCE ? sizeof(VmasBalanceIO)
diff --git a/vectorizedmultiagentsimulator_amd/csrc/vmas_jit_ops.hpp b/vectorizedmultiagentsimulator_amd/csrc/vmas_jit_ops.hpp
--- a/vectorizedmultiagentsimulator_amd/csrc/vmas_jit_ops.hpp
+++ b/vectorizedmultiagentsimulator_amd/csrc/vmas_jit_ops.hpp
@@ -90,6 +90,31 @@
     return cas64(&claim[(size_t)g * kClaimStride], G, G + 1ull);
 }
 
+constexpr u64 kDecSeqMask = (1ull << 46) - 1ull, kDecBad = 1ull << 46;
+constexpr int kDecWgShift = 48;
+
+constexpr int kProgWord = 2, kOwnShift = 44, kOwnList = 12;
+constexpr u64 kProgSeqMask = (1ull << kOwnShift) - 1ull;
+
+__device__ __forceinline__ void grid_prog_done(uint32_t* claim, int g, u64 G, bool listed) {
+    __builtin_amdgcn_s_waitcnt(0);
+    __syncthreads();
+    if (threadIdx.x == 0)
+        st64(&claim[(size_t)g * kClaimStride + kProgWord], (G + 1ull) | (listed ? 0ull : (u64)(blockIdx.x + 1u) << kOwnShift));
+}
+
+__device__ __forceinline__ void grid_prog_wait(const uint32_t* claim, int g, u64 G, uint32_t* err, uint32_t* herr) {
+    const uint32_t* w = &claim[(size_t)g * kClaimStride + kProgWord];
+    const unsigned long long t0 = __builtin_amdgcn_s_memrealtime();
+    while ((ld64(w) & kProgSeqMask) != G) {
+        if (__builtin_amdgcn_s_memrealtime() - t0 > kGridStartWaitTicks) {
+            report_err(err, herr, kGridErrStateTimeout);
+            break;
+        }
+        __builtin_amdgcn_s_sleep(4);
+    }
+}
+
 __device__ __forceinline__ int grid_steal(uint32_t* claim, int ngrp, u64 G, uint32_t* LIST, bool* seen) {
     if (threadIdx.x == 0) LIST[64] = 0u;
     __syncthreads();
@@ -152,7 +177,7 @@
 
 __device__ inline bool grid_decide(const uint32_t* blk, uint32_t* nmask, const uint32_t* MSK, uint32_t* ctl, uint32_t* err,
                                    uint32_t* herr, int nwords, int ngrp, u64 G, int pass, int max_pass, uint32_t* RED,
-                                   unsigned long long* tm, TimerStart t0s, GridCursor* CUR) {
+                                   unsigned long long* tm, TimerStart t0s, GridCursor* CUR, bool defer_close = false) {
     const int nw2 = 2 * nwords;
     const bool force = pass + 1 < VMAS_GRID_MIN_PASSES;
     if (threadIdx.x == 0) RED[nw2] = (force || ld64(&ctl[kGridCand]) == G + 1ull) ? 1u : 0u;
@@ -199,7 +224,14 @@
     if (threadIdx.x == 0) {
         if (viol && !more) report_err(err, herr, kGridErrNoConverge);
         if (!more) st_agent(&ctl[2], (uint32_t)(pass + 1));
-        st64(&ctl[kGridDec + 2 * (int)(G % (u64)kGridMaxPasses)], ((G + 1ull) << 1) | (more ? 1ull : 0ull));
+        st64(&ctl[kGridDec + 2 * (int)(G % (u64)kGridMaxPasses)],
+             ((G + 1ull) << 1) | (more ? 1ull : 0ull) | (viol && !more ? kDecBad : 0ull) |
+                 ((u64)(blockIdx.x & 0xffffu) << kDecWgShift));
+    }
+    if (!more && defer_close) {
+        if (threadIdx.x == 0) CUR->fin = 2 | (viol ? 4 : 0);
+        __syncthreads();
+        return viol;
     }
     if (!more) {
         const bool self = CUR->started != 0;
@@ -227,7 +259,7 @@
                 grid_started(ctl);
                 CUR->started = 1;
             }
-            CUR->fin = 1;
+            CUR->fin = 1 | (viol ? 4 : 0);
             if (tm) grid_time(tm, t0s);
         }
         __syncthreads();
@@ -238,13 +270,60 @@
     return RED[nw2 + 1] == 2u || (viol && !more);
 }
 
-__device__ __forceinline__ bool grid_wait(uint32_t* ctl, u64 G, uint32_t* FLAG, int* started) {
+__device__ inline bool grid_close(uint32_t* nmask, uint32_t* ctl, uint32_t* err, uint32_t* herr, int nwords,
+                                  unsigned long long* tm, TimerStart t0s, GridCursor* CUR, uint32_t* FLAG) {
+    __syncthreads();
+    const int pass = CUR->pass;
+    const u64 G = CUR->base + (u64)pass;
+    const bool self = CUR->started != 0;
+    if (threadIdx.x == 0) *FLAG = 0u;
+    __syncthreads();
+    if (threadIdx.x < 64) {
+        const u64 base = ld64(&ctl[kGridStartBase]);
+        const u64 want = base + (u64)gridDim.x - (self ? 0ull : 1ull);
+        const unsigned long long t0 = __builtin_amdgcn_s_memrealtime();
+        bool late = false;
+        while (grid_starts(ctl) != want) {
+            if (__builtin_amdgcn_s_memrealtime() - t0 > kGridStartWaitTicks) {
+                late = true;
+                break;
+            }
+            __builtin_amdgcn_s_sleep(8);
+        }
+        if (threadIdx.x == 0) {
+            st64(&ctl[kGridStartBase], base + (u64)gridDim.x);
+            if (late) {
+                *FLAG = 1u;
+                report_err(err, herr, kGridErrStateTimeout);
+            }
+            st64(&ctl[kGridEpoch], G + 1ull);
+            if (!self) {
+                grid_started(ctl);
+                CUR->started = 1;
+            }
+            CUR->fin = (CUR->fin & 4) | 1;
+            if (tm) grid_time(tm, t0s);
+        }
+    }
+    __syncthreads();
+    if (pass > 0)
+        for (int w = threadIdx.x; w < nwords; w += blockDim.x) st_agent(&nmask[w], 0u);
+    const bool late = *FLAG != 0u;
+    __syncthreads();
+    return late;
+}
+
+__device__ __forceinline__ bool grid_wait(uint32_t* ctl, u64 G, uint32_t* FLAG, int* started, uint32_t* FINAL) {
     if (threadIdx.x == 0) {
         if (!*started) grid_started(ctl);
         const uint32_t* dec = &ctl[kGridDec + 2 * (int)(G % (u64)kGridMaxPasses)];
         u64 d;
-        while (((d = ld64(dec)) >> 1) != G + 1ull) __builtin_amdgcn_s_sleep(4);
+        while ((((d = ld64(dec)) & kDecSeqMask) >> 1) != G + 1ull) __builtin_amdgcn_s_sleep(4);
         *FLAG = (uint32_t)(d & 1ull);
+        if (FINAL && !(d & 1ull)) {
+            FINAL[0] = (uint32_t)(d >> kDecWgShift);
+            FINAL[1] = (d & kDecBad) ? 1u : 0u;
+        }
     }
     *started = 1;
     __syncthreads();
@@ -258,7 +337,8 @@
 #endif
 
 __device__ __attribute__((noinline)) int grid_next(bool persistent, uint32_t* ctl, uint32_t* claim, const uint32_t* mask,
-                                                   uint32_t* MSK, int nwords, int ngrp, GridCursor* CUR, uint32_t* QL) {
+                                                   uint32_t* MSK, int nwords, int ngrp, GridCursor* CUR, uint32_t* QL,
+                                                   uint32_t* FINAL = nullptr) {
     GridCursor c = *CUR;
     int g = -1;
     if (c.fin) return g;
@@ -297,7 +377,7 @@
             c.nl = grid_steal(claim, ngrp, c.base + (u64)c.pass, QL, &seen);
             c.il = 0;
             if (seen) continue;
-            if (!grid_wait(ctl, c.base + (u64)c.pass, &QL[65], &c.started)) break;
+            if (!grid_wait(ctl, c.base + (u64)c.pass, &QL[65], &c.started, FINAL)) break;
             ++c.pass;
             c.own = (int)blockIdx.x;
             c.nl = c.il = 0;
@@ -314,7 +394,8 @@
                                                       const uint32_t* MSK, uint32_t* ctl, uint32_t* err, uint32_t* herr,
                                                       int nwords, int ngrp, GridCursor* CUR, int max_pass,
                                                       uint32_t* RED, uint32_t* FLAG, unsigned long long* tm,
-                                                      unsigned long long t0_rt, unsigned long long t0_sc) {
+                                                      unsigned long long t0_rt, unsigned long long t0_sc,
+                                                      bool defer_close = false) {
     const TimerStart t0s{t0_rt, t0_sc};
     __syncthreads();
     const int pass = CUR->pass;
@@ -327,7 +408,29 @@
                                          __HIP_MEMORY_SCOPE_AGENT);
     }
     return grid_complete(ctl, g, ngrp, G, FLAG) &&
-           grid_decide(blk, nmask, MSK, ctl, err, herr, nwords, ngrp, G, pass, max_pass, RED, tm, t0s, CUR);
-}
-
-}
+           grid_decide(blk, nmask, MSK, ctl, err, herr, nwords, ngrp, G, pass, max_pass, RED, tm, t0s, CUR, defer_close);
+}
+
+constexpr int kOwnFull = 2 + kOwnList, kOwnDwg = 3 + kOwnList, kOwnBad = 4 + kOwnList;
+
+__device__ __attribute__((noinline)) void grid_enter(const uint32_t* claim, int g, const GridCursor* CUR, uint32_t* OWN,
+                                                     uint32_t* err, uint32_t* herr) {
+    if (threadIdx.x != 0) return;
+    const int pass = CUR->pass;
+    if ((int)OWN[1] != pass) {
+        OWN[0] = 0u;
+        OWN[1] = (uint32_t)pass;
+        OWN[kOwnFull] = 0u;
+    }
+    if (pass > 0) grid_prog_wait(claim, g, CUR->base + (u64)pass, err, herr);
+}
+
+__device__ __attribute__((noinline)) void grid_listed(uint32_t* claim, int g, const GridCursor* CUR, uint32_t* OWN, bool listed) {
+    grid_prog_done(claim, g, CUR->base + (u64)CUR->pass, listed);
+    if (threadIdx.x == 0) {
+        if (listed) OWN[2 + OWN[0]++] = (uint32_t)g;
+        else OWN[kOwnFull] = 1u;
+    }
+}
+
+}
diff --git a/vectorizedmultiagentsimulator_amd/csrc/vmas_jit_registry.hpp b/vectorizedmultiagentsimulator_amd/csrc/vmas_jit_registry.hpp
--- a/vectorizedmultiagentsimulator_amd/csrc/vmas_jit_registry.hpp
+++ b/vectorizedmultiagentsimulator_amd/csrc/vmas_jit_registry.hpp
@@ -20,6 +20,7 @@
     int batch;
     int epilogue;
     size_t io_bytes;
+    int completion_first;
 };
 
 bool jit_fn_info(const void* f, JitFnInfo* out);
diff --git a/vectorizedmultiagentsimulator_amd/csrc/vmas_kernels.hip b/vectorizedmultiagentsimulator_amd/csrc/vmas_kernels.hip
--- a/vectorizedmultiagentsimulator_amd/csrc/vmas_kernels.hip
+++ b/vectorizedmultiagentsimulator_amd/csrc/vmas_kernels.hip
@@ -882,6 +882,8 @@
     mutable std::vector<char> tail_buf;
     mutable size_t tail_size = 0;
     mutable void* tail_extra[5] = {nullptr, nullptr, nullptr, nullptr, nullptr};
+    bool tail_sources_set = false;
+    std::vector<VmasTailSource> tail_sources;
 };
 
 namespace {
@@ -1137,6 +1139,13 @@
 
 int32_t vmas_graph_chain_launch_wb(const VmasKernelChain* c, void* stream) { return chain_launch(c, stream, true); }
 
+int32_t vmas_graph_chain_set_tail_sources(VmasKernelChain* c, const VmasTailSource* sources, int32_t n) {
+    if (!c || n < 0 || (n > 0 && !sources)) return fail(VMAS_E_INVALID, "vmas_graph_chain_set_tail_sources: bad arguments");
+    c->tail_sources.assign(sources, sources + n);
+    c->tail_sources_set = true;
+    return VMAS_OK;
+}
+
 int32_t vmas_graph_chain_launch_tail(const VmasKernelChain* c, int32_t wb, const VmasCopySpan* spans, int32_t n_spans,
                                      int64_t numel, const VmasUniformColumn* cols, int32_t n_cols, uint64_t seed,
                                      uint64_t offset, const uint64_t* offset_dev, int32_t mode, int64_t u_snap_delta,
@@ -1155,11 +1164,30 @@
     static const char* diag = getenv("VMAS_TAIL_DIAG");
     const bool no_copy = diag && strcmp(diag, "nocopy") == 0, no_draw = diag && strcmp(diag, "nodraw") == 0;
     if (no_draw) n_cols = 0;
-    int n = 0;
+    int n = 0, n_own = 0;
+    VmasCopySpan own[kTailOwn];
+    const bool owners = a.completion_first != 0;
+    if (owners && !c->tail_sources_set) return 0;
     for (int i = 0; i < n_spans; ++i) {
         const VmasCopySpan& sp = spans[i];
         if (sp.nbytes == 0 || (sp.nbytes > 0 && sp.src == sp.dst)) continue;
         if (no_copy && sp.src && sp.nbytes != VMAS_COPY_STORE64) continue;
+        if (owners && sp.src && sp.nbytes > 0) {
+            const VmasTailSource* hit = nullptr;
+            for (const VmasTailSource& ts : c->tail_sources)
+                if ((uintptr_t)sp.src < (uintptr_t)ts.base + (uint64_t)ts.nbytes &&
+                    (uintptr_t)sp.src + (uint64_t)sp.nbytes > (uintptr_t)ts.base)
+                    hit = &ts;
+            if (hit) {
+                if (sp.src != hit->base || sp.nbytes != hit->nbytes || hit->row_bytes <= 0 ||
+                    hit->row_bytes > (1 << 20) || sp.nbytes != (int64_t)a.batch * hit->row_bytes || !sp.dst ||
+                    (((uintptr_t)sp.src | (uintptr_t)sp.dst | (uintptr_t)sp.nbytes) & 3) || n_own == kTailOwn)
+                    return 0;
+                t.own_rb[n_own] = (int)hit->row_bytes;
+                own[n_own++] = sp;
+                continue;
+            }
+        }
         if (sp.nbytes == VMAS_COPY_STORE64) {
             if (!sp.dst || ((uintptr_t)sp.dst & 7)) return 0;
         } else if (sp.nbytes < 0 || !sp.dst || (((uintptr_t)sp.src | (uintptr_t)sp.dst | (uintptr_t)sp.nbytes) & 3)) {
@@ -1168,6 +1196,9 @@
         if (n == kTailSpans) return 0;
         t.s[n++] = sp;
     }
+    if (n + n_own > kTailSpans) return 0;
+    for (int k = 0; k < n_own; ++k) t.s[n + k] = own[k];
+    t.n_own = n_own;
     int gx = 0;
     unsigned long long inc = 0;
     if (n_cols > 0) {
diff --git a/vectorizedmultiagentsimulator_amd/csrc/vmas_tail.hpp b/vectorizedmultiagentsimulator_amd/csrc/vmas_tail.hpp
--- a/vectorizedmultiagentsimulator_amd/csrc/vmas_tail.hpp
+++ b/vectorizedmultiagentsimulator_amd/csrc/vmas_tail.hpp
@@ -6,7 +6,7 @@
 
 #include "../../include/vmas_mi355x.h"
 
-constexpr int kTailSpans = 16, kTailCols = 12, kTailThreads = 256;
+constexpr int kTailSpans = 16, kTailCols = 12, kTailThreads = 256, kTailOwn = 8;
 
 struct VmasTail {
     VmasCopySpan s[kTailSpans];
@@ -16,6 +16,8 @@
     const unsigned long long* off_dev;
     int n_spans, n_items, gx_draw, mode;
     int first[kTailSpans + kTailCols + 1];
+    int n_own, skip1;
+    int own_rb[kTailOwn];
     int pad;
 };
 
@@ -125,8 +127,14 @@
 }
 
 __device__ __forceinline__ void run(const VmasTail& t) {
-    const long long T = (long long)gridDim.x * blockDim.x, total = t.first[t.n_items];
-    for (long long u = (long long)blockIdx.x * blockDim.x + threadIdx.x; u < total; u += 2 * T) {
+    long long nb = gridDim.x, bi = blockIdx.x;
+    if (t.skip1 > 0 && nb > 1) {
+        if (bi == t.skip1 - 1) return;
+        nb -= 1;
+        bi -= bi >= t.skip1 ? 1 : 0;
+    }
+    const long long T = nb * blockDim.x, total = t.first[t.n_items];
+    for (long long u = bi * blockDim.x + threadIdx.x; u < total; u += 2 * T) {
         Unit a, b;
         prep(t, u, a);
         prep(t, u + T, b);
@@ -135,5 +143,24 @@
     }
 }
 
+__device__ __forceinline__ void own_rows(const VmasTail& t, int g, int batch) {
+    const long long r0 = (long long)g * 64, r1 = r0 + 64 < (long long)batch ? r0 + 64 : (long long)batch;
+    for (int k = 0; k < t.n_own; ++k) {
+        const VmasCopySpan& s = t.s[t.n_spans + k];
+        const long long lo = r0 * t.own_rb[k], hi = r1 * t.own_rb[k];
+        if ((((unsigned long long)s.src | (unsigned long long)s.dst | (unsigned long long)s.nbytes) & 7) == 0) {
+            const unsigned long long* src = reinterpret_cast<const unsigned long long*>(s.src);
+            unsigned long long* dst = reinterpret_cast<unsigned long long*>(s.dst);
+            for (long long i = lo / 8 + threadIdx.x; i < hi / 8; i += blockDim.x)
+                dst[i] = __hip_atomic_load(src + i, __ATOMIC_RELAXED, __HIP_MEMORY_SCOPE_AGENT);
+        } else {
+            const uint32_t* src = reinterpret_cast<const uint32_t*>(s.src);
+            uint32_t* dst = reinterpret_cast<uint32_t*>(s.dst);
+            for (long long i = lo / 4 + threadIdx.x; i < hi / 4; i += blockDim.x)
+                dst[i] = __hip_atomic_load(src + i, __ATOMIC_RELAXED, __HIP_MEMORY_SCOPE_AGENT);
+        }
+    }
+}
+
 }
 #endif
diff --git a/vectorizedmultiagentsimulator_amd/simulator/environment/_post.py b/vectorizedmultiagentsimulator_amd/simulator/environment/_post.py
--- a/vectorizedmultiagentsimulator_amd/simulator/environment/_post.py
+++ b/vectorizedmultiagentsimulator_amd/simulator/environment/_post.py
@@ -143,6 +143,20 @@
         t.steps = st
 
 
+def tail_source(v: Tensor, batch: int) -> Optional[Tuple[int, int, int]]:
+    if v.dim() < 1 or v.shape[0] != batch or batch <= 0 or not v.is_contiguous():
+        return None
+    nbytes = v.numel() * v.element_size()
+    if nbytes == 0 or nbytes % 4 or v.data_ptr() % 4:
+        return None
+    return v.data_ptr(), nbytes, nbytes // batch
+
+
+def tail_group_words(g: int, batch: int, row_bytes: int, word: int) -> Tuple[int, int]:
+    r0, r1 = 64 * g, min(64 * g + 64, batch)
+    return r0 * row_bytes // word, r1 * row_bytes // word
+
+
 def _ahead_offset_word(deferred):
     if len(deferred) != 1:
         return None if deferred else 0
@@ -229,10 +243,19 @@
             tensors = list(srcs())
         except Exception:
             return False
+        sources = []
         for v in tensors:
             if not isinstance(v, Tensor) or not v.is_contiguous() or v.device.type != "cuda":
                 return False
             ranges.append((v.data_ptr(), v.data_ptr() + v.numel() * v.element_size()))
+            sources.append(tail_source(v, self.env.num_envs))
+        if any(s is None for s in sources):
+            return False
+        arr = (N.VmasTailSource * max(len(sources), 1))()
+        for i, (base, nbytes, row_bytes) in enumerate(sources):
+            arr[i].base, arr[i].nbytes, arr[i].row_bytes = base, nbytes, row_bytes
+        if N.load_library().vmas_graph_chain_set_tail_sources(ch.handle, arr, len(sources)) != 0:
+            return False
         if self.state_idx is not None:
             y = self.carry_src[self.state_idx]
             ranges.append((y.data_ptr(), y.data_ptr() + y.numel()))
@@ -284,9 +307,9 @@
                 tail = 0
                 if ch[0] and not mid:
                     ok = t.tail_ok
-                    if ok is None:
-                        ok = t.tail_ok = self._tail_admit(t, chain)
-                    if ok:
+                    if ok is None or ok[0] != chain.addr:
+                        ok = t.tail_ok = (chain.addr, self._tail_admit(t, chain))
+                    if ok[1]:
                         tail = fns[2]
                 views, acts, snap, seed, off, inc = N.load_host().post_draw(
                     host, drawer, mid, hi, P.data_ptr(), P.numel(), fns[3], off_dev, *ch, tail, int(wb))
```
